# qq456cvb/CanonicalVoting

Hardware: AMD Instinct MI355X
Metric: scenes/sec (80k-pt synthetic scans) (higher is better)
Workload: dtype f32

## Files before the change

canonicalvoting_amd/_lib.py:

```python
import ctypes
import os
import threading

_HERE = os.path.dirname(os.path.abspath(__file__))
LIB_PATH = os.path.join(_HERE, "_C", "libcvhip.so")

c_float_p = ctypes.POINTER(ctypes.c_float)
c_int_p = ctypes.POINTER(ctypes.c_int)
c_i32_p = ctypes.POINTER(ctypes.c_int32)
c_i64_p = ctypes.POINTER(ctypes.c_int64)
vp = ctypes.c_void_p
ABI_VERSION = 6


class CvError(RuntimeError):
    pass


class DecodeParams(ctypes.Structure):
    _fields_ = [("thresh_high", ctypes.c_float), ("thresh_low", ctypes.c_float),
                ("valid_ratio", ctypes.c_float), ("elimination", ctypes.c_int),
                ("prob_thresh", ctypes.c_float), ("elim_hi_plus1", ctypes.c_int),
                ("max_iters", ctypes.c_int), ("err_thresh", ctypes.c_double)]


class ConvDesc(ctypes.Structure):
    _fields_ = [("in_", vp), ("n_in", ctypes.c_longlong), ("in_ld", ctypes.c_int), ("cin", ctypes.c_int),
                ("weight", vp), ("K", ctypes.c_int), ("cout", ctypes.c_int), ("nbr", vp),
                ("n_out", ctypes.c_longlong), ("scale", vp), ("shift", vp), ("residual", vp),
                ("res_ld", ctypes.c_int), ("relu", ctypes.c_int), ("out", vp), ("out_ld", ctypes.c_int),
                ("flavour", ctypes.c_int), ("ws", vp), ("ws_bytes", ctypes.c_size_t), ("row_perm", vp),
                ("j_begin", ctypes.c_int), ("j_end", ctypes.c_int), ("acc_in", vp), ("acc_ld", ctypes.c_int),
                ("perm_groups", ctypes.c_int), ("plan_ent", vp), ("plan_cnt", vp),
                ("weight_packed", vp), ("weight_x6", vp), ("in2", vp), ("in2_ld", ctypes.c_int), ("cin2", ctypes.c_int),
                ("weight2_x6", vp), ("perm_has_map", ctypes.c_int), ("weight_pieces", ctypes.c_int),
                ("acc_scale", ctypes.c_float), ("range_flag", vp), ("in_hl", ctypes.c_int), ("out_hl", ctypes.c_int),
                ("res_hl", ctypes.c_int), ("split_tickets", vp), ("acc_scale_dev", vp)]


class SceneMaps(ctypes.Structure):
    _fields_ = [("stem", ctypes.c_longlong), ("out", ctypes.c_longlong), ("down", ctypes.c_longlong * 4),
                ("k3", ctypes.c_longlong * 5), ("up", ctypes.c_longlong * 4), ("mask_perm", ctypes.c_longlong * 5),
                ("up_perm", ctypes.c_longlong * 4), ("scratch", ctypes.c_longlong), ("bitmap", ctypes.c_longlong)]


class ScenePlanLayout(ctypes.Structure):
    _fields_ = [("cap", ctypes.c_longlong), ("perm", ctypes.c_longlong), ("inv", ctypes.c_longlong),
                ("coords", ctypes.c_longlong * 5), ("vals", ctypes.c_longlong * 5), ("counts", ctypes.c_longlong),
                ("arena", ctypes.c_longlong), ("int_words", ctypes.c_longlong), ("key_words", ctypes.c_longlong),
                ("sort_ws_bytes", ctypes.c_size_t), ("levels_ws_bytes", ctypes.c_size_t)]


NET_MAP_SLOTS, NET_PERM_SLOTS = 15, 9


class NetBuf(ctypes.Structure):
    _fields_ = [("level", ctypes.c_int), ("channels", ctypes.c_int), ("rows_level", ctypes.c_int), ("hl", ctypes.c_int)]


class NetOp(ctypes.Structure):
    _fields_ = [("in_buf", ctypes.c_int), ("in_col", ctypes.c_int), ("cin", ctypes.c_int),
                ("out_buf", ctypes.c_int), ("out_col", ctypes.c_int), ("cout", ctypes.c_int),
                ("res_buf", ctypes.c_int), ("res_col", ctypes.c_int), ("map", ctypes.c_int), ("K", ctypes.c_int),
                ("perm", ctypes.c_int), ("perm_groups", ctypes.c_int), ("relu", ctypes.c_int),
                ("weight", vp), ("scale", vp), ("shift", vp), ("weight_x6", vp), ("in2_buf", ctypes.c_int),
                ("in2_col", ctypes.c_int), ("cin2", ctypes.c_int), ("weight2_x6", vp), ("weight_pieces", ctypes.c_int), ("acc_scale", ctypes.c_float)]


class NetModelParams(ctypes.Structure):
    _fields_ = [("weight_x6", vp), ("weight2_x6", vp), ("scale", vp), ("shift", vp), ("acc_scale", ctypes.c_float),
                ("reserved", ctypes.c_int * 3)]


class SceneDesc(ctypes.Structure):
    _fields_ = [("d_coords4", vp), ("n", ctypes.c_longlong), ("d_feats", vp), ("feats_ld", ctypes.c_int), ("d_points", vp),
                ("res", ctypes.c_float), ("num_rots", ctypes.c_int), ("ops", vp), ("n_ops", ctypes.c_int), ("bufs", vp),
                ("n_bufs", ctypes.c_int), ("stem_k", ctypes.c_int), ("mask_groups", ctypes.c_int),
                ("masked_min_rows", ctypes.c_longlong), ("max_channels", ctypes.c_int),
                ("use_range_flag", ctypes.c_int),
                ("d_out_feats", vp), ("out_ld", ctypes.c_int), ("out_channels", ctypes.c_int), ("nclasses", ctypes.c_int),
                ("log_scale", ctypes.c_int), ("d_xyz_in", vp), ("d_scale_in", vp), ("d_prob_in", vp), ("d_class_in", vp),
                ("vote_algo", ctypes.c_int), ("decode", DecodeParams), ("max_candidates", ctypes.c_int),
                ("nms_threshold", ctypes.c_double), ("d_ws", vp), ("ws_bytes", ctypes.c_size_t), ("d_grids", vp),
                ("grid_capacity_floats", ctypes.c_size_t), ("h_pinned", vp), ("pinned_bytes", ctypes.c_size_t),
                ("h_cand_idx", vp), ("h_verdict", vp), ("h_boxes", vp), ("h_scores", vp), ("h_classes", vp), ("h_pick", vp),
                ("adaptive_split", ctypes.c_int), ("events", vp * 5),
                ("conv_split_target", ctypes.c_int), ("vote_part_records", ctypes.c_int)]


MAX_CATEGORIES = 16


class SceneSeparateDesc(ctypes.Structure):
    _fields_ = [("d_coords4", vp), ("n", ctypes.c_longlong), ("d_feats", vp), ("feats_ld", ctypes.c_int), ("d_points", vp),
                ("res", ctypes.c_float), ("num_rots", ctypes.c_int), ("num_models", ctypes.c_int),
                ("ops", vp), ("n_ops", vp), ("bufs", vp), ("n_bufs", vp),
                ("stem_k", ctypes.c_int), ("mask_groups", ctypes.c_int), ("masked_min_rows", ctypes.c_longlong),
                ("max_channels", ctypes.c_int), ("use_range_flag", ctypes.c_int),
                ("d_out_feats", vp), ("out_ld", ctypes.c_int), ("out_channels", ctypes.c_int), ("log_scale", ctypes.c_int),
                ("d_xyz_in", vp), ("d_scale_in", vp), ("d_prob_in", vp), ("vote_algo", ctypes.c_int), ("decode", DecodeParams),
                ("max_candidates", ctypes.c_int), ("nms_threshold", ctypes.c_double), ("d_ws", vp), ("ws_bytes", ctypes.c_size_t),
                ("h_pinned", vp), ("pinned_bytes", ctypes.c_size_t), ("h_cand_idx", vp), ("h_verdict", vp), ("h_boxes", vp),
                ("h_scores", vp), ("h_det_cat", vp), ("h_det_box", vp), ("events", vp * 5),
                ("conv_split_target", ctypes.c_int), ("vote_part_records", ctypes.c_int),
                ("models_per_pass", ctypes.c_int), ("d_model_params", vp)]


class SceneSeparateResult(ctypes.Structure):
    _fields_ = [("n_cand", ctypes.c_int * MAX_CATEGORIES), ("n_boxes", ctypes.c_int * MAX_CATEGORIES),
                ("truncated", ctypes.c_int * MAX_CATEGORIES), ("n_det", ctypes.c_int), ("range_flag", ctypes.c_int),
                ("duplicates", ctypes.c_int), ("out_of_window", ctypes.c_int), ("dims", ctypes.c_int * 3),
                ("corner", ctypes.c_float * 3), ("level_rows", ctypes.c_longlong * 5), ("needed_ws_bytes", ctypes.c_size_t),
                ("d_grid_obj", vp), ("d_grid_rot", vp), ("d_grid_scale", vp), ("d_xyz", vp), ("d_scale", vp), ("d_prob", vp),
                ("host_us", ctypes.c_float * 4)]


class PackJob(ctypes.Structure):
    _fields_ = [("w", vp), ("wp", vp), ("K", ctypes.c_int), ("cin", ctypes.c_int), ("cout", ctypes.c_int), ("trans", ctypes.c_int),
                ("scale_log2", ctypes.c_int), ("reserved", ctypes.c_int)]


class SceneResult(ctypes.Structure):
    _fields_ = [("n_cand", ctypes.c_int), ("n_boxes", ctypes.c_int), ("n_det", ctypes.c_int), ("truncated", ctypes.c_int),
                ("range_flag", ctypes.c_int), ("duplicates", ctypes.c_int), ("out_of_window", ctypes.c_int),
                ("scenes_in_flight", ctypes.c_int), ("dims", ctypes.c_int * 3), ("corner", ctypes.c_float * 3), ("level_rows", ctypes.c_longlong * 5),
                ("needed_ws_bytes", ctypes.c_size_t), ("needed_grid_floats", ctypes.c_size_t),
                ("d_grid_obj", vp), ("d_grid_rot", vp), ("d_grid_scale", vp), ("d_xyz", vp), ("d_scale", vp),
                ("d_prob", vp), ("d_class", vp), ("host_us", ctypes.c_float * 4)]


GATHER_MAX_JOBS = 8


class GatherJob(ctypes.Structure):
    _fields_ = [("d_src", vp), ("src_ld", ctypes.c_longlong), ("d_dst", vp), ("dst_ld", ctypes.c_longlong),
                ("width", ctypes.c_int), ("recentre_from", ctypes.c_int)]


class PointsFront(ctypes.Structure):
    _fields_ = [("d_raw_points", vp), ("m", ctypes.c_longlong), ("points_ld", ctypes.c_longlong), ("points_f64", ctypes.c_int),
                ("quantization_size", ctypes.c_double), ("d_raw_feats", vp), ("raw_feats_ld", ctypes.c_longlong),
                ("in_channels", ctypes.c_int), ("recentre_from", ctypes.c_int), ("d_raw_xyz", vp), ("d_raw_scale", vp),
                ("d_raw_prob", vp), ("d_raw_class", vp), ("d_coords4", vp), ("d_index", vp), ("d_inverse", vp)]


class PointsDesc(ctypes.Structure):
    _fields_ = [("front", PointsFront), ("scene", SceneDesc)]


class PointsSeparateDesc(ctypes.Structure):
    _fields_ = [("front", PointsFront), ("scene", SceneSeparateDesc)]


class PointsResult(ctypes.Structure):
    _fields_ = [("scene", SceneResult), ("n", ctypes.c_longlong), ("rejected", ctypes.c_int), ("host_us_front", ctypes.c_float),
                ("front_ws_bytes", ctypes.c_size_t), ("d_feats", vp), ("d_points", vp), ("d_xyz_in", vp), ("d_scale_in", vp),
                ("d_prob_in", vp), ("d_class_in", vp)]


class PointsSeparateResult(ctypes.Structure):
    _fields_ = [("scene", SceneSeparateResult), ("n", ctypes.c_longlong), ("rejected", ctypes.c_int),
                ("host_us_front", ctypes.c_float), ("front_ws_bytes", ctypes.c_size_t), ("d_feats", vp), ("d_points", vp),
                ("d_xyz_in", vp), ("d_scale_in", vp), ("d_prob_in", vp)]


SIGNATURES = {
    "cv_abi_version": (ctypes.c_int, []),
    "cv_last_error": (ctypes.c_char_p, []),
    "cv_hv_minmax_workspace_bytes": (ctypes.c_size_t, []),
    "cv_hv_minmax_f32": (ctypes.c_int, [vp, ctypes.c_int64, c_float_p, c_float_p, vp, ctypes.c_size_t, vp]),
    "cv_hv_minmax_async_f32": (ctypes.c_int, [vp, ctypes.c_int64, vp, vp, ctypes.c_size_t, vp]),
    "cv_hv_grid_dims_f32": (ctypes.c_int, [c_float_p, c_float_p, ctypes.c_float, c_int_p]),
    "cv_hv_forward_workspace_bytes": (ctypes.c_size_t, [ctypes.c_int64, ctypes.c_int, c_int_p, ctypes.c_int]),
    "cv_hv_forward_f32": (ctypes.c_int, [vp, vp, vp, vp, ctypes.c_int64, ctypes.c_float, ctypes.c_int,
                                         c_float_p, c_int_p, vp, vp, vp, vp, ctypes.c_size_t,
                                         ctypes.c_int, vp]),
    "cv_hv_forward_cat_workspace_bytes": (ctypes.c_size_t, [ctypes.c_int64, ctypes.c_int, c_int_p, ctypes.c_int, ctypes.c_int]),
    "cv_hv_forward_cat_f32": (ctypes.c_int, [vp, vp, vp, vp, ctypes.c_int64, ctypes.c_float, ctypes.c_int, c_float_p, c_int_p,
                                             ctypes.c_int, vp, vp, vp, vp, ctypes.c_size_t, ctypes.c_int, vp]),
    "cv_hv_set_kernel_events": (ctypes.c_int, [vp, vp]),
    "cv_hv_backward_f32": (ctypes.c_int, [vp, vp, vp, vp, vp, ctypes.c_int64, ctypes.c_float,
                                          ctypes.c_int, c_float_p, c_int_p, vp, vp, vp, vp]),
    "cv_hv_count_votes_f32": (ctypes.c_int, [vp, vp, vp, ctypes.c_int64, ctypes.c_float, ctypes.c_int,
                                             c_float_p, c_int_p, c_i64_p, vp, ctypes.c_size_t, vp]),
    "cv_decode_workspace_bytes": (ctypes.c_size_t, [c_int_p, ctypes.c_int64, ctypes.c_int]),
    "cv_decode_f32": (ctypes.c_int, [vp, vp, vp, c_int_p, c_float_p, ctypes.c_float, vp, vp, vp, vp,
                                     ctypes.c_int64, ctypes.POINTER(DecodeParams), ctypes.c_int, vp,
                                     ctypes.c_size_t, c_int_p, c_i64_p, c_i32_p, c_int_p, c_float_p,
                                     c_float_p, c_i32_p, c_int_p, vp]),
    "cv_decode_cat_workspace_bytes": (ctypes.c_size_t, [c_int_p, ctypes.c_int64, ctypes.c_int, ctypes.c_int]),
    "cv_decode_cat_f32": (ctypes.c_int, [vp, vp, vp, c_int_p, c_float_p, ctypes.c_float, vp, vp, vp, vp, ctypes.c_int64,
                                         ctypes.c_int, ctypes.POINTER(DecodeParams), ctypes.c_int, vp, ctypes.c_size_t, c_int_p,
                                         c_i64_p, c_i32_p, c_int_p, c_float_p, c_float_p, c_i32_p, c_int_p, vp]),
    "cv_detect_scene_separate_f32": (ctypes.c_int, [ctypes.POINTER(SceneSeparateDesc), ctypes.POINTER(SceneSeparateResult), vp]),
    "cv_sp_table_capacity": (ctypes.c_longlong, [ctypes.c_longlong]),
    "cv_sp_levels_workspace_bytes": (ctypes.c_size_t, [ctypes.c_longlong]),
    "cv_sp_build_levels": (ctypes.c_int, [ctypes.POINTER(vp), ctypes.POINTER(vp), ctypes.POINTER(vp),
                                          ctypes.c_longlong, ctypes.c_longlong, ctypes.c_int, vp,
                                          c_i32_p, vp, ctypes.c_size_t, vp]),
    "cv_sp_quantize_workspace_bytes": (ctypes.c_size_t, [ctypes.c_longlong]),
    "cv_sp_quantize_f32": (ctypes.c_int, [vp, ctypes.c_longlong, ctypes.c_longlong, ctypes.c_float, ctypes.c_int, c_i64_p,
                                          ctypes.c_int, vp, vp, vp, vp, c_i32_p, vp, ctypes.c_size_t, vp]),
    "cv_sp_quantize_f64": (ctypes.c_int, [vp, ctypes.c_longlong, ctypes.c_longlong, ctypes.c_double, ctypes.c_int, c_i64_p,
                                          ctypes.c_int, vp, vp, vp, vp, c_i32_p, vp, ctypes.c_size_t, vp]),
    "cv_sp_voxel_rows_f32": (ctypes.c_int, [vp, vp, ctypes.c_longlong, ctypes.c_float, vp, ctypes.POINTER(GatherJob), ctypes.c_int, vp]),
    "cv_sizeof_gather_job": (ctypes.c_size_t, []),
    "cv_sp_morton_keys": (ctypes.c_int, [vp, ctypes.c_longlong, vp, vp]),
    "cv_sp_sort_workspace_bytes": (ctypes.c_size_t, [ctypes.c_longlong]),
    "cv_sp_sort_rows": (ctypes.c_int, [vp, ctypes.c_longlong, vp, vp, vp, vp, ctypes.c_size_t, vp]),
    "cv_sp_pack_weights_stem_h2_f32": (ctypes.c_int, [vp, ctypes.c_int, ctypes.c_int, vp, ctypes.c_int, vp, vp]),
    "cv_sp_to_hl_f32": (ctypes.c_int, [vp, ctypes.c_longlong, ctypes.c_int, ctypes.c_int, vp, ctypes.c_int, vp, vp]),
    "cv_sp_from_hl_f32": (ctypes.c_int, [vp, ctypes.c_longlong, ctypes.c_int, ctypes.c_int, vp, ctypes.c_int, vp]),
    "cv_sp_kernel_map": (ctypes.c_int, [vp, ctypes.c_longlong, vp, vp, ctypes.c_longlong, ctypes.c_int,
                                        ctypes.c_int, vp, vp]),
    "cv_sp_up_map": (ctypes.c_int, [vp, ctypes.c_longlong, ctypes.c_longlong, vp, vp]),
    "cv_sp_conv_workspace_bytes": (ctypes.c_size_t, [ctypes.c_longlong, ctypes.c_int, ctypes.c_int]),
    "cv_sp_conv_f32": (ctypes.c_int, [ctypes.POINTER(ConvDesc), vp]),
    "cv_sp_set_split_target": (ctypes.c_int, [ctypes.c_int]),
    "cv_hv_set_part_records": (ctypes.c_int, [ctypes.c_int]),
    "cv_hv_set_part_records_thread": (ctypes.c_int, [ctypes.c_int]),
    "cv_sp_pack_weights_h2_batch_f32": (ctypes.c_int, [ctypes.POINTER(PackJob), ctypes.c_int, vp, vp]),
    "cv_sp_copy_unless_flag": (ctypes.c_int, [ctypes.POINTER(vp), ctypes.POINTER(vp), ctypes.POINTER(ctypes.c_longlong), ctypes.c_int, vp, vp]),
    "cv_sp_pack_weights_t_f32": (ctypes.c_int, [vp, ctypes.c_int, ctypes.c_int, ctypes.c_int, ctypes.c_int, ctypes.c_int, vp, vp]),
    "cv_sp_set_split_target_thread": (ctypes.c_int, [ctypes.c_int]),
    "cv_sp_set_ablation": (ctypes.c_int, [ctypes.c_int]),
    "cv_sp_set_option": (ctypes.c_int, [ctypes.c_char_p, ctypes.c_longlong, ctypes.POINTER(ctypes.c_longlong)]),
    "cv_sp_get_option": (ctypes.c_int, [ctypes.c_char_p, ctypes.POINTER(ctypes.c_longlong)]),
    "cv_sp_pack_weights_x6_f32": (ctypes.c_int, [vp, ctypes.c_int, ctypes.c_int, ctypes.c_int, vp, vp, vp]),
    "cv_sp_pack_weights_h2_f32": (ctypes.c_int, [vp, ctypes.c_int, ctypes.c_int, ctypes.c_int, vp, ctypes.c_int, vp, vp]),
    "cv_sp_pack_weights_bf16_f32": (ctypes.c_int, [vp, ctypes.c_int, ctypes.c_int, ctypes.c_int, vp, vp, vp]),
    "cv_sp_scene_maps_words": (ctypes.c_size_t, [c_i64_p, ctypes.c_longlong, ctypes.c_int, ctypes.c_int,
                                                 ctypes.c_longlong, ctypes.POINTER(SceneMaps)]),
    "cv_sp_scene_maps": (ctypes.c_int, [ctypes.POINTER(vp), ctypes.POINTER(vp), ctypes.POINTER(vp), ctypes.c_longlong,
                                        c_i64_p, vp, ctypes.c_longlong, ctypes.c_int,
                                        ctypes.c_int, ctypes.c_longlong, vp, ctypes.c_size_t, vp]),
    "cv_sp_scene_plan_words": (ctypes.c_size_t, [ctypes.c_longlong, ctypes.c_int, ctypes.c_int, ctypes.c_longlong]),
    "cv_sp_scene_plan": (ctypes.c_int, [vp, ctypes.c_longlong, vp, vp, ctypes.POINTER(vp), ctypes.POINTER(vp),
                                        ctypes.POINTER(vp), ctypes.c_longlong, vp, c_i32_p, ctypes.c_int, ctypes.c_int,
                                        ctypes.c_longlong, vp, ctypes.c_size_t, ctypes.POINTER(SceneMaps), vp,
                                        ctypes.c_size_t, vp, ctypes.c_size_t, vp]),
    "cv_sp_scene_plan_layout": (ctypes.c_int, [ctypes.c_longlong, ctypes.c_int, ctypes.c_int, ctypes.c_longlong,
                                               ctypes.POINTER(ScenePlanLayout)]),
    "cv_sp_scene_plan_slots": (ctypes.c_int, [ctypes.POINTER(ScenePlanLayout), ctypes.POINTER(SceneMaps), c_i64_p,
                                              ctypes.c_longlong, vp, ctypes.POINTER(vp), ctypes.POINTER(vp)]),
    "cv_sp_scene_conv_workspace_bytes": (ctypes.c_size_t, [c_i64_p, c_int_p, ctypes.c_int, ctypes.c_int]),
    "cv_net_arena_bytes": (ctypes.c_size_t, [ctypes.POINTER(NetBuf), ctypes.c_int, c_i64_p, ctypes.c_int]),
    "cv_net_run_f32": (ctypes.c_int, [ctypes.POINTER(NetOp), ctypes.c_int, ctypes.POINTER(NetBuf), ctypes.c_int,
                                      c_i64_p, ctypes.c_int, vp, ctypes.c_size_t, ctypes.POINTER(vp), c_int_p,
                                      ctypes.POINTER(vp), ctypes.c_int, ctypes.POINTER(vp), ctypes.c_int,
                                      vp, ctypes.c_size_t, vp, vp]),
    "cv_net_models_params_bytes": (ctypes.c_size_t, [ctypes.c_int, ctypes.c_int]),
    "cv_net_models_params_fill": (ctypes.c_int, [ctypes.POINTER(vp), ctypes.c_int, ctypes.c_int, vp, ctypes.c_size_t]),
    "cv_net_models_arena_bytes": (ctypes.c_size_t, [ctypes.POINTER(NetBuf), ctypes.c_int, c_i64_p, ctypes.c_int, ctypes.c_int]),
    "cv_net_models_workspace_bytes": (ctypes.c_size_t, [ctypes.c_size_t, ctypes.c_int]),
    "cv_net_run_models_f32": (ctypes.c_int, [ctypes.POINTER(vp), ctypes.POINTER(vp), ctypes.c_int, ctypes.c_int, ctypes.c_int,
                                             c_i64_p, ctypes.c_int, vp, ctypes.c_size_t, ctypes.POINTER(vp), c_int_p,
                                             ctypes.POINTER(vp), ctypes.c_int, ctypes.POINTER(vp), ctypes.c_int,
                                             vp, ctypes.c_size_t, vp, vp, ctypes.c_int, vp]),
    "cv_head_separate_models_f32": (ctypes.c_int, [ctypes.POINTER(vp), ctypes.c_int, ctypes.c_longlong, ctypes.c_int, ctypes.c_int,
                                                   vp, vp, vp, vp]),
    "cv_sp_mask_keys": (ctypes.c_int, [vp, ctypes.c_longlong, ctypes.c_int, ctypes.c_int, ctypes.c_int, vp, vp]),
    "cv_sp_mask_perms": (ctypes.c_int, [vp, ctypes.c_longlong, ctypes.c_int, ctypes.c_int, vp, vp, ctypes.c_size_t,
                                        ctypes.c_int, vp]),
    "cv_sp_transpose_map": (ctypes.c_int, [vp, ctypes.c_longlong, ctypes.c_int, ctypes.c_longlong, vp, vp]),
    "cv_sp_wgrad_workspace_bytes": (ctypes.c_size_t, [ctypes.c_longlong, ctypes.c_int, ctypes.c_int, ctypes.c_int]),
    "cv_sp_conv_wgrad_f32": (ctypes.c_int, [vp, ctypes.c_int, ctypes.c_int, vp, ctypes.c_int, ctypes.c_int, vp,
                                            ctypes.c_int, ctypes.c_longlong, vp, vp, ctypes.c_size_t, vp]),
    "cv_sp_conv_wgrad_px_f32": (ctypes.c_int, [vp, ctypes.c_int, ctypes.c_int, vp, ctypes.c_int, ctypes.c_int, vp,
                                               ctypes.c_int, ctypes.c_longlong, vp, vp, ctypes.c_size_t, ctypes.c_int,
                                               vp]),
    "cv_sp_col_sum_f32": (ctypes.c_int, [vp, ctypes.c_longlong, ctypes.c_int, ctypes.c_int, vp, vp]),
    "cv_sp_col_sum_workspace_bytes": (ctypes.c_size_t, [ctypes.c_longlong, ctypes.c_int]),
    "cv_sp_col_sum_det_f32": (ctypes.c_int, [vp, ctypes.c_longlong, ctypes.c_int, ctypes.c_int, vp, vp, ctypes.c_size_t, vp]),
    "cv_sp_bn_workspace_bytes": (ctypes.c_size_t, [ctypes.c_int]),
    "cv_sp_bn_stats_f32": (ctypes.c_int, [vp, ctypes.c_longlong, ctypes.c_int, ctypes.c_int, vp, vp, ctypes.c_float,
                                          ctypes.c_float, vp, vp, vp, vp, vp, vp, vp, ctypes.c_size_t, vp]),
    "cv_sp_bn_backward_f32": (ctypes.c_int, [vp, vp, vp, ctypes.c_longlong, ctypes.c_int, ctypes.c_int, vp, vp,
                                             ctypes.c_float, vp, vp, vp, vp, vp, vp, ctypes.c_size_t, vp]),
    "cv_sp_bn_backward_hl_f32": (ctypes.c_int, [vp, vp, vp, ctypes.c_longlong, ctypes.c_int, ctypes.c_int, vp, vp,
                                                ctypes.c_float, vp, vp, vp, vp, vp, vp, ctypes.c_size_t, vp, vp, vp, vp, vp]),
    "cv_sp_affine_f32": (ctypes.c_int, [vp, ctypes.c_longlong, ctypes.c_int, ctypes.c_int, vp, vp, vp, ctypes.c_int,
                                        ctypes.c_int, vp, ctypes.c_int, vp]),
    "cv_sp_affine_hl_f32": (ctypes.c_int, [vp, ctypes.c_longlong, ctypes.c_int, ctypes.c_int, vp, vp, vp, ctypes.c_int,
                                           ctypes.c_int, vp, ctypes.c_int, vp, ctypes.c_int, vp, vp, vp]),
    "cv_sp_bn_fold_f32": (ctypes.c_int, [vp, vp, vp, vp, vp, ctypes.c_float, ctypes.c_int, vp, vp, vp]),
    "cv_head_joint_f32": (ctypes.c_int, [vp, ctypes.c_longlong, ctypes.c_int, ctypes.c_int, ctypes.c_int,
                                         vp, vp, vp, vp, vp]),
    "cv_head_separate_f32": (ctypes.c_int, [vp, ctypes.c_longlong, ctypes.c_int, ctypes.c_int, vp, vp, vp, vp]),
    "cv_detect_scene_f32": (ctypes.c_int, [ctypes.POINTER(SceneDesc), ctypes.POINTER(SceneResult), vp]),
    "cv_detect_points_f32": (ctypes.c_int, [ctypes.POINTER(PointsDesc), ctypes.POINTER(PointsResult), vp]),
    "cv_detect_points_separate_f32": (ctypes.c_int, [ctypes.POINTER(PointsSeparateDesc), ctypes.POINTER(PointsSeparateResult), vp]),
    "cv_sizeof_points_desc": (ctypes.c_size_t, []),
    "cv_sizeof_points_separate_desc": (ctypes.c_size_t, []),
    "cv_sizeof_points_result": (ctypes.c_size_t, []),
    "cv_sizeof_points_separate_result": (ctypes.c_size_t, []),
    "cv_iou_obb": (ctypes.c_double, [c_float_p, c_float_p]),
    "cv_nms_obb": (ctypes.c_int, [c_float_p, c_float_p, ctypes.c_int, ctypes.c_double, c_i32_p]),
}

_lib = None


def lib():
    global _lib
    if _lib is None:
        if not os.path.exists(LIB_PATH):
            raise CvError(
                "canonicalvoting_amd: HIP library %s not found. Build it with "
                "`python -m canonicalvoting_amd.csrc.build` (hipcc, gfx950). There is no CPU "
                "fallback for this op." % LIB_PATH)
        import torch
        if torch.cuda.is_available():
            torch.cuda.init()
        L = ctypes.CDLL(LIB_PATH)
        for name, (res, args) in SIGNATURES.items():
            fn = getattr(L, name)
            fn.restype = res
            fn.argtypes = args
        _lib = L
    return _lib


_scratch_lock = threading.Lock()
_scratch_bufs = {}


def scratch(dev, name, nbytes):
    import torch
    key = (dev.index if dev.index is not None else torch.cuda.current_device(),
           torch.cuda.current_stream(dev).cuda_stream, name)
    nbytes = max(int(nbytes), 256)
    with _scratch_lock:
# ... 26 lines not shown
```

canonicalvoting_amd/csrc/hv_vote.hip:

```cpp
#include "cv_common.h"

#include <atomic>
#include <algorithm>
#include <cmath>
#include <cstddef>
#include <mutex>
#include <type_traits>
#include <unordered_map>
#include <vector>

namespace {

struct F3 { float x, y, z; };
struct I3 { int x, y, z; };

std::mutex g_tab_mu;
std::unordered_map<uint64_t, float2*> g_tabs;

int get_rot_table(int num_rots, const float2** out) {
    int dev = 0;
    CV_HIP_CHECK(hipGetDevice(&dev));
    const uint64_t key = (uint64_t(uint32_t(dev)) << 32) | uint32_t(num_rots);
    std::lock_guard<std::mutex> lk(g_tab_mu);
    auto it = g_tabs.find(key);
// ... 343 lines not shown
    __shared__ int wsum[FILL ? 1 : LIST_MAX_TILES];
    const int ntiles = tiles_x * tiles_z;
    const int c = blockIdx.x;
    if (c >= chunk_start[Y]) return;
    if (FILL && list_ctl[1] != 0) return;
    const int bin = bin_of_chunk[c];
    const int idx = ystart[bin] + (c - chunk_start[bin]) * LIST_CHUNK_RECORDS + (int)threadIdx.x;
    const int end = ystart[bin + 1];
    for (int t = threadIdx.x; t < ntiles; t += 1024) {
        cnt[t] = FILL ? list_start[(int64_t)bin * ntiles + t] + chunk_off[(int64_t)c * ntiles + t] : 0;
        if (!FILL) wsum[t] = 0;
    }
    __syncthreads();
    if (idx < end) {
        const float ux = rec[9 * rec_stride + idx], uz = rec[10 * rec_stride + idx], r = rec[11 * rec_stride + idx];
        const float a0 = rec[12 * rec_stride + idx];
        const float ext = r + 2.f + 1e-5f * (r + fabsf(ux) + fabsf(uz));
        const int tx0 = max(0, (int)floorf((ux - ext - (float)TX) / (float)TX));
        const int tx1 = min(tiles_x - 1, (int)floorf((ux + ext + 1.f) / (float)TX));
        const int tz0 = max(0, (int)floorf((uz - ext - (float)TZ) / (float)TZ));
        const int tz1 = min(tiles_z - 1, (int)floorf((uz + ext + 1.f) / (float)TZ));
        for (int tx = tx0; tx <= tx1; ++tx)
            for (int tz = tz0; tz <= tz1; ++tz) {
                const float xlo = (float)(tx * TX - 1), xhi = (float)(tx * TX + TX), zlo = (float)(tz * TZ - 1),
                            zhi = (float)(tz * TZ + TZ);
                float dxn, dzn;
                if (!ring_touches(ux, uz, r, xlo, xhi, zlo, zhi, dxn, dzn)) continue;
                int a_start, a_len;
                ring_arc(ux, uz, a0, R, xlo, xhi, zlo, zhi, dxn, dzn, a_start, a_len);
                const int t = tx * tiles_z + tz;
                if (FILL) {
                    const int p = atomicAdd(&cnt[t], 1);
                    entries[p] = make_int2(idx, a_start | (a_len << 16));
                } else {
                    if (want_lists) atomicAdd(&cnt[t], 1);
                    atomicAdd(&wsum[t], a_len);
                }
            }
    }
    if (FILL) return;
    __syncthreads();
    for (int t = threadIdx.x; t < ntiles; t += 1024) {
        if (want_lists) chunk_off[(int64_t)c * ntiles + t] = cnt[t] ? atomicAdd(&list_cnt[(int64_t)bin * ntiles + t], cnt[t]) : 0;
        if (wsum[t]) atomicAdd(&tile_w[(int64_t)bin * ntiles + t], wsum[t]);
    }
}

__global__ __launch_bounds__(1024) void hv_list_scan(const int* __restrict__ list_cnt, int Y, int ntiles, long long list_cap,
                                                     int* __restrict__ list_ctl, int* __restrict__ list_start, int64_t ks_ws) {
    list_cnt = cat_ws(list_cnt, ks_ws); list_ctl = cat_ws(list_ctl, ks_ws); list_start = cat_ws(list_start, ks_ws);
    __shared__ int s[1024];
    __shared__ long long carry_s;
    if (threadIdx.x == 0) carry_s = 0;
    __syncthreads();
    const int total_lists = Y * ntiles;
    for (int base = 0; base < total_lists; base += 1024) {
        const int i = base + threadIdx.x;
        const int v = i < total_lists ? list_cnt[i] : 0;
        s[threadIdx.x] = v;
        __syncthreads();
        for (int off = 1; off < 1024; off <<= 1) {
            const int t = (int)threadIdx.x >= off ? s[threadIdx.x - off] : 0;
            __syncthreads();
            s[threadIdx.x] += t;
            __syncthreads();
        }
        const long long incl = (long long)s[threadIdx.x] + carry_s;
        if (i < total_lists) list_start[i] = incl - v < 0x7fffffffll ? (int)(incl - v) : 0x7fffffff;
        __syncthreads();
        if (threadIdx.x == 1023) carry_s = incl;
        __syncthreads();
    }
    if (threadIdx.x == 0) { list_ctl[0] = carry_s < 0x7fffffffll ? (int)carry_s : 0x7fffffff; list_ctl[1] = carry_s > list_cap ? 1 : 0; }
}

constexpr int PART_VOTES = 32768;
constexpr int QUEUE_MAX_PARTS = 32;

__global__ __launch_bounds__(1024) void hv_build_queue(const int* __restrict__ tile_w, int Y, int ntiles, int max_items,
                                                       int max_slots, int* __restrict__ list_ctl ,
                                                       int4* __restrict__ items, int64_t ks_ws) {
    tile_w = cat_ws(tile_w, ks_ws); list_ctl = cat_ws(list_ctl, ks_ws); items = cat_ws(items, ks_ws);
    __shared__ unsigned long long s[1024];
    __shared__ unsigned long long carry_s;
    const int total = Y * ntiles;
    for (int pass = 0; pass < 2; ++pass) {
        if (threadIdx.x == 0) carry_s = 0ull;
        __syncthreads();
        for (int base = 0; base < total; base += 1024) {
            const int i = base + threadIdx.x;
            int parts = 0, y = 0, t = 0;
            if (i < total) {
                y = i / ntiles; t = i - y * ntiles;
                const long long w = (long long)(y >= 1 ? tile_w[(int64_t)(y - 1) * ntiles + t] : 0) +
                                    (long long)(y <= Y - 2 ? tile_w[(int64_t)y * ntiles + t] : 0);
                parts = w == 0 ? 0 : (pass ? 1 : (int)min((long long)QUEUE_MAX_PARTS, (w + PART_VOTES - 1) / PART_VOTES));
            }
            const unsigned long long v = i < total ? (((unsigned long long)max(parts, 1) << 32) | (unsigned)(parts > 1 ? parts : 0)) : 0ull;
            s[threadIdx.x] = v;
            __syncthreads();
            for (int off = 1; off < 1024; off <<= 1) {
                const unsigned long long x = (int)threadIdx.x >= off ? s[threadIdx.x - off] : 0ull;
                __syncthreads();
                s[threadIdx.x] += x;
                __syncthreads();
            }
            const unsigned long long excl = s[threadIdx.x] + carry_s - v;
            const int item0 = (int)(excl >> 32), slot0 = (int)(excl & 0xffffffffull);
            if (i < total && item0 + max(parts, 1) <= max_items && slot0 + (parts > 1 ? parts : 0) <= max_slots) {
                if (parts == 0) items[item0] = make_int4(y, t, 0, 0);
                for (int p2 = 0; p2 < parts; ++p2) items[item0 + p2] = make_int4(y, t, p2 | (parts << 8), slot0);
            }
            __syncthreads();
            if (threadIdx.x == 1023) carry_s = s[1023] + carry_s;
            __syncthreads();
        }
        const int n_items = (int)(carry_s >> 32), n_slots = (int)(carry_s & 0xffffffffull);
        if (n_items <= max_items && n_slots <= max_slots) {
            if (threadIdx.x == 0) list_ctl[2] = n_items;
            return;
        }
        __syncthreads();
    }
    if (threadIdx.x == 0) list_ctl[2] = min(total, max_items);
}

__device__ __forceinline__ int lanes_below(uint64_t mask) {
    return __builtin_amdgcn_mbcnt_hi((uint32_t)(mask >> 32),
                                     __builtin_amdgcn_mbcnt_lo((uint32_t)mask, 0));
}

constexpr double FX_SCALE = 68719476736.0;
constexpr double FX_MAGIC = 6755399441055744.0;
template <bool SMALL>
__device__ __forceinline__ unsigned long long fx_from_float(float v) {
    if (SMALL) {
        const double d = __builtin_fma((double)v, FX_SCALE, FX_MAGIC);
        return (unsigned long long)__double_as_longlong(d) - (unsigned long long)__double_as_longlong(FX_MAGIC);
    }
    return (unsigned long long)__double2ll_rn((double)fminf(fmaxf(v, -6.0e7f), 6.0e7f) * FX_SCALE);
}
template <bool SMALL>
__device__ __forceinline__ void lds_add(unsigned long long* p, float v) {
    __hip_atomic_fetch_add(p, fx_from_float<SMALL>(v), __ATOMIC_RELAXED, __HIP_MEMORY_SCOPE_WORKGROUP);
}
__device__ __forceinline__ double fx_value(unsigned long long q) { return (double)(long long)q * (1.0 / FX_SCALE); }
template <bool SMALL>
__device__ __forceinline__ void lds_add_obj(unsigned long long* p, float v) {
    unsigned long long q = fx_from_float<SMALL>(v);
    if (q == 0ull && v != 0.f) q = v > 0.f ? 1ull : ~0ull;
    __hip_atomic_fetch_add(p, q, __ATOMIC_RELAXED, __HIP_MEMORY_SCOPE_WORKGROUP);
}

constexpr int ACC_PITCH = TZ + 8, ACC_CH = TX * ACC_PITCH + 4, ACC_WORDS = 6 * ACC_CH;
__device__ __forceinline__ int acc_idx(int ch, int cell) { return ch * ACC_CH + (cell >> 5) * ACC_PITCH + (cell & 31); }

struct TileShared {
    unsigned long long acc[ACC_WORDS];
    float pq[9][LQ];
    int arc_start[LQ];
    int arc_cum[LQ];
    uint32_t vq_rec[TW][VQ];
    float vq_rx[TW][VQ];
    float vq_rz[TW][VQ];
    float2 tab[MAX_R_TILES];
    int next_chunk[2];
    int wtot[TW];
    int list_len;
    int more;
};

template <bool SMALL>
__device__ __forceinline__ void drain_vote(TileShared& sh, int lx, int lz, float rx, float rz, float wy, float ob,
                                           float s0, float s1, float s2, float2 cs) {
    const float wx[2] = {1.f - rx, rx}, wz[2] = {1.f - rz, rz};
#pragma unroll
    for (int bx = 0; bx < 2; ++bx)
#pragma unroll
        for (int bz = 0; bz < 2; ++bz) {
            const int cxl = lx + bx, czl = lz + bz;
            if (cxl < 0 || cxl >= TX || czl < 0 || czl >= TZ) continue;
            const float w = wx[bx] * wy * wz[bz] * ob;
            unsigned long long* a = sh.acc + cxl * ACC_PITCH + czl;
            lds_add_obj<SMALL>(a, w);
            lds_add<SMALL>(a + ACC_CH, w * cs.x);
            lds_add<SMALL>(a + 2 * ACC_CH, w * cs.y);
            lds_add<SMALL>(a + 3 * ACC_CH, w * s0);
            lds_add<SMALL>(a + 4 * ACC_CH, w * s1);
            lds_add<SMALL>(a + 5 * ACC_CH, w * s2);
        }
}

__device__ __forceinline__ void drain64(TileShared& sh, int wave, int slot, bool active) {
    float rx = 0.f, rz = 0.f, wy = 0.f, ob = 0.f, s0 = 0.f, s1 = 0.f, s2 = 0.f;
    float2 cs = make_float2(0.f, 0.f);
    int lx = 0, lz = 0;
    if (active) {
        const uint32_t rec = sh.vq_rec[wave][slot];
        rx = sh.vq_rx[wave][slot]; rz = sh.vq_rz[wave][slot];
        const int e = rec & 511, rot = (rec >> 9) & 255;
        lx = (int)((rec >> 17) & 63) - 1; lz = (int)((rec >> 23) & 63) - 1;
        wy = sh.pq[4][e]; ob = sh.pq[5][e];
        s0 = sh.pq[6][e]; s1 = sh.pq[7][e]; s2 = sh.pq[8][e];
        cs = sh.tab[rot];
    }
    const bool small = fabsf(ob) * fmaxf(1.f, fmaxf(fabsf(s0), fmaxf(fabsf(s1), fabsf(s2)))) < 16384.f;
    if (__all(small)) {
        if (active) drain_vote<true>(sh, lx, lz, rx, rz, wy, ob, s0, s1, s2, cs);
    } else {
        if (active) drain_vote<false>(sh, lx, lz, rx, rz, wy, ob, s0, s1, s2, cs);
    }
}

__device__ __forceinline__ void wave_sync_lds() {
    __builtin_amdgcn_fence(__ATOMIC_RELEASE, "wavefront");
    __builtin_amdgcn_wave_barrier();
    __builtin_amdgcn_fence(__ATOMIC_ACQUIRE, "wavefront");
}

__device__ __forceinline__ float arc_atan2(float y, float x) {
    const float ax = fabsf(x), ay = fabsf(y);
    const float a = fminf(ax, ay) * __builtin_amdgcn_rcpf(fmaxf(fmaxf(ax, ay), 1e-30f));
    const float q = a * a;
    float r = ((-0.0464964749f * q + 0.15931422f) * q - 0.327622764f) * q * a + a;
    r = ay > ax ? 1.57079637f - r : r;
    r = x < 0.f ? 3.14159274f - r : r;
    return y < 0.f ? -r : r;
}

__device__ __forceinline__ void edge_arc(float ux, float uz, float r, float a0, int R, float xlo, float xhi, float zlo,
                                         float zhi, int& a_start, int& a_len) {
    if (!(r >= 2.f)) return;
    const float slack = 0.05f, half_pi = 1.57079637f, two_pi = 6.28318531f;
    const float d4[4] = {xhi - ux, zhi - uz, ux - xlo, uz - zlo};
    const float inv_r = 1.f / r;
    float h[4];
#pragma unroll
    for (int k = 0; k < 4; ++k) {
        const float t = (d4[k] + slack) * inv_r;
        const float hk = arc_atan2(sqrtf(fmaxf(1.f - t * t, 0.f)), t) - 0.01f;
        h[k] = (t < 1.f && hk > 0.f) ? hk : -1.f;
    }
    float best = 0.f, best_end = 0.f;
#pragma unroll
    for (int k = 0; k < 4; ++k) {
        float lo = -h[k], hi = h[k];
        bool ok = h[k] > 0.f;
        if (ok && hi - lo > best) { best = hi - lo; best_end = (float)k * half_pi + hi; }
#pragma unroll
        for (int j = 1; j < 4; ++j) {
            const float hp = h[(k + j - 1) & 3], hn = h[(k + j) & 3];
            ok = ok && hn > 0.f && hp + hn >= half_pi;
            if (ok) {
                lo = fminf(lo, (float)j * half_pi - hn);
                hi = fmaxf(hi, (float)j * half_pi + hn);
                if (hi - lo > best) { best = hi - lo; best_end = (float)k * half_pi + hi; }
            }
        }
    }
    const float inside = fmaxf(two_pi - best, 0.f);
    const float inv_step = (float)R * 0.159154943f;
    const int len = (int)(inside * inv_step) + 6;
    if (len < a_len) {
        float first = (best_end - a0) * inv_step - 2.f;
        first -= (float)R * floorf(first / (float)R);
        a_start = min(max((int)first, 0), R - 1);
        a_len = len;
    }
}

template <bool QUEUE>
__global__ __launch_bounds__(TW * 64) void hv_fwd_tiles(
    int R, float res, F3 corner, I3 dims, const float2* __restrict__ tab,
    const int* __restrict__ ystart, const int4* __restrict__ items, const float* __restrict__ rec,
    int64_t rec_stride, int tiles_x, int tiles_z, unsigned long long* __restrict__ partials,
    int* __restrict__ arrivals, float* __restrict__ g_obj, float* __restrict__ g_rot,
    float* __restrict__ g_scale, const int* __restrict__ list_ctl, const int* __restrict__ list_start, const int* __restrict__ list_cnt,
    const int2* __restrict__ entries, int list_mode ,
    const int4* __restrict__ q_info, CatStride ks) {
    ystart = cat_ws(ystart, ks.ws); items = cat_ws(items, ks.ws); rec = cat_ws(rec, ks.ws);
    partials = cat_ws(partials, ks.ws); arrivals = cat_ws(arrivals, ks.ws); list_ctl = cat_ws(list_ctl, ks.ws);
    list_start = cat_ws(list_start, ks.ws); list_cnt = cat_ws(list_cnt, ks.ws); entries = cat_ws(entries, ks.ws);
    q_info = cat_ws(q_info, ks.ws);
    g_obj = cat_el(g_obj, ks.cells); g_rot = cat_el(g_rot, 2 * ks.cells); g_scale = cat_el(g_scale, 3 * ks.cells);
    __shared__ TileShared sh;
    __shared__ int last_flag;
    const int X = dims.x, Y = dims.y, Z = dims.z;
    const int ntiles = tiles_x * tiles_z;
    int y, tile, part, nparts, slot0, slot_stride;
    if (QUEUE) {
        if ((int)blockIdx.x >= list_ctl[2]) return;
        const int4 item = items[blockIdx.x];
        y = item.x; tile = item.y; part = item.z & 0xff; nparts = item.z >> 8; slot0 = item.w; slot_stride = 1;
    } else {
        tile = blockIdx.x % ntiles;
        const int4 qi = q_info[blockIdx.x / ntiles];
        if (qi.z < 0) return;
        y = qi.x; part = qi.y; nparts = qi.z;
        slot0 = qi.w * ntiles + tile; slot_stride = ntiles;
    }
    const int x0 = (tile / tiles_z) * TX, z0 = (tile % tiles_z) * TZ;
    const int lane = threadIdx.x & 63, wave = threadIdx.x >> 6;
    if (nparts == 0) {
        const int nx0 = min(TX, X - x0), nz0 = min(TZ, Z - z0);
        for (int i = threadIdx.x; i < TCELLS; i += TW * 64) {
            const int lx = i / TZ, lz = i % TZ;
            if (lx < nx0 && lz < nz0) {
                const int64_t cell = ((int64_t)(x0 + lx) * Y + y) * Z + z0 + lz;
                g_obj[cell] = 0.f;
                reinterpret_cast<float2*>(g_rot)[cell] = make_float2(0.f, 0.f);
                g_scale[cell * 3 + 0] = 0.f; g_scale[cell * 3 + 1] = 0.f; g_scale[cell * 3 + 2] = 0.f;
            }
        }
        return;
    }
    const bool use_list = QUEUE && list_mode == 2 && list_ctl[1] == 0;
    int lbeg[2] = {0, 0}, llen[2] = {0, 0};
    if (use_list) {
#pragma unroll
        for (int k = 0; k < 2; ++k) {
            const int s = y - 1 + k;
            if (s >= 0 && s <= Y - 2) {
                lbeg[k] = list_start[(int64_t)s * ntiles + tile];
                llen[k] = list_cnt[(int64_t)s * ntiles + tile];
            }
        }
    }

    int bin_beg[2], bin_end[2];
#pragma unroll
    for (int k = 0; k < 2; ++k) {
        const int s = y - 1 + k;
        const bool valid = s >= 0 && s <= Y - 2;
        bin_beg[k] = !valid ? 0 : (use_list ? lbeg[k] : ystart[s]);
        bin_end[k] = !valid ? 0 : (use_list ? lbeg[k] + llen[k] : ystart[s + 1]);
    }
    const float2 tab_mine = (int)threadIdx.x < R ? tab[threadIdx.x] : make_float2(0.f, 0.f);
    for (int i = threadIdx.x; i < ACC_WORDS; i += TW * 64) sh.acc[i] = 0ull;
    if ((int)threadIdx.x < R) sh.tab[threadIdx.x] = tab_mine;
    if (threadIdx.x < 2) sh.next_chunk[threadIdx.x] = 0;
    if (threadIdx.x == 2) { sh.list_len = 0; sh.more = 0; }
    __syncthreads();

    const float slack = 0.05f;
    const float xlo = (float)(x0 - 1), xhi = (float)(x0 + TX), zlo = (float)(z0 - 1),
                zhi = (float)(z0 + TZ);
    int vq_len = 0;

    const int per = use_list ? LIST_CHUNK : 64;
    int sb = 0;
    int c_mask = 0, c_idx[CULL_BATCH], c_arc = 0, c_k = 0;
#pragma unroll
    for (int j = 0; j < CULL_BATCH; ++j) c_idx[j] = 0;
    auto append = [&](int mask, const int (&idx)[CULL_BATCH], int arc, int k) -> int {
        int tot = 0, before[CULL_BATCH];
#pragma unroll
        for (int j = 0; j < CULL_BATCH; ++j) {
            const uint64_t m = __ballot((mask >> j) & 1);
            before[j] = tot + lanes_below(m);
            tot += __popcll(m);
        }
        if (tot == 0) return 0;
        int p0 = 0;
        if (lane == 0) p0 = atomicAdd(&sh.list_len, tot);
        p0 = __builtin_amdgcn_readfirstlane(p0);
#pragma unroll
        for (int j = 0; j < CULL_BATCH; ++j) {
            const int pos = p0 + before[j];
            if (((mask >> j) & 1) && pos < LQ) {
                sh.arc_start[pos] = idx[j] | (int)((unsigned)k << 31);
                if (use_list) sh.arc_cum[pos] = arc;
                mask &= ~(1 << j);
            }
        }
        return mask;
    };

    for (;;) {
        bool more = false;
        if (__ballot(c_mask != 0) != 0) {
            c_mask = append(c_mask, c_idx, c_arc, c_k);
            more = __ballot(c_mask != 0) != 0;
        }
        while (!more && sb < 2) {
            if (bin_beg[sb] >= bin_end[sb]) { ++sb; continue; }
            const int len = __builtin_amdgcn_readfirstlane(
                __hip_atomic_load(&sh.list_len, __ATOMIC_RELAXED, __HIP_MEMORY_SCOPE_WORKGROUP));
            if (len > LQ - 64) { more = true; break; }
            const int take = use_list ? 64 / LIST_CHUNK : CULL_BATCH;
            int c = 0;
            if (lane == 0) c = atomicAdd(&sh.next_chunk[sb], take);
            c = __builtin_amdgcn_readfirstlane(c);
            const int end = bin_end[sb];
            if (bin_beg[sb] + (c * nparts + part) * per >= end) { ++sb; continue; }
            int idx[CULL_BATCH], mask = 0, arc = 0;
#pragma unroll
            for (int j = 0; j < CULL_BATCH; ++j) idx[j] = 0;
            if (use_list) {
                const int e = bin_beg[sb] + ((c + lane / LIST_CHUNK) * nparts + part) * LIST_CHUNK + lane % LIST_CHUNK;
                if (e < end) {
                    const int2 en = entries[e];
                    idx[0] = en.x;
                    arc = en.y;
                    mask = 1;
                }
            } else {
                float ux[CULL_BATCH], uz[CULL_BATCH], r[CULL_BATCH];
#pragma unroll
                for (int j = 0; j < CULL_BATCH; ++j) {
                    idx[j] = bin_beg[sb] + ((c + j) * nparts + part) * 64 + lane;
                    const bool in = idx[j] < end;
                    ux[j] = in ? rec[9 * rec_stride + idx[j]] : 0.f;
                    uz[j] = in ? rec[10 * rec_stride + idx[j]] : 0.f;
                    r[j] = in ? rec[11 * rec_stride + idx[j]] : 0.f;
                }
#pragma unroll
                for (int j = 0; j < CULL_BATCH; ++j) {
                    const float dxn = fmaxf(0.f, fmaxf(xlo - ux[j], ux[j] - xhi));
                    const float dzn = fmaxf(0.f, fmaxf(zlo - uz[j], uz[j] - zhi));
                    const float dxf = fmaxf(fabsf(ux[j] - xlo), fabsf(ux[j] - xhi));
                    const float dzf = fmaxf(fabsf(uz[j] - zlo), fabsf(uz[j] - zhi));
                    const float dmin = sqrtf(dxn * dxn + dzn * dzn), dmax = sqrtf(dxf * dxf + dzf * dzf);
                    const float tol = slack + 1e-5f * (r[j] + fabsf(ux[j]) + fabsf(uz[j]));
                    const bool keep = idx[j] < end && (r[j] >= dmin - tol) && (r[j] <= dmax + tol);
                    mask |= (int)keep << j;
                }
            }
            c_mask = append(mask, idx, arc, sb);
            if (__ballot(c_mask != 0) != 0) {
#pragma unroll
                for (int j = 0; j < CULL_BATCH; ++j) c_idx[j] = idx[j];
                c_arc = arc; c_k = sb;
                more = true;
            }
        }
        if (more && lane == 0) sh.more = 1;
        __syncthreads();
        const int n = min(sh.list_len, LQ);
        const bool again = sh.more != 0;
        if (n == 0) break;

        const int p = threadIdx.x;
        int a_start = 0, a_len = 0;
        if (p < n) {
            const int w = sh.arc_start[p];
            const int idx = w & 0x7fffffff;
            if (use_list) {
                const int arc = sh.arc_cum[p];
                a_start = arc & 0xffff;
                a_len = arc >> 16;
            } else {
                const float ux = rec[9 * rec_stride + idx], uz = rec[10 * rec_stride + idx];
                const float dxn = fmaxf(0.f, fmaxf(xlo - ux, ux - xhi));
                const float dzn = fmaxf(0.f, fmaxf(zlo - uz, uz - zhi));
                a_len = R;
                if (dxn + dzn > 0.5f) {
                    const float b0 = arc_atan2(0.5f * (zlo + zhi) - uz, 0.5f * (xlo + xhi) - ux);
                    float lo = 0.f, hi = 0.f;
#pragma unroll
                    for (int k = 0; k < 4; ++k) {
                        float d = arc_atan2(((k & 2) ? zhi : zlo) - uz, ((k & 1) ? xhi : xlo) - ux) - b0;
                        d -= 6.28318531f * rintf(d * 0.159154943f);
                        lo = fminf(lo, d);
                        hi = fmaxf(hi, d);
                    }
                    const float a0 = rec[12 * rec_stride + idx];
                    const float inv_step = (float)R * 0.159154943f;
                    float first = (b0 + lo - a0) * inv_step - 2.f;
                    const int len = (int)((hi - lo) * inv_step) + 6;
                    first -= (float)R * floorf(first / (float)R);
                    a_start = min(max((int)first, 0), R - 1);
                    a_len = min(len, R);
                }
                edge_arc(ux, uz, rec[11 * rec_stride + idx], rec[12 * rec_stride + idx], R, xlo, xhi, zlo, zhi, a_start, a_len);
            }
            const float ry = rec[4 * rec_stride + idx];
            sh.pq[0][p] = rec[0 * rec_stride + idx];
            sh.pq[1][p] = rec[1 * rec_stride + idx];
            sh.pq[2][p] = rec[2 * rec_stride + idx];
            sh.pq[3][p] = rec[3 * rec_stride + idx];
            sh.pq[4][p] = (w < 0) ? (1.f - ry) : ry;
            sh.pq[5][p] = rec[5 * rec_stride + idx];
            sh.pq[6][p] = rec[6 * rec_stride + idx];
            sh.pq[7][p] = rec[7 * rec_stride + idx];
            sh.pq[8][p] = rec[8 * rec_stride + idx];
            sh.arc_start[p] = a_start;
        }
        int cum = a_len;
#pragma unroll
        for (int off = 1; off < 64; off <<= 1) {
            const int t = __shfl_up(cum, off);
            if (lane >= off) cum += t;
        }
        if (lane == 63) sh.wtot[wave] = cum;
        __syncthreads();
        if (threadIdx.x == 0) { sh.list_len = 0; sh.more = 0; }
        int items = 0;
#pragma unroll
        for (int w = 0; w < TW; ++w) {
            const int t = sh.wtot[w];
            if (w < wave) cum += t;
            items += t;
        }
        if (p < n) sh.arc_cum[p] = cum;
        __syncthreads();

        const int S = (items + LQ - 1) / LQ;
        const int slice = wave * 64 + lane;
        int it0 = slice * S;
        const int it1 = min(it0 + S, items);
        int e = 0;
        {
            int lo = 0, hi = n - 1;
            while (lo < hi) {
                const int mid = (lo + hi) >> 1;
                if (sh.arc_cum[mid] > it0) hi = mid; else lo = mid + 1;
            }
            e = lo;
        }
        int e_end = it0 < items ? sh.arc_cum[e] : 0;
        int rot = 0;
        float epx = 0.f, epz = 0.f, ecx = 0.f, ecz = 0.f;
        if (it0 < items) {
            const int e_beg = e > 0 ? sh.arc_cum[e - 1] : 0;
            rot = sh.arc_start[e] + (it0 - e_beg);
            if (rot >= R) rot -= R;
            epx = sh.pq[0][e]; epz = sh.pq[1][e];
            ecx = sh.pq[2][e]; ecz = sh.pq[3][e];
        }
        for (int step = 0; step < S; ++step, ++it0) {
            bool isvote = false;
            uint32_t vrec = 0;
            float rx = 0, rz = 0;
            if (it0 < it1) {
                if (it0 == e_end) {
                    ++e;
                    e_end = sh.arc_cum[e];
                    rot = sh.arc_start[e];
                    epx = sh.pq[0][e]; epz = sh.pq[1][e];
                    ecx = sh.pq[2][e]; ecz = sh.pq[3][e];
                }
                const float2 cs = sh.tab[rot];
                const float ox = (-cs.x) * ecx + cs.y * ecz;
                const float oz = (-cs.y) * ecx - cs.x * ecz;
                const float gx = grid_pos(epx, ox, corner.x, res);
                const float gz = grid_pos(epz, oz, corner.z, res);
                if (gx >= 0 && gz >= 0 && gx < (float)(X - 1) && gz < (float)(Z - 1)) {
                    const int lx = (int)gx - x0, lz = (int)gz - z0;
                    if (lx >= -1 && lx < TX && lz >= -1 && lz < TZ) {
                        isvote = true;
                        rx = gx - floorf(gx);
                        rz = gz - floorf(gz);
                        vrec = (uint32_t)e | ((uint32_t)rot << 9) | ((uint32_t)(lx + 1) << 17) |
                               ((uint32_t)(lz + 1) << 23);
                    }
                }
                if (++rot == R) rot = 0;
            }
            const uint64_t mv = __ballot(isvote);
            if (isvote) {
                const int q = vq_len + lanes_below(mv);
                sh.vq_rec[wave][q] = vrec;
                sh.vq_rx[wave][q] = rx;
                sh.vq_rz[wave][q] = rz;
            }
            vq_len += __popcll(mv);
            wave_sync_lds();
            if (vq_len >= 64) {
                vq_len -= 64;
                drain64(sh, wave, vq_len + lane, true);
            }
        }
        if (vq_len > 0) {
            drain64(sh, wave, lane, lane < vq_len);
            vq_len = 0;
        }
        wave_sync_lds();
        if (!again) break;
        __syncthreads();
    }
    __syncthreads();

    if (nparts > 1) {
        unsigned long long* mine = partials + ((int64_t)slot0 + (int64_t)part * slot_stride) * (6 * TCELLS);
        for (int i = threadIdx.x; i < 6 * TCELLS; i += TW * 64) mine[i] = sh.acc[acc_idx(i / TCELLS, i % TCELLS)];
        asm volatile("s_waitcnt vmcnt(0)" ::: "memory");
        __syncthreads();
        if (threadIdx.x == 0) {
            __builtin_amdgcn_fence(__ATOMIC_RELEASE, "agent");
            asm volatile("s_waitcnt vmcnt(0)" ::: "memory");
            const int old = __hip_atomic_fetch_add(&arrivals[y * ntiles + tile], 1, __ATOMIC_RELAXED,
                                                   __HIP_MEMORY_SCOPE_AGENT);
            last_flag = old == nparts - 1;
            if (last_flag) __builtin_amdgcn_fence(__ATOMIC_ACQUIRE, "agent");
        }
        __syncthreads();
        if (!last_flag) return;
        const unsigned long long* base = partials + (int64_t)slot0 * (6 * TCELLS);
        for (int i = threadIdx.x; i < 6 * TCELLS; i += TW * 64) {
            unsigned long long sum = 0ull;
            for (int p2 = 0; p2 < nparts; ++p2) sum += base[(int64_t)p2 * slot_stride * (6 * TCELLS) + i];
            sh.acc[acc_idx(i / TCELLS, i % TCELLS)] = sum;
        }
        __syncthreads();
    }

    const int nx = min(TX, X - x0), nz = min(TZ, Z - z0);
    for (int i = threadIdx.x; i < TCELLS; i += TW * 64) {
        const int lx = i / TZ, lz = i % TZ;
        if (lx < nx && lz < nz)
            g_obj[((int64_t)(x0 + lx) * Y + y) * Z + z0 + lz] = (float)fx_value(sh.acc[acc_idx(0, i)]);
    }
    for (int i = threadIdx.x; i < TCELLS * 2; i += TW * 64) {
        const int cell = i >> 1, j = i & 1;
        const int lx = cell / TZ, lz = cell % TZ;
        if (lx < nx && lz < nz) {
            const double d = (double)(float)fx_value(sh.acc[acc_idx(0, cell)]) + 1e-7;
            g_rot[(((int64_t)(x0 + lx) * Y + y) * Z + z0 + lz) * 2 + j] =
                (float)((double)(float)fx_value(sh.acc[acc_idx(1 + j, cell)]) / d);
        }
    }
    for (int i = threadIdx.x; i < TCELLS * 3; i += TW * 64) {
        const int cell = i / 3, j = i - cell * 3;
        const int lx = cell / TZ, lz = cell % TZ;
        if (lx < nx && lz < nz) {
            const double d = (double)(float)fx_value(sh.acc[acc_idx(0, cell)]) + 1e-7;
            g_scale[(((int64_t)(x0 + lx) * Y + y) * Z + z0 + lz) * 3 + j] =
                (float)((double)(float)fx_value(sh.acc[acc_idx(3 + j, cell)]) / d);
        }
    }
}

__global__ __launch_bounds__(256) void hv_bwd(
    const float* __restrict__ grad, const float* __restrict__ pts, const float* __restrict__ xyz,
    const float* __restrict__ scl, const float* __restrict__ obj, int64_t n, int R, float res,
    F3 corner, I3 dims, const float2* __restrict__ tab, float* __restrict__ d_xyz,
    float* __restrict__ d_scl, float* __restrict__ d_obj) {
    const int lane = threadIdx.x & 63;
    const int64_t c = blockIdx.x * 4ll + (threadIdx.x >> 6);
    if (c >= n) return;
    const int Y = dims.y, Z = dims.z;
    const float s0 = scl[c * 3 + 0], s1 = scl[c * 3 + 1], s2 = scl[c * 3 + 2];
    const float x0 = xyz[c * 3 + 0], x1 = xyz[c * 3 + 1], x2 = xyz[c * 3 + 2];
    const float cx = x0 * s0, cy = x1 * s1, cz = x2 * s2;
    const float px = pts[c * 3 + 0], py = pts[c * 3 + 1], pz = pts[c * 3 + 2];
    const float ob = obj[c];
    float a_obj = 0, a_x0 = 0, a_x1 = 0, a_x2 = 0, a_s0 = 0, a_s1 = 0, a_s2 = 0;
    for (int i = lane; i < R; i += 64) {
        const float2 cs = tab[i];
        const float ox = (-cs.x) * cx + cs.y * cz;
        const float oy = -cy;
        const float oz = (-cs.y) * cx - cs.x * cz;
        const float gx = grid_pos(px, ox, corner.x, res);
        const float gy = grid_pos(py, oy, corner.y, res);
        const float gz = grid_pos(pz, oz, corner.z, res);
        if (gx < 0 || gy < 0 || gz < 0 || gx >= (float)(dims.x - 1) || gy >= (float)(dims.y - 1) ||
            gz >= (float)(dims.z - 1))
            continue;
        const int fx = (int)gx, fy = (int)gy, fz = (int)gz;
        const float rx = gx - floorf(gx), ry = gy - floorf(gy), rz = gz - floorf(gz);
        const float w0x = 1.f - rx, w0y = 1.f - ry, w0z = 1.f - rz, w1x = rx, w1y = ry, w1z = rz;
        const int64_t b = ((int64_t)fx * Y + fy) * Z + fz;
        const int64_t sx = (int64_t)Y * Z, sy = Z;
        const float lll = grad[b], llh = grad[b + 1], lhl = grad[b + sy], lhh = grad[b + sy + 1];
        const float hll = grad[b + sx], hlh = grad[b + sx + 1], hhl = grad[b + sx + sy],
                    hhh = grad[b + sx + sy + 1];
        float dob = lll * w0x * w0y * w0z;
        dob += llh * w0x * w0y * w1z;
        dob += lhl * w0x * w1y * w0z;
        dob += lhh * w0x * w1y * w1z;
        dob += hll * w1x * w0y * w0z;
        dob += hlh * w1x * w0y * w1z;
        dob += hhl * w1x * w1y * w0z;
        dob += hhh * w1x * w1y * w1z;
        a_obj += dob;
        float dx = -lll * w0y * w0z;
        dx = dx - llh * w0y * w1z; dx = dx - lhl * w1y * w0z; dx = dx - lhh * w1y * w1z;
        dx = dx + hll * w0y * w0z; dx = dx + hlh * w0y * w1z; dx = dx + hhl * w1y * w0z;
        dx = dx + hhh * w1y * w1z;
        float dy = -lll * w0x * w0z;
        dy = dy - llh * w0x * w1z; dy = dy + lhl * w0x * w0z; dy = dy + lhh * w0x * w1z;
        dy = dy - hll * w1x * w0z; dy = dy - hlh * w1x * w1z; dy = dy + hhl * w1x * w0z;
        dy = dy + hhh * w1x * w1z;
        float dz = -lll * w0x * w0y;
        dz = dz + llh * w0x * w0y; dz = dz - lhl * w0x * w1y; dz = dz + lhh * w0x * w1y;
        dz = dz - hll * w1x * w0y; dz = dz + hlh * w1x * w0y; dz = dz - hhl * w1x * w1y;
        dz = dz + hhh * w1x * w1y;
        dx *= ob; dy *= ob; dz *= ob;
        const float dcx = (-cs.x) * dx - cs.y * dz;
        const float dcy = -dy;
        const float dcz = cs.y * dx - cs.x * dz;
        a_x0 += dcx * s0; a_x1 += dcy * s1; a_x2 += dcz * s2;
        a_s0 += dcx * x0; a_s1 += dcy * x1; a_s2 += dcz * x2;
    }
#pragma unroll
    for (int off = 32; off > 0; off >>= 1) {
        a_obj += __shfl_xor(a_obj, off);
        a_x0 += __shfl_xor(a_x0, off); a_x1 += __shfl_xor(a_x1, off); a_x2 += __shfl_xor(a_x2, off);
        a_s0 += __shfl_xor(a_s0, off); a_s1 += __shfl_xor(a_s1, off); a_s2 += __shfl_xor(a_s2, off);
    }
    if (lane == 0) {
        d_obj[c] = a_obj;
        d_xyz[c * 3 + 0] = a_x0; d_xyz[c * 3 + 1] = a_x1; d_xyz[c * 3 + 2] = a_x2;
        d_scl[c * 3 + 0] = a_s0; d_scl[c * 3 + 1] = a_s1; d_scl[c * 3 + 2] = a_s2;
    }
}

__global__ __launch_bounds__(256) void hv_count_votes(
    const float* __restrict__ pts, const float* __restrict__ xyz, const float* __restrict__ scl,
    int64_t n, int R, float res, F3 corner, I3 dims, const float2* __restrict__ tab,
    unsigned long long* __restrict__ count) {
    unsigned local = 0;
    for (int64_t t = blockIdx.x * 256ll + threadIdx.x; t < n * R; t += (int64_t)gridDim.x * 256) {
        const int64_t c = t / R;
        const int i = (int)(t - c * R);
        const float cx = xyz[c * 3 + 0] * scl[c * 3 + 0], cy = xyz[c * 3 + 1] * scl[c * 3 + 1],
                    cz = xyz[c * 3 + 2] * scl[c * 3 + 2];
        const float2 cs = tab[i];
        const float ox = (-cs.x) * cx + cs.y * cz, oy = -cy, oz = (-cs.y) * cx - cs.x * cz;
        const float gx = grid_pos(pts[c * 3 + 0], ox, corner.x, res);
        const float gy = grid_pos(pts[c * 3 + 1], oy, corner.y, res);
        const float gz = grid_pos(pts[c * 3 + 2], oz, corner.z, res);
        local += !(gx < 0 || gy < 0 || gz < 0 || gx >= (float)(dims.x - 1) ||
                   gy >= (float)(dims.y - 1) || gz >= (float)(dims.z - 1));
    }
    __shared__ unsigned s[256];
    s[threadIdx.x] = local;
    __syncthreads();
    for (int st = 128; st > 0; st >>= 1) {
        if (threadIdx.x < st) s[threadIdx.x] += s[threadIdx.x + st];
        __syncthreads();
    }
    if (threadIdx.x == 0 && s[0]) atomicAdd(count, (unsigned long long)s[0]);
}

__global__ __launch_bounds__(256) void hv_zero_cat(int* __restrict__ base, int64_t words, int64_t ks_ws) {
    base = cat_ws(base, ks_ws);
    for (int64_t i = blockIdx.x * 256ll + threadIdx.x; i < words; i += (int64_t)gridDim.x * 256) base[i] = 0;
}

int check_common(const void* a, const void* b, const void* c, int64_t n, float res, int num_rots,
                 const float* corner, const int* dims) {
    CV_REQUIRE(a && b && c && corner && dims, CV_EINVAL, "null pointer argument");
    CV_REQUIRE(n > 0, CV_EINVAL, "n must be positive (got %lld)", (long long)n);
    CV_REQUIRE(res > 0.f, CV_EINVAL, "res must be positive");
    CV_REQUIRE(num_rots > 0 && num_rots <= 4096, CV_EINVAL, "num_rots out of range (%d)", num_rots);
    CV_REQUIRE(dims[0] > 0 && dims[1] > 0 && dims[2] > 0, CV_EINVAL, "bad grid dims");
    CV_REQUIRE((int64_t)dims[0] * dims[1] * dims[2] < (1ll << 31), CV_EINVAL, "grid too large");
    CV_REQUIRE(n * (int64_t)num_rots < (1ll << 40), CV_EINVAL, "n*num_rots too large");
    return CV_OK;
}

int64_t tiles_q_bound(int64_t n, int Y) { return (int64_t)Y + (2 * n + PART_RECORDS - 1) / PART_RECORDS; }
constexpr int QUEUE_MIN_TILES = 128;
int64_t queue_max_slots(int64_t n, int num_rots) { return 4 * n * (int64_t)num_rots / PART_VOTES + 256; }
int64_t queue_max_items(int64_t n, int num_rots, int64_t Y, int64_t ntiles) { return Y * ntiles + queue_max_slots(n, num_rots); }
int64_t list_capacity(int64_t n, int64_t ntiles) { return std::min<int64_t>(n * ntiles, 40 * n + 65536); }

struct TilesLayout {
    bool queue;
    int tiles_x, tiles_z, ntiles;
    int64_t max_q;
    int64_t max_items, max_slots;
    int64_t list_cap, max_chunks;
    int* fy; float* rec;
    int* list_ctl; int* list_cnt; int* tile_w; int* ycount; int* arrivals;
    int* ystart; int* cursor; int* part_start; int4* q_info;
    unsigned long long* partials;
    int4* items; int* list_start; int* chunk_start; int* bin_of_chunk; int* chunk_off; int2* entries;
    int* zero_from;
    size_t zero_bytes;
    size_t bytes;
};
TilesLayout tiles_layout(int64_t n, int num_rots, const int* dims, void* base) {
    TilesLayout L{};
    const size_t Y = (size_t)dims[1];
    L.tiles_x = (dims[0] + TX - 1) / TX;
    L.tiles_z = (dims[2] + TZ - 1) / TZ;
    const int64_t ntiles = (int64_t)L.tiles_x * L.tiles_z;
    L.ntiles = (int)ntiles;
    L.max_q = tiles_q_bound(n, (int)Y);
    L.max_slots = queue_max_slots(n, num_rots);
    L.max_items = queue_max_items(n, num_rots, (int64_t)Y, ntiles);
    L.list_cap = list_capacity(n, ntiles);
    L.max_chunks = (int64_t)Y + (n + LIST_CHUNK_RECORDS - 1) / LIST_CHUNK_RECORDS;
    L.queue = ntiles >= QUEUE_MIN_TILES && ntiles <= LIST_MAX_TILES && L.list_cap < (1ll << 31) && L.max_items < (1ll << 31);
    const size_t q = L.queue ? 1 : 0, planes = Y * (size_t)ntiles;
    size_t off = 0;
    auto take = [&](auto*& p, size_t count) {
        off = cv_align_up(off, 256);
        const size_t at = off;
        p = reinterpret_cast<std::remove_reference_t<decltype(p)>>(reinterpret_cast<uintptr_t>(base) + at);
        off += count * sizeof(*p);
        return at;
    };
    take(L.fy, (size_t)n);
    take(L.rec, (size_t)n * REC_F);
    const size_t ctl_at = take(L.list_ctl, 64);
    take(L.list_cnt, q * planes);
    take(L.tile_w, q * planes);
    const size_t ycount_at = take(L.ycount, Y);
    take(L.arrivals, planes);
    L.zero_from = L.queue ? L.list_ctl : L.ycount;
    L.zero_bytes = off - (L.queue ? ctl_at : ycount_at);
    take(L.ystart, Y + 1);
    take(L.cursor, Y);
    take(L.part_start, Y + 1);
    take(L.q_info, (size_t)L.max_q);
    take(L.partials, (size_t)(L.queue ? L.max_slots : L.max_q * ntiles) * 6 * TCELLS);
    take(L.items, q * (size_t)L.max_items);
    take(L.list_start, q * planes);
    take(L.chunk_start, Y + 1);
    take(L.bin_of_chunk, (size_t)L.max_chunks);
    take(L.chunk_off, q * (size_t)L.max_chunks * (size_t)ntiles);
    take(L.entries, q * (size_t)L.list_cap);
    L.bytes = cv_align_up(off, 256);
    return L;
}

bool algo_ok(int algo) { return algo >= 0 && algo <= 2; }
int pick_algo(int algo, int64_t n, int num_rots) {
    if (algo == 1 || algo == 2) return algo;
    if (num_rots <= MAX_R_TILES && n < (1ll << 31)) return 2;
    return 1;
}

}

extern "C" {

size_t cv_hv_minmax_workspace_bytes(void) { return 256 + sizeof(float) * 6 * (MM_BLOCKS + 1) + 256; }

int cv_hv_minmax_f32(const float* d_points, int64_t n, float* h_min3, float* h_max3, void* d_ws,
                     size_t ws_bytes, void* stream) {
    CV_REQUIRE(h_min3 && h_max3, CV_EINVAL, "null pointer argument");
    float h[6];
    const int rc = cv_hv_minmax_async_ex(d_points, n, h, d_ws, ws_bytes, nullptr, nullptr, stream);
    if (rc) return rc;
    CV_HIP_CHECK(hipStreamSynchronize(static_cast<hipStream_t>(stream)));
    for (int k = 0; k < 3; ++k) { h_min3[k] = h[k]; h_max3[k] = h[3 + k]; }
    return CV_OK;
}

int cv_hv_minmax_async_f32(const float* d_points, int64_t n, float* h_minmax6, void* d_ws, size_t ws_bytes,
                           void* stream) {
    return cv_hv_minmax_async_ex(d_points, n, h_minmax6, d_ws, ws_bytes, nullptr, nullptr, stream);
}

}

int cv_hv_minmax_async_ex(const float* d_points, int64_t n, float* h_minmax6, void* d_ws, size_t ws_bytes, int32_t* d_zero_word,
                          int32_t* d_fill7f, void* stream) {
    CV_REQUIRE(d_points && h_minmax6 && d_ws, CV_EINVAL, "null pointer argument");
    CV_REQUIRE(n > 0, CV_EINVAL, "n must be positive (got %lld)", (long long)n);
    CV_REQUIRE(ws_bytes >= cv_hv_minmax_workspace_bytes(), CV_ENOMEM, "workspace too small");
    hipStream_t st = static_cast<hipStream_t>(stream);
    CvCarver cv(d_ws);
    float* part = cv.take<float>(6 * MM_BLOCKS);
    float* out = cv.take<float>(6);
    const int blocks = (int)std::min<int64_t>(MM_BLOCKS, (n + 255) / 256);
    minmax_partial<<<blocks, 256, 0, st>>>(d_points, n, part);
    CV_LAUNCH_CHECK();
    minmax_final<<<1, 256, 0, st>>>(part, blocks, out, d_zero_word, d_fill7f);
    CV_LAUNCH_CHECK();
    CV_HIP_CHECK(hipMemcpyAsync(h_minmax6, out, 6 * sizeof(float), hipMemcpyDeviceToHost, st));
    return CV_OK;
}

extern "C" {

int cv_hv_grid_dims_f32(const float h_min3[3], const float h_max3[3], float res, int dims_out[3]) {
    CV_REQUIRE(h_min3 && h_max3 && dims_out, CV_EINVAL, "null pointer argument");
    CV_REQUIRE(res > 0.f, CV_EINVAL, "res must be positive");
    for (int k = 0; k < 3; ++k) {
        volatile float d = h_max3[k] - h_min3[k];
        volatile float q = d / res;
        dims_out[k] = (int)q + 1;
    }
    return CV_OK;
}

size_t cv_hv_forward_workspace_bytes(int64_t n, int num_rots, const int dims[3], int algo) {
    if (!dims || n <= 0 || !algo_ok(algo)) return 0;
    if (pick_algo(algo, n, num_rots) == 1) return 256;
    return tiles_layout(n, num_rots, dims, nullptr).bytes;
}

static thread_local hipEvent_t t_ev_start = nullptr, t_ev_stop = nullptr;

static std::atomic<long long> g_part_records{getenv("CV_HV_PART_RECORDS") ? std::max<long long>(PART_RECORDS, atoll(getenv("CV_HV_PART_RECORDS")))
                                                                          : (long long)PART_RECORDS};

static thread_local long long t_part_records = 0;

int cv_hv_set_part_records(int records) {
    const long long v = records <= 0 ? (long long)PART_RECORDS : std::max<long long>(PART_RECORDS, records);
    return (int)g_part_records.exchange(v, std::memory_order_relaxed);
}

int cv_hv_set_part_records_thread(int records) {
    const int before = (int)t_part_records;
    t_part_records = records <= 0 ? 0 : std::max<long long>(PART_RECORDS, records);
    return before;
}

int cv_hv_set_kernel_events(void* ev_start, void* ev_stop) {
    t_ev_start = static_cast<hipEvent_t>(ev_start);
    t_ev_stop = static_cast<hipEvent_t>(ev_stop);
    return CV_OK;
}

size_t cv_hv_forward_cat_workspace_bytes(int64_t n, int num_rots, const int dims[3], int algo, int num_cats) {
    if (num_cats < 1 || num_cats > CV_MAX_CATEGORIES) return 0;
    return (size_t)num_cats * cv_hv_forward_workspace_bytes(n, num_rots, dims, algo);
}

static int hv_forward_cats(const float* d_points, const float* d_xyz, const float* d_scale, const float* d_obj, int64_t n,
                           float res, int num_rots, const float h_corner3[3], const int dims[3], float* d_grid_obj,
                           float* d_grid_rot, float* d_grid_scale, void* d_ws, size_t ws_bytes, int algo, int K,
                           hipStream_t st) {
    int rc = CV_OK;
    const float2* tab = nullptr;
    rc = get_rot_table(num_rots, &tab);
    if (rc) return rc;
    const F3 corner{h_corner3[0], h_corner3[1], h_corner3[2]};
    const I3 d3{dims[0], dims[1], dims[2]};
    const int64_t cells = (int64_t)dims[0] * dims[1] * dims[2];
    const int a = pick_algo(algo, n, num_rots);
    if (a == 2) CV_REQUIRE(num_rots <= MAX_R_TILES, CV_EINVAL, "tiles algorithm needs num_rots <= %d", MAX_R_TILES);
    if (a == 1) {
        for (int k = 0; k < K; ++k) {
            float* g_obj = d_grid_obj + (int64_t)k * cells;
            float* g_rot = d_grid_rot + (int64_t)k * cells * 2;
            float* g_scale = d_grid_scale + (int64_t)k * cells * 3;
            CV_HIP_CHECK(hipMemsetAsync(g_obj, 0, sizeof(float) * cells, st));
            CV_HIP_CHECK(hipMemsetAsync(g_rot, 0, sizeof(float) * cells * 2, st));
            CV_HIP_CHECK(hipMemsetAsync(g_scale, 0, sizeof(float) * cells * 3, st));
            const int64_t total = n * num_rots;
            hv_fwd_direct<<<(unsigned)((total + 255) / 256), 256, 0, st>>>(
                d_points, d_xyz + (int64_t)k * n * 3, d_scale + (int64_t)k * n * 3, d_obj + (int64_t)k * n, n, num_rots, res,
                corner, d3, tab, g_obj, g_rot, g_scale);
            CV_LAUNCH_CHECK();
            hv_normalise<<<(unsigned)((cells + 255) / 256), 256, 0, st>>>(g_obj, g_rot, g_scale, cells);
            CV_LAUNCH_CHECK();
        }
        return CV_OK;
    }
    const int Y = dims[1];
    const TilesLayout L = tiles_layout(n, num_rots, dims, d_ws);
    CV_REQUIRE(d_ws && ws_bytes >= (size_t)K * L.bytes, CV_ENOMEM, "workspace too small for the tiles algorithm");
    const CatStride ks{K > 1 ? (int64_t)L.bytes : 0, n, cells};
    const int tiles_x = L.tiles_x, tiles_z = L.tiles_z, ntiles = L.ntiles;
    const bool queue = L.queue;
    const int list_mode = queue ? 2 : 1;
    if (K == 1) CV_HIP_CHECK(hipMemsetAsync(L.zero_from, 0, L.zero_bytes, st));
    else {
        hv_zero_cat<<<dim3((unsigned)std::min<size_t>((L.zero_bytes / 4 + 255) / 256, 1024), K), 256, 0, st>>>(L.zero_from,
                                                                                                          L.zero_bytes / 4, ks.ws);
        CV_LAUNCH_CHECK();
    }
    const unsigned prep_wgs = (unsigned)((n + PREP_THREADS - 1) / PREP_THREADS);
    hv_prep_count<<<dim3(prep_wgs, K), PREP_THREADS, 0, st>>>(d_points, d_xyz, d_scale, n, res, corner.y, Y, L.fy, L.ycount, ks);
    CV_LAUNCH_CHECK();
    hv_prep_scan<<<dim3(1, K), 256, 0, st>>>(L.ycount, Y, L.ystart, L.cursor, L.part_start, L.q_info, (int)L.max_q, L.chunk_start,
                                             L.bin_of_chunk,
                                             (int)(t_part_records > 0 ? t_part_records : g_part_records.load(std::memory_order_relaxed)),
                                             ks.ws);
    CV_LAUNCH_CHECK();
    hv_prep_scatter<<<dim3(prep_wgs, K), PREP_THREADS, 0, st>>>(d_points, d_xyz, d_scale, d_obj, L.fy, n, Y, res, corner, L.cursor,
                                                                 L.rec, n, ks);
    CV_LAUNCH_CHECK();
    if (queue) {
        hv_list_pass<false><<<dim3((unsigned)L.max_chunks, K), 1024, 0, st>>>(L.ystart, L.chunk_start, L.bin_of_chunk, Y, L.rec, n,
                                                                               num_rots, tiles_x, tiles_z, L.list_ctl, L.list_cnt,
                                                                               L.list_start, L.chunk_off, L.entries, L.tile_w, 1, ks.ws);
        CV_LAUNCH_CHECK();
        hv_build_queue<<<dim3(1, K), 1024, 0, st>>>(L.tile_w, Y, ntiles, (int)L.max_items, (int)L.max_slots, L.list_ctl, L.items,
                                                    ks.ws);
        CV_LAUNCH_CHECK();
        hv_list_scan<<<dim3(1, K), 1024, 0, st>>>(L.list_cnt, Y, ntiles, L.list_cap, L.list_ctl, L.list_start, ks.ws);
        CV_LAUNCH_CHECK();
        hv_list_pass<true><<<dim3((unsigned)L.max_chunks, K), 1024, 0, st>>>(L.ystart, L.chunk_start, L.bin_of_chunk, Y, L.rec, n,
                                                                              num_rots, tiles_x, tiles_z, L.list_ctl, L.list_cnt,
                                                                              L.list_start, L.chunk_off, L.entries, L.tile_w, 1, ks.ws);
        CV_LAUNCH_CHECK();
    }
    const int64_t wgs = queue ? L.max_items : L.max_q * ntiles;
    CV_REQUIRE(wgs < (1ll << 31), CV_EINVAL, "grid too large");
#define CV_TILES_ARGS num_rots, res, corner, d3, tab, L.ystart, L.items, L.rec, n, tiles_x, tiles_z, L.partials, L.arrivals, d_grid_obj, \
                      d_grid_rot, d_grid_scale, L.list_ctl, L.list_start, L.list_cnt, L.entries, list_mode, L.q_info, ks
    if (t_ev_start) CV_HIP_CHECK(hipEventRecord(t_ev_start, st));
    if (queue) hv_fwd_tiles<true><<<dim3((unsigned)wgs, K), TW * 64, 0, st>>>(CV_TILES_ARGS);
    else hv_fwd_tiles<false><<<dim3((unsigned)wgs, K), TW * 64, 0, st>>>(CV_TILES_ARGS);
    if (t_ev_stop) CV_HIP_CHECK(hipEventRecord(t_ev_stop, st));
#undef CV_TILES_ARGS
    CV_LAUNCH_CHECK();
    return CV_OK;
}

int cv_hv_forward_f32(const float* d_points, const float* d_xyz, const float* d_scale,
                      const float* d_obj, int64_t n, float res, int num_rots,
                      const float h_corner3[3], const int dims[3], float* d_grid_obj,
                      float* d_grid_rot, float* d_grid_scale, void* d_ws, size_t ws_bytes, int algo,
                      void* stream) {
    CV_REQUIRE(algo_ok(algo), CV_EINVAL, "algo out of range (%d: 0 auto, 1 direct, 2 tiles)", algo);
    int rc = check_common(d_points, d_xyz, d_scale, n, res, num_rots, h_corner3, dims);
    if (rc) return rc;
    CV_REQUIRE(d_obj && d_grid_obj && d_grid_rot && d_grid_scale, CV_EINVAL, "null pointer argument");
    return hv_forward_cats(d_points, d_xyz, d_scale, d_obj, n, res, num_rots, h_corner3, dims, d_grid_obj, d_grid_rot, d_grid_scale,
                           d_ws, ws_bytes, algo, 1, static_cast<hipStream_t>(stream));
}

int cv_hv_forward_cat_f32(const float* d_points, const float* d_xyz, const float* d_scale, const float* d_obj, int64_t n,
                          float res, int num_rots, const float h_corner3[3], const int dims[3], int num_cats, float* d_grid_obj,
                          float* d_grid_rot, float* d_grid_scale, void* d_ws, size_t ws_bytes, int algo, void* stream) {
    CV_REQUIRE(num_cats >= 1 && num_cats <= CV_MAX_CATEGORIES, CV_EINVAL, "num_cats out of range (%d, 1..%d)", num_cats,
               CV_MAX_CATEGORIES);
    CV_REQUIRE(algo_ok(algo), CV_EINVAL, "algo out of range (%d: 0 auto, 1 direct, 2 tiles)", algo);
    int rc = check_common(d_points, d_xyz, d_scale, n, res, num_rots, h_corner3, dims);
    if (rc) return rc;
    CV_REQUIRE(d_obj && d_grid_obj && d_grid_rot && d_grid_scale, CV_EINVAL, "null pointer argument");
    return hv_forward_cats(d_points, d_xyz, d_scale, d_obj, n, res, num_rots, h_corner3, dims, d_grid_obj, d_grid_rot, d_grid_scale,
                           d_ws, ws_bytes, algo, num_cats, static_cast<hipStream_t>(stream));
}

int cv_hv_backward_f32(const float* d_grad_obj, const float* d_points, const float* d_xyz,
                       const float* d_scale, const float* d_obj, int64_t n, float res, int num_rots,
                       const float h_corner3[3], const int dims[3], float* d_dxyz, float* d_dscale,
                       float* d_dobj, void* stream) {
    int rc = check_common(d_points, d_xyz, d_scale, n, res, num_rots, h_corner3, dims);
    if (rc) return rc;
    CV_REQUIRE(d_grad_obj && d_obj && d_dxyz && d_dscale && d_dobj, CV_EINVAL, "null pointer argument");
    hipStream_t st = static_cast<hipStream_t>(stream);
    const float2* tab = nullptr;
    rc = get_rot_table(num_rots, &tab);
    if (rc) return rc;
    const F3 corner{h_corner3[0], h_corner3[1], h_corner3[2]};
    const I3 d3{dims[0], dims[1], dims[2]};
    hv_bwd<<<(unsigned)((n + 3) / 4), 256, 0, st>>>(d_grad_obj, d_points, d_xyz, d_scale, d_obj, n,
                                                   num_rots, res, corner, d3, tab, d_dxyz, d_dscale,
                                                   d_dobj);
    CV_LAUNCH_CHECK();
    return CV_OK;
}

int cv_hv_count_votes_f32(const float* d_points, const float* d_xyz, const float* d_scale, int64_t n,
                          float res, int num_rots, const float h_corner3[3], const int dims[3],
                          int64_t* h_count, void* d_ws, size_t ws_bytes, void* stream) {
    int rc = check_common(d_points, d_xyz, d_scale, n, res, num_rots, h_corner3, dims);
    if (rc) return rc;
    CV_REQUIRE(h_count && d_ws && ws_bytes >= 256, CV_ENOMEM, "workspace too small");
    hipStream_t st = static_cast<hipStream_t>(stream);
    const float2* tab = nullptr;
    rc = get_rot_table(num_rots, &tab);
    if (rc) return rc;
    unsigned long long* cnt = static_cast<unsigned long long*>(d_ws);
    CV_HIP_CHECK(hipMemsetAsync(cnt, 0, sizeof(*cnt), st));
    const F3 corner{h_corner3[0], h_corner3[1], h_corner3[2]};
    const I3 d3{dims[0], dims[1], dims[2]};
    const int64_t total = n * num_rots;
    hv_count_votes<<<(unsigned)std::min<int64_t>((total + 255) / 256, 2048), 256, 0, st>>>(
        d_points, d_xyz, d_scale, n, num_rots, res, corner, d3, tab, cnt);
    CV_LAUNCH_CHECK();
    unsigned long long h = 0;
    CV_HIP_CHECK(hipMemcpyAsync(&h, cnt, sizeof h, hipMemcpyDeviceToHost, st));
    CV_HIP_CHECK(hipStreamSynchronize(st));
    *h_count = (int64_t)h;
    return CV_OK;
}

}
```

canonicalvoting_amd/csrc/scene_exec.cpp:

```cpp
#include <algorithm>
#include <atomic>
#include <chrono>
#include <cstdlib>
#include <cstring>
#include <vector>

#include "cv_common.h"

namespace {

struct Carver {
    char* base; size_t off = 0, cap;
    Carver(void* p, size_t c) : base(static_cast<char*>(p)), cap(c) {}
    template <typename T> T* take(size_t count) {
        off = cv_align_up(off, 256);
        T* r = (base && off + count * sizeof(T) <= cap) ? reinterpret_cast<T*>(base + off) : nullptr;
        off += count * sizeof(T);
        return r;
    }
};

std::atomic<int> g_scenes_inside{0};
struct SceneCount {
    int before;
// ... 11 lines not shown
        g_scenes_inside.fetch_sub(1, std::memory_order_relaxed);
    }
};

struct StageClock {
    void* const* events; hipStream_t st; float* host_us;
    std::chrono::steady_clock::time_point t_prev = std::chrono::steady_clock::now();
    hipError_t mark(int i) const { return events[i] ? hipEventRecord(static_cast<hipEvent_t>(events[i]), st) : hipSuccess; }
    void lap(int i) {
        const auto t = std::chrono::steady_clock::now();
        host_us[i] += std::chrono::duration<float, std::micro>(t - t_prev).count();
        t_prev = t;
    }
};

struct SceneFront {
    const int32_t* d_coords4; long long n; const float* d_points; float res;
    int stem_k, mask_groups; long long masked_min_rows; int max_channels;
    float* h_minmax;
    cv_scene_plan_layout lay;
    void* mm_ws; int32_t* ibuf; unsigned long long* kbuf; char* sort_ws; char* lev_ws;
    cv_scene_maps off;
    long long rows[5];
    float mn[3]; int dims[3]; size_t cells;
    const int32_t* maps[CV_NET_MAP_SLOTS]; const int32_t* perms[CV_NET_PERM_SLOTS];
    size_t conv_ws_b;

    template <class D> explicit SceneFront(const D* d)
        : d_coords4(d->d_coords4), n(d->n), d_points(d->d_points), res(d->res), stem_k(d->stem_k), mask_groups(d->mask_groups),
          masked_min_rows(d->masked_min_rows), max_channels(d->max_channels), h_minmax(static_cast<float*>(d->h_pinned)) {}

    bool carve(Carver& cv) {
        mm_ws = cv.take<char>(cv_hv_minmax_workspace_bytes());
        cv_sp_scene_plan_layout(n, stem_k, mask_groups, masked_min_rows, &lay);
        ibuf = cv.take<int32_t>((size_t)lay.int_words);
        kbuf = cv.take<unsigned long long>((size_t)lay.key_words);
        sort_ws = cv.take<char>(lay.sort_ws_bytes);
        lev_ws = cv.take<char>(lay.levels_ws_bytes);
        return mm_ws && ibuf && kbuf && sort_ws && lev_ws;
    }

    template <class R> int run(int32_t* d_zero_word, R* r, StageClock& clock, void* stream) {
        int rc = cv_hv_minmax_async_ex(d_points, n, h_minmax, mm_ws, cv_hv_minmax_workspace_bytes(), d_zero_word,
                                       reinterpret_cast<int32_t*>(sort_ws), stream);
        if (rc != CV_OK) return rc;
        int32_t *c_coords[5], *c_vals[5];
        unsigned long long* c_keys[5];
        for (int i = 0; i < 5; ++i) {
            c_coords[i] = ibuf + lay.coords[i];
            c_keys[i] = kbuf + (size_t)lay.cap * i;
            c_vals[i] = ibuf + lay.vals[i];
        }
        int32_t counts_h[8] = {0};
        rc = cv_sp_scene_plan_ex(d_coords4, n, ibuf + lay.perm, ibuf + lay.inv, c_coords, c_keys, c_vals, lay.cap, ibuf + lay.counts,
                                 counts_h, stem_k, mask_groups, masked_min_rows, ibuf + lay.arena, (size_t)(lay.int_words - lay.arena),
                                 &off, sort_ws, lay.sort_ws_bytes, lev_ws, lay.levels_ws_bytes,
                                  true, stream,  true);
        if (rc != CV_OK) return rc;
        r->duplicates = counts_h[5];
        r->out_of_window = counts_h[6];
        CV_REQUIRE(counts_h[5] == 0 && counts_h[6] == 0, CV_EINVAL,
                   "duplicate coordinates (%d) or coordinates outside the 16-bit key window (%d)", counts_h[5], counts_h[6]);
        clock.lap(0);
        for (int i = 0; i < 5; ++i) { rows[i] = counts_h[i]; r->level_rows[i] = counts_h[i]; }
        float mx[3];
        for (int k = 0; k < 3; ++k) { mn[k] = h_minmax[k]; mx[k] = h_minmax[3 + k]; r->corner[k] = mn[k]; }
        rc = cv_hv_grid_dims_f32(mn, mx, res, dims);
        if (rc != CV_OK) return rc;
        for (int k = 0; k < 3; ++k) r->dims[k] = dims[k];
        cells = (size_t)dims[0] * dims[1] * dims[2];
        int masked[5];
        for (int i = 0; i < 5; ++i) masked[i] = off.mask_perm[i] >= 0;
        conv_ws_b = cv_sp_scene_conv_workspace_bytes(rows, masked, mask_groups, max_channels);
        return cv_sp_scene_plan_slots(&lay, &off, rows, masked_min_rows, ibuf, maps, perms);
    }
};

template <class R> int fixed_part_too_small(R* r, size_t fixed_end) {
    r->needed_ws_bytes = fixed_end * 2 + ((size_t)256 << 20);
    cv_set_error("scene workspace too small (needs at least %zu bytes)", r->needed_ws_bytes);
    return CV_ENOMEM;
}

}

extern "C" {

int cv_detect_scene_f32(const cv_scene_desc* d, cv_scene_result* r, void* stream) {
    CV_REQUIRE(d && r, CV_EINVAL, "null scene descriptor / result");
    CV_REQUIRE(d->d_coords4 && d->d_feats && d->d_points && d->n > 0 && d->ops && d->bufs && d->n_ops > 0 && d->n_bufs > 0,
               CV_EINVAL, "bad scene descriptor");
    CV_REQUIRE(d->d_out_feats && d->out_ld >= d->out_channels && d->out_channels > 0, CV_EINVAL, "bad network output buffer");
    CV_REQUIRE(d->h_pinned && d->pinned_bytes >= 256 && d->d_ws, CV_EINVAL, "pinned scratch (>= 256 bytes) and a device workspace are required");
    CV_REQUIRE(d->h_boxes && d->h_scores && d->h_classes && d->h_cand_idx && d->h_verdict && d->h_pick && d->max_candidates > 0,
               CV_EINVAL, "null result arrays");
    hipStream_t st = static_cast<hipStream_t>(stream);
    const long long n = d->n;
    std::memset(r, 0, sizeof(*r));
    CV_REQUIRE(d->conv_split_target >= 0 && d->vote_part_records >= 0, CV_EINVAL, "negative launch sizing");
    CV_REQUIRE(d->vote_algo >= 0 && d->vote_algo <= 2, CV_EINVAL, "vote_algo out of range (%d: 0 auto, 1 direct, 2 tiles)", d->vote_algo);
    SceneCount in_flight(d->adaptive_split != 0, d->conv_split_target, d->vote_part_records);
    r->scenes_in_flight = in_flight.before + 1;
    Carver cv(d->d_ws, d->ws_bytes);
    StageClock clock{d->events, st, r->host_us};
    CV_HIP_CHECK(clock.mark(0));

    SceneFront f(d);
    int32_t* h_flag = reinterpret_cast<int32_t*>(static_cast<char*>(d->h_pinned) + 64);
    const bool plan_fits = f.carve(cv);
    float* xyz = cv.take<float>((size_t)n * 3);
    float* scale = cv.take<float>((size_t)n * 3);
    float* prob = cv.take<float>((size_t)n);
    int32_t* cls = cv.take<int32_t>((size_t)n);
    int32_t* d_flag = cv.take<int32_t>(64);
    if (!plan_fits || !xyz || !scale || !prob || !cls || !d_flag) return fixed_part_too_small(r, cv.off);
    int rc = f.run(d_flag, r, clock, stream);
    if (rc != CV_OK) return rc;
    const size_t cells = f.cells;

    const size_t arena_b = cv_net_arena_bytes(d->bufs, d->n_bufs, f.rows, 5);
    const size_t vote_ws_b = cv_hv_forward_workspace_bytes(n, d->num_rots, f.dims, d->vote_algo);
    const size_t dec_ws_b = cv_decode_workspace_bytes(f.dims, n, d->max_candidates);
    char* arena = cv.take<char>(arena_b);
    char* conv_ws = cv.take<char>(f.conv_ws_b);
    char* vote_ws = cv.take<char>(std::max<size_t>(vote_ws_b, 256));
    char* dec_ws = cv.take<char>(dec_ws_b);
    float* grids = d->d_grids ? d->d_grids : cv.take<float>(6 * cells);
    r->needed_ws_bytes = cv.off + 4096;
    r->needed_grid_floats = 6 * cells;
    CV_REQUIRE(arena && conv_ws && vote_ws && dec_ws && grids, CV_ENOMEM, "scene workspace too small (needs %zu bytes)", r->needed_ws_bytes);
    CV_REQUIRE(!d->d_grids || d->grid_capacity_floats >= 6 * cells, CV_ENOMEM, "grid buffer too small (needs %zu floats)", 6 * cells);
    float* g_obj = grids;
    float* g_rot = grids + cells;
    float* g_scale = grids + 3 * cells;
    r->d_grid_obj = g_obj; r->d_grid_rot = g_rot; r->d_grid_scale = g_scale;

    const void* ext_ptr[2] = {d->d_feats, d->d_out_feats};
    const int ext_ld[2] = {d->feats_ld, d->out_ld};
    rc = cv_net_run_f32(d->ops, d->n_ops, d->bufs, d->n_bufs, f.rows, 5, arena, arena_b, ext_ptr, ext_ld, f.maps, CV_NET_MAP_SLOTS,
                        f.perms, CV_NET_PERM_SLOTS, conv_ws, f.conv_ws_b, d->use_range_flag ? d_flag : nullptr, stream);
    if (rc != CV_OK) return rc;
    clock.lap(1);
    CV_HIP_CHECK(clock.mark(1));
    rc = cv_head_joint_f32(d->d_out_feats, n, d->out_ld, d->nclasses, d->log_scale, xyz, scale, prob, cls, stream);
    if (rc != CV_OK) return rc;
    if (d->use_range_flag) CV_HIP_CHECK(hipMemcpyAsync(h_flag, d_flag, sizeof(int32_t), hipMemcpyDeviceToHost, st));
    r->d_xyz = xyz; r->d_scale = scale; r->d_prob = prob; r->d_class = cls;
    CV_HIP_CHECK(clock.mark(2));

    const float* v_xyz = d->d_xyz_in ? d->d_xyz_in : xyz;
    const float* v_scale = d->d_scale_in ? d->d_scale_in : scale;
    const float* v_prob = d->d_prob_in ? d->d_prob_in : prob;
    const int32_t* v_cls = d->d_class_in ? d->d_class_in : cls;
    rc = cv_hv_forward_f32(d->d_points, v_xyz, v_scale, v_prob, n, d->res, d->num_rots, f.mn, f.dims, g_obj, g_rot, g_scale, vote_ws,
                           std::max<size_t>(vote_ws_b, 256), d->vote_algo, stream);
    if (rc != CV_OK) return rc;
    CV_HIP_CHECK(clock.mark(3));
    clock.lap(2);
    cv_decode_params prm = d->decode;
    prm.max_iters = d->max_candidates;
    int n_cand = 0, n_boxes = 0, truncated = 0;
    const DecodeCall dc{g_obj, g_rot, g_scale, f.dims, f.mn, d->res, d->d_points, v_xyz, v_prob, v_cls, n, &prm, 0, dec_ws, dec_ws_b, &n_cand,
                        d->h_cand_idx, d->h_verdict, &n_boxes, d->h_boxes, d->h_scores, d->h_classes, &truncated, stream, d->events[4]};
    rc = cv_decode_run(dc, 1, true);
    if (rc != CV_OK) return rc;
    r->n_cand = n_cand;
    r->n_boxes = n_boxes;
    r->truncated = truncated;
    r->range_flag = d->use_range_flag ? *h_flag : 0;

    int n_det = 0;
    std::vector<float> bc, sc;
    std::vector<int32_t> idx, pick;
    for (int c = 0; c < d->nclasses; ++c) {
        bc.clear(); sc.clear(); idx.clear();
        for (int i = 0; i < n_boxes; ++i)
            if (d->h_classes[i] == c) {
                bc.insert(bc.end(), d->h_boxes + (size_t)i * 24, d->h_boxes + (size_t)i * 24 + 24);
                sc.push_back(d->h_scores[i]);
                idx.push_back(i);
            }
        if (idx.empty()) continue;
        pick.assign(idx.size(), 0);
        const int k = cv_nms_obb(bc.data(), sc.data(), (int)idx.size(), d->nms_threshold, pick.data());
        if (k < 0) return k;
        for (int j = 0; j < k; ++j) d->h_pick[n_det++] = idx[(size_t)pick[j]];
    }
    r->n_det = n_det;
    clock.lap(3);
    return CV_OK;
}

int cv_detect_scene_separate_f32(const cv_scene_separate_desc* d, cv_scene_separate_result* r, void* stream) {
    CV_REQUIRE(d && r, CV_EINVAL, "null scene descriptor / result");
    std::memset(r, 0, sizeof(*r));
    const int K = d->num_models;
    CV_REQUIRE(K >= 1 && K <= CV_MAX_CATEGORIES, CV_EINVAL, "num_models out of range (%d, 1..%d)", K, CV_MAX_CATEGORIES);
    CV_REQUIRE(d->d_coords4 && d->d_feats && d->d_points && d->n > 0 && d->ops && d->n_ops && d->bufs && d->n_bufs && d->d_out_feats,
               CV_EINVAL, "bad scene descriptor");
    for (int k = 0; k < K; ++k)
        CV_REQUIRE(d->ops[k] && d->bufs[k] && d->n_ops[k] > 0 && d->n_bufs[k] > 0 && d->d_out_feats[k], CV_EINVAL,
                   "bad program or output buffer of model %d", k);
    CV_REQUIRE(d->out_ld >= d->out_channels && d->out_channels >= 8, CV_EINVAL, "bad network output buffer");
    CV_REQUIRE(d->h_pinned && d->pinned_bytes >= 64 + 64 * (size_t)K && d->d_ws, CV_EINVAL,
               "pinned scratch (>= 64 + 64 K bytes) and a device workspace are required");
    CV_REQUIRE(d->h_boxes && d->h_scores && d->h_cand_idx && d->h_verdict && d->h_det_cat && d->h_det_box && d->max_candidates > 0,
               CV_EINVAL, "null result arrays");
    CV_REQUIRE(!!d->d_xyz_in == !!d->d_scale_in && !!d->d_xyz_in == !!d->d_prob_in, CV_EINVAL, "predictions: all three or none");
    CV_REQUIRE(d->conv_split_target >= 0 && d->vote_part_records >= 0, CV_EINVAL, "negative launch sizing");
    CV_REQUIRE(d->vote_algo >= 0 && d->vote_algo <= 2, CV_EINVAL, "vote_algo out of range (%d: 0 auto, 1 direct, 2 tiles)", d->vote_algo);
    CV_REQUIRE(d->models_per_pass >= 0, CV_EINVAL, "negative models_per_pass (%d)", d->models_per_pass);
    const int G = std::min(d->models_per_pass, K);
    if (G > 0) {
        CV_REQUIRE(d->d_model_params, CV_EINVAL, "models_per_pass needs d_model_params (cv_net_models_params_fill)");
        for (int k = 1; k < K; ++k)
            CV_REQUIRE(d->n_ops[k] == d->n_ops[0] && d->n_bufs[k] == d->n_bufs[0], CV_EINVAL,
                       "models_per_pass: the program of model %d has another length than model 0's", k);
    }
    hipStream_t st = static_cast<hipStream_t>(stream);
    const long long n = d->n;
    SceneCount in_flight(false, d->conv_split_target, d->vote_part_records);
    Carver cv(d->d_ws, d->ws_bytes);
    StageClock clock{d->events, st, r->host_us};
    CV_HIP_CHECK(clock.mark(0));

    SceneFront f(d);
    int32_t* h_flags = reinterpret_cast<int32_t*>(static_cast<char*>(d->h_pinned) + 64);
    const bool plan_fits = f.carve(cv);
    float* xyz = cv.take<float>((size_t)K * n * 3);
    float* scale = cv.take<float>((size_t)K * n * 3);
    float* prob = cv.take<float>((size_t)K * n);
    int32_t* d_flags = cv.take<int32_t>(16 * (size_t)K);
    if (!plan_fits || !xyz || !scale || !prob || !d_flags) return fixed_part_too_small(r, cv.off);
    if (d->use_range_flag) CV_HIP_CHECK(hipMemsetAsync(d_flags, 0, sizeof(int32_t) * 16 * K, st));
    int rc = f.run(nullptr, r, clock, stream);
    if (rc != CV_OK) return rc;
    const size_t cells = f.cells;

    size_t arena_b = 0;
    for (int k = 0; k < K; ++k) arena_b = std::max(arena_b, cv_net_arena_bytes(d->bufs[k], d->n_bufs[k], f.rows, 5));
    const size_t vote_ws_b = cv_hv_forward_cat_workspace_bytes(n, d->num_rots, f.dims, d->vote_algo, K);
    const size_t dec_ws_b = cv_decode_cat_workspace_bytes(f.dims, n, d->max_candidates, K);
    const size_t arena_all = G > 0 ? (size_t)G * arena_b : arena_b;
    const size_t conv_ws_all = G > 0 ? cv_net_models_workspace_bytes(f.conv_ws_b, G) : f.conv_ws_b;
    char* arena = cv.take<char>(arena_all);
    char* conv_ws = cv.take<char>(conv_ws_all);
    char* vote_ws = cv.take<char>(std::max<size_t>(vote_ws_b, 256));
    char* dec_ws = cv.take<char>(dec_ws_b);
    float* grids = cv.take<float>(6 * cells * (size_t)K);
    r->needed_ws_bytes = cv.off + 4096;
    CV_REQUIRE(arena && conv_ws && vote_ws && dec_ws && grids, CV_ENOMEM, "scene workspace too small (needs %zu bytes)", r->needed_ws_bytes);
    float* g_obj = grids;
    float* g_rot = grids + cells * K;
    float* g_scale = grids + 3 * cells * K;
    r->d_grid_obj = g_obj; r->d_grid_rot = g_rot; r->d_grid_scale = g_scale;

    for (int m0 = 0; G > 0 && m0 < K; m0 += G) {
        const int g = std::min(G, K - m0);
        const void* ext_ptr[CV_MAX_CATEGORIES][2];
        const void* const* ext_tab[CV_MAX_CATEGORIES];
        for (int m = 0; m < g; ++m) {
            ext_ptr[m][0] = d->d_feats, ext_ptr[m][1] = d->d_out_feats[m0 + m];
            ext_tab[m] = ext_ptr[m];
        }
        const int ext_ld[2] = {d->feats_ld, d->out_ld};
        rc = cv_net_run_models_f32(d->ops + m0, d->bufs + m0, d->n_ops[0], d->n_bufs[0], g, f.rows, 5, arena, arena_all, ext_tab, ext_ld,
                                   f.maps, CV_NET_MAP_SLOTS, f.perms, CV_NET_PERM_SLOTS, conv_ws, conv_ws_all,
                                   d->use_range_flag ? d_flags + 16 * m0 : nullptr,
                                   static_cast<const cv_net_model_params*>(d->d_model_params) + m0, K, stream);
        if (rc != CV_OK) return rc;
    }
    for (int k = 0; G == 0 && k < K; ++k) {
        const void* ext_ptr[2] = {d->d_feats, d->d_out_feats[k]};
        const int ext_ld[2] = {d->feats_ld, d->out_ld};
        rc = cv_net_run_f32(d->ops[k], d->n_ops[k], d->bufs[k], d->n_bufs[k], f.rows, 5, arena, arena_b, ext_ptr, ext_ld, f.maps,
                            CV_NET_MAP_SLOTS, f.perms, CV_NET_PERM_SLOTS, conv_ws, f.conv_ws_b,
                            d->use_range_flag ? d_flags + 16 * k : nullptr, stream);
        if (rc != CV_OK) return rc;
    }
    clock.lap(1);
    CV_HIP_CHECK(clock.mark(1));
    if (G > 0) {
        rc = cv_head_separate_models_f32(d->d_out_feats, K, n, d->out_ld, d->log_scale, xyz, scale, prob, stream);
        if (rc != CV_OK) return rc;
    }
    for (int k = 0; G == 0 && k < K; ++k) {
        rc = cv_head_separate_f32(d->d_out_feats[k], n, d->out_ld, d->log_scale, xyz + (size_t)k * n * 3, scale + (size_t)k * n * 3,
                                  prob + (size_t)k * n, stream);
        if (rc != CV_OK) return rc;
    }
    if (d->use_range_flag) CV_HIP_CHECK(hipMemcpyAsync(h_flags, d_flags, sizeof(int32_t) * 16 * K, hipMemcpyDeviceToHost, st));
    r->d_xyz = xyz; r->d_scale = scale; r->d_prob = prob;
    CV_HIP_CHECK(clock.mark(2));

    const float* v_xyz = d->d_xyz_in ? d->d_xyz_in : xyz;
    const float* v_scale = d->d_xyz_in ? d->d_scale_in : scale;
    const float* v_prob = d->d_xyz_in ? d->d_prob_in : prob;
    rc = cv_hv_forward_cat_f32(d->d_points, v_xyz, v_scale, v_prob, n, d->res, d->num_rots, f.mn, f.dims, K, g_obj, g_rot, g_scale, vote_ws,
                               std::max<size_t>(vote_ws_b, 256), d->vote_algo, stream);
    if (rc != CV_OK) return rc;
    CV_HIP_CHECK(clock.mark(3));
    clock.lap(2);
    cv_decode_params prm = d->decode;
    prm.max_iters = d->max_candidates;
    const int M = d->max_candidates;
    std::vector<int32_t> classes((size_t)K * M);
    const DecodeCall dc{g_obj, g_rot, g_scale, f.dims, f.mn, d->res, d->d_points, v_xyz, v_prob, nullptr, n, &prm, 0, dec_ws, dec_ws_b,
                        r->n_cand, d->h_cand_idx, d->h_verdict, r->n_boxes, d->h_boxes, d->h_scores, classes.data(), r->truncated, stream,
// ... 172 lines not shown
```

canonicalvoting_amd/pipeline.py:

```python
import collections
import contextlib
import ctypes
import os

import torch

from . import _lib, decode, hv_cuda
from . import me as ME

vp = ctypes.c_void_p


class ScenePolicy(collections.namedtuple("ScenePolicy", "conv_split_target vote_part_records masked_min_rows")):
    __slots__ = ()

    def as_config(self):
        return {"conv_split_target": self.conv_split_target, "vote_part_records": self.vote_part_records,
                "masked_min_rows": self.masked_min_rows}


def policy_for_scenes_in_flight(n):
    lib_rows = ME.CoordinateManager.LIB_MASKED_MIN_ROWS
    if int(n) >= 4:
        return ScenePolicy(256, 12288, min(8192, lib_rows))
# ... 218 lines not shown
                                               c_ext, ext_ld, c_maps, len(map_ptrs), c_perms, len(perm_ptrs), vp(ws.data_ptr()),
                                               ws.numel(), flag, vp(table.data_ptr() + entry * k0), K,
                                               vp(torch.cuda.current_stream(dev).cuda_stream)), "cv_net_run_models_f32")
    return ys


def detect_scene_separate_c(models, hv, coords4, feats, res, predictions=None, policy=None, keep=None, events=None,
                            log_scale=True, overlap_threshold=0.3, max_candidates=512, scan_points=None,
                            models_per_pass=None, **decode_kw):
    import numpy as np
    decode_kw.setdefault("separate_variant", True)
    decode_kw.setdefault("err_thresh", float(np.float32(0.3)))
    L = _lib.lib()
    dev = feats.device
    n = coords4.shape[0]
    categories = list(models.keys())
    mods = [models[c] for c in categories]
    K = len(mods)
    if not 1 <= K <= _lib.MAX_CATEGORIES:
        raise ValueError("detect_scene_separate_c: 1..%d models (got %d)" % (_lib.MAX_CATEGORIES, K))
    if scan_points is None:
        scan_points = (coords4[:, 1:].to(dev) * res).float().contiguous()
    pieces = 1 if ME.COMPUTE_DTYPE == "bf16" else mods[0].PIECES
    G = int(models_per_pass or 0)
    if G < 0:
        raise ValueError("detect_scene_separate_c: models_per_pass must be >= 0 (got %d)" % G)
    if G > 0:
        progs, table = model_params_table(mods, dev, pieces)
    else:
        progs, table = [m._program(dev, pieces) for m in mods], None
    coords4 = coords4.to(device=dev, dtype=torch.int32).contiguous()
    feats = feats.contiguous()
    ys = [torch.empty((n, m.final.out_channels), dtype=torch.float32, device=dev) for m in mods]
    M = int(max_candidates)
    host = _sep_host(dev, K, M)
    d = _lib.SceneSeparateDesc()
    _fill_scene_desc(d, mods[0], hv, coords4, feats, scan_points, res, policy, pieces, max(max(m.PLANES) for m in mods), log_scale)
    if predictions is not None:
        px, ps, pp = [a.contiguous() for a in predictions]
        d.d_xyz_in, d.d_scale_in, d.d_prob_in = vp(px.data_ptr()), vp(ps.data_ptr()), vp(pp.data_ptr())
    alive = _fill_separate_desc(d, host, progs, table, G, ys, decode_kw, overlap_threshold, events)
    r = _lib.SceneSeparateResult()
    ws = _call_growing(L.cv_detect_scene_separate_f32, "cv_detect_scene_separate_f32", d, r, dev, "scene_call_separate",
                       host["ws_hint"])
    del alive
    host["ws_hint"] = max(host["ws_hint"], int(r.needed_ws_bytes))
    if keep is not None:
        keep.update(range_flag=int(r.range_flag), needed_ws_bytes=int(r.needed_ws_bytes))
    if r.range_flag or any(r.truncated[k] for k in range(K)):
        kw = dict(decode_kw, max_candidates=M)
        if predictions is None:
            return detect_scene_separate(models, hv, coords4, feats, res, log_scale=log_scale,
                                         overlap_threshold=overlap_threshold, **kw)
        return _separate_by_calls(hv, scan_points, predictions[0], predictions[1], predictions[2], res, categories,
                                  overlap_threshold, **kw)
    return _separate_results(host, r, keep, categories, ys, n, dev, ws)


def _sep_host(dev, K, M):
    import numpy as np
    key = (dev.index, torch.cuda.current_stream(dev).cuda_stream)
    with _scene_lock:
        host = _sep_hosts.get(key)
        if host is None or host["M"] < M or host["K"] < K:
            host = _sep_hosts[key] = dict(
                M=M, K=K, ws_hint=0, pinned=torch.empty(64 + 64 * _lib.MAX_CATEGORIES, dtype=torch.uint8).pin_memory(),
                cand=np.zeros((K, M), np.int64), verdict=np.zeros((K, M), np.int32), boxes=np.zeros((K, M, 8, 3), np.float32),
                scores=np.zeros((K, M), np.float32), det_cat=np.zeros(K * M, np.int32), det_box=np.zeros(K * M, np.int32))
    return host


def _fill_separate_desc(d, host, progs, table, G, ys, decode_kw, overlap_threshold, events):
    K = len(progs)
    d.num_models = K
    if G > 0:
        d.models_per_pass, d.d_model_params = G, vp(table.data_ptr())
    ops = (vp * K)(*[ctypes.cast(p[0], vp) for p in progs])
    n_ops = (ctypes.c_int * K)(*[len(p[0]) for p in progs])
    bufs = (vp * K)(*[ctypes.cast(p[1], vp) for p in progs])
    n_bufs = (ctypes.c_int * K)(*[len(p[1]) for p in progs])
    outs = (vp * K)(*[y.data_ptr() for y in ys])
    d.ops, d.n_ops, d.bufs, d.n_bufs = ctypes.cast(ops, vp), ctypes.cast(n_ops, vp), ctypes.cast(bufs, vp), ctypes.cast(n_bufs, vp)
    d.d_out_feats, d.out_ld, d.out_channels = ctypes.cast(outs, vp), ys[0].stride(0), ys[0].shape[1]
    _fill_decode_params(d.decode, decode_kw, True)
    d.max_candidates, d.nms_threshold = host["M"], float(overlap_threshold)
    _set_events(d, events)
    d.h_pinned, d.pinned_bytes = vp(host["pinned"].data_ptr()), host["pinned"].numel()
    d.h_cand_idx, d.h_verdict = vp(host["cand"].ctypes.data), vp(host["verdict"].ctypes.data)
    d.h_boxes, d.h_scores = vp(host["boxes"].ctypes.data), vp(host["scores"].ctypes.data)
    d.h_det_cat, d.h_det_box = vp(host["det_cat"].ctypes.data), vp(host["det_box"].ctypes.data)
    return ops, n_ops, bufs, n_bufs, outs


def _separate_results(host, r, keep, categories, ys, n, dev, ws):
    K = len(categories)
    dets = [(categories[int(c)], host["boxes"][int(c), int(b)].copy(), float(host["scores"][int(c), int(b)]))
            for c, b in zip(host["det_cat"][:r.n_det], host["det_box"][:r.n_det])]
    if keep is not None:
        X, Y, Z = r.dims
        view = lambda ptr, shape: _device_view(ptr, shape, torch.float32, dev, ws)
        raw = [dict(boxes=host["boxes"][k, :r.n_boxes[k]].copy(), scores=host["scores"][k, :r.n_boxes[k]].copy(),
                    cand_idx=host["cand"][k, :r.n_cand[k]].copy(), verdict=host["verdict"][k, :r.n_cand[k]].copy())
               for k in range(K)]
        keep.update(y=ys, dims=(X, Y, Z), corner=tuple(r.corner), level_rows=list(r.level_rows), raw=raw,
                    grids=(view(r.d_grid_obj, (K, X, Y, Z)), view(r.d_grid_rot, (K, X, Y, Z, 2)),
                           view(r.d_grid_scale, (K, X, Y, Z, 3))),
                    net_pred=(view(r.d_xyz, (K, n, 3)), view(r.d_scale, (K, n, 3)), view(r.d_prob, (K, n))),
                    host_us=tuple(r.host_us))
    return dets


class _SceneHost:

    def __init__(self, max_candidates):
        import numpy as np
        self.M = max_candidates
        self.pinned = torch.empty(256, dtype=torch.uint8).pin_memory()
        self.cand = np.zeros(max_candidates, np.int64)
        self.verdict = np.zeros(max_candidates, np.int32)
        self.boxes = np.zeros((max_candidates, 8, 3), np.float32)
        self.scores = np.zeros(max_candidates, np.float32)
        self.classes = np.zeros(max_candidates, np.int32)
        self.pick = np.zeros(max_candidates, np.int32)
        self.ws_hint = 0
        self.last_host_us = (0.0, 0.0, 0.0, 0.0)


_scene_hosts = {}
_scene_lock = __import__("threading").Lock()


def detect_scene_c(model, hv, coords4, feats, res, nclasses=9, log_scale=True, scan_points=None, predictions=None,
                   max_candidates=512, keep=None, events=None, adaptive_split=False, policy=None, **decode_kw):
    import numpy as np
    L = _lib.lib()
    dev = feats.device
    n = coords4.shape[0]
    if scan_points is None:
        scan_points = (coords4[:, 1:].to(dev) * res).float().contiguous()
    pieces = 1 if ME.COMPUTE_DTYPE == "bf16" else model.PIECES
    c_ops, c_bufs, _ = model._program(dev, pieces)
    coords4 = coords4.to(device=dev, dtype=torch.int32).contiguous()
    feats = feats.contiguous()
    y = torch.empty((n, model.final.out_channels), dtype=torch.float32, device=dev)
    host = _scene_host(dev, max_candidates)
    d = _lib.SceneDesc()
    _fill_scene_desc(d, model, hv, coords4, feats, scan_points, res, policy, pieces, max(model.PLANES), log_scale)
    if predictions is not None:
        px, ps, pp, pc = predictions
        pc = pc.to(torch.int32).contiguous()
        d.d_xyz_in, d.d_scale_in, d.d_prob_in, d.d_class_in = (vp(px.data_ptr()), vp(ps.data_ptr()), vp(pp.data_ptr()),
                                                                 vp(pc.data_ptr()))
    _fill_joint_desc(d, host, c_ops, c_bufs, y, nclasses, decode_kw, adaptive_split, events)
    r = _lib.SceneResult()
    ws = _call_growing(L.cv_detect_scene_f32, "cv_detect_scene_f32", d, r, dev, "scene_call", host.ws_hint)
    host.ws_hint = max(host.ws_hint, int(r.needed_ws_bytes))
    host.last_host_us = tuple(r.host_us)
    if r.range_flag or r.truncated:
        if r.range_flag:
            model.range_fallbacks = getattr(model, "range_fallbacks", 0) + 1
        with torch.no_grad(), scene_policy(policy):
            x = ME.SparseTensor(feats, coords4, device=dev)
            yy = model.program_forward(x, pieces=3) if r.range_flag else x._like(y, 1)
            pred = head_joint(yy.F, nclasses, log_scale) if predictions is None else predictions
            dets, raw = decode.detect(hv, coords4[:, 1:], pred[0], pred[1], pred[2], pred[3], res, nclasses,
                                      scan_points=scan_points, **decode_kw)
        return dets, raw, yy.F
    dets, raw = _joint_results(host, r, keep, y, n, dev, ws)
    return dets, raw, y


def _scene_host(dev, max_candidates):
    key = (dev.index, torch.cuda.current_stream(dev).cuda_stream)
    with _scene_lock:
        host = _scene_hosts.get(key)
        if host is None or host.M < max_candidates:
            host = _scene_hosts[key] = _SceneHost(max_candidates)
    return host


def _fill_joint_desc(d, host, c_ops, c_bufs, y, nclasses, decode_kw, adaptive_split, events):
    d.ops, d.n_ops, d.bufs, d.n_bufs = ctypes.cast(c_ops, vp), len(c_ops), ctypes.cast(c_bufs, vp), len(c_bufs)
    d.d_out_feats, d.out_ld, d.out_channels = vp(y.data_ptr()), y.stride(0), y.shape[1]
    d.nclasses = nclasses
    _fill_decode_params(d.decode, decode_kw, False)
    d.max_candidates, d.nms_threshold = host.M, 0.3
    d.adaptive_split = 1 if adaptive_split else 0
    _set_events(d, events)
    d.h_pinned, d.pinned_bytes = vp(host.pinned.data_ptr()), host.pinned.numel()
    d.h_cand_idx, d.h_verdict = vp(host.cand.ctypes.data), vp(host.verdict.ctypes.data)
    d.h_boxes, d.h_scores, d.h_classes, d.h_pick = (vp(host.boxes.ctypes.data), vp(host.scores.ctypes.data),
                                                    vp(host.classes.ctypes.data), vp(host.pick.ctypes.data))


def _joint_results(host, r, keep, y, n, dev, ws):
    k, m = r.n_boxes, r.n_cand
    raw = dict(boxes=host.boxes[:k].copy(), scores=host.scores[:k].copy(), classes=host.classes[:k].copy(),
               cand_idx=host.cand[:m].copy(), verdict=host.verdict[:m].copy(), truncated=False)
    dets = [(int(raw["classes"][i]), raw["boxes"][i], float(raw["scores"][i])) for i in host.pick[:r.n_det]]
    if keep is not None:
        view = lambda ptr, shape, dt=torch.float32: _device_view(ptr, shape, dt, dev, ws)
        X, Y, Z = r.dims
        keep.update(y=y, dims=(X, Y, Z), corner=tuple(r.corner), level_rows=list(r.level_rows),
                    grids=(view(r.d_grid_obj, (X, Y, Z)), view(r.d_grid_rot, (X, Y, Z, 2)), view(r.d_grid_scale, (X, Y, Z, 3))),
                    net_pred=(view(r.d_xyz, (n, 3)), view(r.d_scale, (n, 3)), view(r.d_prob, (n,)),
                              view(r.d_class, (n,), torch.int32)), raw=raw)
    return dets, raw


def detect_points(model, hv, points, feats, res, predictions=None, return_inverse=False, **kw):
    coords4, index, inverse = ME.utils.quantize_device(points, res, None, return_inverse)
    gi = index.long()
    dev = coords4.device
    f = feats.to(dev)[gi]
    if predictions is not None:
        predictions = tuple(p.to(dev)[gi].contiguous() for p in predictions)
    out = detect_scene_c(model, hv, coords4, f, res, predictions=predictions, **kw)
    return out + ((index, inverse) if return_inverse else (index,))


def _points_front(front, points, feats, in_channels, recentre_from, predictions, return_inverse, with_class):
    dev = points.device
    assert points.is_cuda and points.dim() == 2 and points.shape[1] == 3, "points: a [M, 3] device tensor"
    if points.dtype not in (torch.float32, torch.float64):
        points = points.to(torch.float64)
    if points.stride(1) != 1 or points.stride(0) < 3:
        points = points.contiguous()
    m = points.shape[0]
    if m == 0:
        raise RuntimeError("sparse_quantize: empty point cloud")
    feats = feats.to(device=dev, dtype=torch.float32)
    if feats.stride(1) != 1 or feats.stride(0) < feats.shape[1]:
        feats = feats.contiguous()
    if feats.shape != (m, in_channels):
        raise ValueError("raw cloud: feats must be [%d, %d] (got %s)" % (m, in_channels, tuple(feats.shape)))
    coords4 = torch.empty((m, 4), dtype=torch.int32, device=dev)
    index = torch.empty(m, dtype=torch.int32, device=dev)
    inverse = torch.empty(m, dtype=torch.int32, device=dev) if return_inverse else None
    front.d_raw_points, front.m, front.points_ld = vp(points.data_ptr()), m, points.stride(0)
    front.points_f64 = 1 if points.dtype == torch.float64 else 0
    front.d_raw_feats, front.raw_feats_ld, front.in_channels = vp(feats.data_ptr()), feats.stride(0), in_channels
    front.recentre_from = -1 if recentre_from is None else int(recentre_from)
    front.d_coords4, front.d_index = vp(coords4.data_ptr()), vp(index.data_ptr())
    front.d_inverse = vp(inverse.data_ptr()) if return_inverse else None
    alive = [points, feats]
    if predictions is not None:
        pred = [p.to(dev).contiguous() for p in predictions]
        if with_class:
            pred[3] = pred[3].to(torch.int32).contiguous()
            front.d_raw_class = vp(pred[3].data_ptr())
        front.d_raw_xyz, front.d_raw_scale, front.d_raw_prob = vp(pred[0].data_ptr()), vp(pred[1].data_ptr()), vp(pred[2].data_ptr())
        alive += pred
    return coords4, index, inverse, alive


def _call_points(fn, name, d, r, dev, scratch_name, ws_hint):
    call = lambda _d, _r, stream: fn(ctypes.byref(d), ctypes.byref(r), stream)
    try:
        return _call_growing(call, name, d.scene, r.scene, dev, scratch_name, ws_hint)
    except _lib.CvError:
        if r.rejected:
            raise RuntimeError("sparse_quantize: %d points rejected (a non-finite component, or a voxel outside the supported "
                               "window: spatial coordinates in [-32704, 32703])" % r.rejected) from None
        raise


def detect_points_c(model, hv, points, feats, res, predictions=None, return_inverse=False, recentre_from=None, nclasses=9,
                    log_scale=True, max_candidates=512, keep=None, events=None, adaptive_split=False, policy=None, **decode_kw):
    L = _lib.lib()
    dev = points.device
    pieces = 1 if ME.COMPUTE_DTYPE == "bf16" else model.PIECES
    c_ops, c_bufs, _ = model._program(dev, pieces)
    d, r = _lib.PointsDesc(), _lib.PointsResult()
    coords4, index, inverse, alive = _points_front(d.front, points, feats, feats.shape[1], recentre_from, predictions,
                                                   return_inverse, True)
    d.front.quantization_size = float(res)
    y = torch.empty((coords4.shape[0], model.final.out_channels), dtype=torch.float32, device=dev)
    host = _scene_host(dev, max_candidates)
    _fill_scene_desc(d.scene, model, hv, None, None, None, res, policy, pieces, max(model.PLANES), log_scale)
    _fill_joint_desc(d.scene, host, c_ops, c_bufs, y, nclasses, decode_kw, adaptive_split, events)
    ws = _call_points(L.cv_detect_points_f32, "cv_detect_points_f32", d, r, dev, "scene_call", host.ws_hint)
    del alive
    n = int(r.n)
    host.ws_hint = max(host.ws_hint, int(r.scene.needed_ws_bytes))
    host.last_host_us = tuple(r.scene.host_us)
    coords4, index, y = coords4[:n], index[:n], y[:n]
    tail = (index, inverse) if return_inverse else (index,)
    view = lambda ptr, shape, dt=torch.float32: _device_view(ptr, shape, dt, dev, ws)
    if r.scene.range_flag or r.scene.truncated:
        pred = None
        if predictions is not None:
            pred = (view(r.d_xyz_in, (n, 3)), view(r.d_scale_in, (n, 3)), view(r.d_prob_in, (n,)), view(r.d_class_in, (n,), torch.int32))
        return detect_scene_c(model, hv, coords4, view(r.d_feats, (n, d.front.in_channels)), res, nclasses=nclasses,
                              log_scale=log_scale, predictions=pred, max_candidates=max_candidates, keep=keep, events=events,
                              adaptive_split=adaptive_split, policy=policy, **decode_kw) + tail
    if keep is not None:
        keep.update(scan_points=view(r.d_points, (n, 3)), feats=view(r.d_feats, (n, d.front.in_channels)),
                    host_us=tuple(r.scene.host_us), host_us_front=float(r.host_us_front), front_ws_bytes=int(r.front_ws_bytes))
    dets, raw = _joint_results(host, r.scene, keep, y, n, dev, ws)
    return (dets, raw, y) + tail


def detect_points_separate_c(models, hv, points, feats, res, predictions=None, models_per_pass=None, return_inverse=False,
                             recentre_from=None, policy=None, keep=None, events=None, log_scale=True, overlap_threshold=0.3,
                             max_candidates=512, **decode_kw):
    import numpy as np
    decode_kw.setdefault("separate_variant", True)
    decode_kw.setdefault("err_thresh", float(np.float32(0.3)))
    L = _lib.lib()
    dev = points.device
    categories = list(models.keys())
    mods = [models[c] for c in categories]
    K = len(mods)
    if not 1 <= K <= _lib.MAX_CATEGORIES:
        raise ValueError("detect_points_separate_c: 1..%d models (got %d)" % (_lib.MAX_CATEGORIES, K))
    pieces = 1 if ME.COMPUTE_DTYPE == "bf16" else mods[0].PIECES
    G = int(models_per_pass or 0)
    if G < 0:
        raise ValueError("detect_points_separate_c: models_per_pass must be >= 0 (got %d)" % G)
    if G > 0:
        progs, table = model_params_table(mods, dev, pieces)
    else:
        progs, table = [m._program(dev, pieces) for m in mods], None
    d, r = _lib.PointsSeparateDesc(), _lib.PointsSeparateResult()
    coords4, index, inverse, alive = _points_front(d.front, points, feats, feats.shape[1], recentre_from, predictions,
                                                   return_inverse, False)
    d.front.quantization_size = float(res)
    m = coords4.shape[0]
    ys = [torch.empty((m, mod.final.out_channels), dtype=torch.float32, device=dev) for mod in mods]
    M = int(max_candidates)
    host = _sep_host(dev, K, M)
    _fill_scene_desc(d.scene, mods[0], hv, None, None, None, res, policy, pieces, max(max(mod.PLANES) for mod in mods), log_scale)
    alive.append(_fill_separate_desc(d.scene, host, progs, table, G, ys, decode_kw, overlap_threshold, events))
    ws = _call_points(L.cv_detect_points_separate_f32, "cv_detect_points_separate_f32", d, r, dev, "scene_call_separate",
                      host["ws_hint"])
    del alive
    n = int(r.n)
    host["ws_hint"] = max(host["ws_hint"], int(r.scene.needed_ws_bytes))
    coords4, index, ys = coords4[:n], index[:n], [y[:n] for y in ys]
    tail = (index, inverse) if return_inverse else (index,)
    if keep is not None:
        keep.update(range_flag=int(r.scene.range_flag), needed_ws_bytes=int(r.scene.needed_ws_bytes), coords4=coords4)
    if r.scene.range_flag or any(r.scene.truncated[k] for k in range(K)):
        view = lambda ptr, shape: _device_view(ptr, shape, torch.float32, dev, ws)
        pred = None
        if predictions is not None:
            pred = (view(r.d_xyz_in, (K, n, 3)), view(r.d_scale_in, (K, n, 3)), view(r.d_prob_in, (K, n)))
        return (detect_scene_separate_c(models, hv, coords4, view(r.d_feats, (n, d.front.in_channels)), res, predictions=pred,
                                        policy=policy, keep=keep, events=events, log_scale=log_scale,
                                        overlap_threshold=overlap_threshold, max_candidates=M, models_per_pass=models_per_pass,
                                        **decode_kw),) + tail
    return (_separate_results(host, r.scene, keep, categories, ys, n, dev, ws),) + tail


def last_scene_host_us(dev=None):
    dev = torch.device("cuda", torch.cuda.current_device()) if dev is None else dev
    host = _scene_hosts.get((dev.index, torch.cuda.current_stream(dev).cuda_stream))
    return host.last_host_us if host is not None else None


def _device_view(ptr, shape, dtype, dev, owner):
    import numpy as np
    count = int(np.prod(shape))
    off = int(ptr) - owner.data_ptr()
    nbytes = count * torch.empty((), dtype=dtype).element_size()
    assert 0 <= off and off + nbytes <= owner.numel()
    return owner[off:off + nbytes].view(dtype).view(*shape).clone()
```

include/cv_hip.h:

```cpp
#ifndef CV_HIP_H
#define CV_HIP_H

#include <stddef.h>
#include <stdint.h>

#ifdef __cplusplus
extern "C" {
#endif

#define CV_OK 0
#define CV_EINVAL (-22)
#define CV_ENOMEM (-12)
#define CV_EHIP (-5)
#define CV_ERANGE (-34)

#define CV_ABI_VERSION 6
int cv_abi_version(void);
const char* cv_last_error(void);


size_t cv_hv_minmax_workspace_bytes(void);
int cv_hv_minmax_f32(const float* d_points, int64_t n, float* h_min3, float* h_max3,
                     void* d_ws, size_t ws_bytes, void* stream);
int cv_hv_minmax_async_f32(const float* d_points, int64_t n, float* h_minmax6, void* d_ws, size_t ws_bytes,
                           void* stream);

int cv_hv_grid_dims_f32(const float h_min3[3], const float h_max3[3], float res, int dims_out[3]);

size_t cv_hv_forward_workspace_bytes(int64_t n, int num_rots, const int dims[3], int algo);

int cv_hv_forward_f32(const float* d_points, const float* d_xyz, const float* d_scale,
                      const float* d_obj, int64_t n, float res, int num_rots,
                      const float h_corner3[3], const int dims[3], float* d_grid_obj,
                      float* d_grid_rot, float* d_grid_scale, void* d_ws, size_t ws_bytes,
                      int algo, void* stream);

#define CV_MAX_CATEGORIES 16
size_t cv_hv_forward_cat_workspace_bytes(int64_t n, int num_rots, const int dims[3], int algo, int num_cats);
int cv_hv_forward_cat_f32(const float* d_points, const float* d_xyz, const float* d_scale, const float* d_obj, int64_t n,
                          float res, int num_rots, const float h_corner3[3], const int dims[3], int num_cats, float* d_grid_obj,
                          float* d_grid_rot, float* d_grid_scale, void* d_ws, size_t ws_bytes, int algo, void* stream);

int cv_hv_set_part_records(int records);
int cv_hv_set_part_records_thread(int records);
int cv_hv_set_kernel_events(void* ev_start, void* ev_stop);

int cv_hv_backward_f32(const float* d_grad_obj, const float* d_points, const float* d_xyz,
                       const float* d_scale, const float* d_obj, int64_t n, float res,
                       int num_rots, const float h_corner3[3], const int dims[3], float* d_dxyz,
                       float* d_dscale, float* d_dobj, void* stream);

int cv_hv_count_votes_f32(const float* d_points, const float* d_xyz, const float* d_scale, int64_t n,
                          float res, int num_rots, const float h_corner3[3], const int dims[3],
                          int64_t* h_count, void* d_ws, size_t ws_bytes, void* stream);

typedef struct cv_decode_params {
    float thresh_high;
    float thresh_low;
    float valid_ratio;
    int elimination;
    float prob_thresh;
    int elim_hi_plus1;
    int max_iters;
    double err_thresh;
} cv_decode_params;

size_t cv_decode_workspace_bytes(const int dims[3], int64_t n, int max_iters);

int cv_decode_f32(float* d_grid_obj, const float* d_grid_rot, const float* d_grid_scale,
                  const int dims[3], const float h_corner3[3], float res, const float* d_points,
                  const float* d_xyz, const float* d_prob, const int32_t* d_class, int64_t n,
                  const cv_decode_params* params, int mutate_grid, void* d_ws, size_t ws_bytes,
                  int* h_n_cand, int64_t* h_cand_idx, int32_t* h_verdict, int* h_n_boxes,
                  float* h_boxes, float* h_scores, int32_t* h_classes, int* h_truncated, void* stream);

size_t cv_decode_cat_workspace_bytes(const int dims[3], int64_t n, int max_iters, int num_cats);
int cv_decode_cat_f32(float* d_grid_obj, const float* d_grid_rot, const float* d_grid_scale, const int dims[3],
                      const float h_corner3[3], float res, const float* d_points, const float* d_xyz, const float* d_prob,
                      const int32_t* d_class, int64_t n, int num_cats, const cv_decode_params* params, int mutate_grid, void* d_ws,
                      size_t ws_bytes, int* h_n_cand, int64_t* h_cand_idx, int32_t* h_verdict, int* h_n_boxes, float* h_boxes,
                      float* h_scores, int32_t* h_classes, int* h_truncated, void* stream);

double cv_iou_obb(const float* h_box1, const float* h_box2);
int cv_nms_obb(const float* h_boxes, const float* h_scores, int n, double thr, int32_t* h_pick);


long long cv_sp_table_capacity(long long n);
size_t cv_sp_levels_workspace_bytes(long long n);

int cv_sp_build_levels(int32_t* const* d_coords, unsigned long long* const* d_keys,
                       int32_t* const* d_vals, long long n, long long cap, int num_levels,
                       int32_t* d_counts, int32_t* h_counts, void* d_ws, size_t ws_bytes, void* stream);

#define CV_QUANTIZE_MAX_CLOUDS 256
size_t cv_sp_quantize_workspace_bytes(long long m);
int cv_sp_quantize_f32(const float* d_points, long long m, long long ld, float quantization_size, int floor_only,
                       const long long* h_offsets, int n_clouds, int32_t* d_coords4, int32_t* d_index, int32_t* d_inverse,
                       int32_t* d_counts, int32_t* h_counts, void* d_ws, size_t ws_bytes, void* stream);
int cv_sp_quantize_f64(const double* d_points, long long m, long long ld, double quantization_size, int floor_only,
                       const long long* h_offsets, int n_clouds, int32_t* d_coords4, int32_t* d_index, int32_t* d_inverse,
                       int32_t* d_counts, int32_t* h_counts, void* d_ws, size_t ws_bytes, void* stream);

#define CV_GATHER_MAX_JOBS 8
typedef struct cv_gather_job {
    const void* d_src; long long src_ld;
    void* d_dst; long long dst_ld;
    int width;
    int recentre_from;
} cv_gather_job;
int cv_sp_voxel_rows_f32(const int32_t* d_coords4, const int32_t* d_index, long long n, float res, float* d_points_out,
                         const cv_gather_job* jobs, int n_jobs, void* stream);

size_t cv_sp_sort_workspace_bytes(long long n);
int cv_sp_sort_rows(const int32_t* d_coords, long long n, int32_t* d_sorted, int32_t* d_perm, int32_t* d_inv,
                    void* d_ws, size_t ws_bytes, void* stream);

int cv_sp_morton_keys(const int32_t* d_coords, long long n, long long* d_keys, void* stream);

int cv_sp_kernel_map(const int32_t* d_out_coords, long long n_out, const unsigned long long* d_keys,
                     const int32_t* d_vals, long long cap, int k, int ts, int32_t* d_nbr, void* stream);

int cv_sp_up_map(const int32_t* d_nbr_down, long long n_coarse, long long n_fine, int32_t* d_up,
                 void* stream);

typedef struct cv_conv_desc {
    const float* in;
    long long n_in;
    int in_ld, cin;
    const float* weight;
    int K, cout;
    const int32_t* nbr;
    long long n_out;
    const float* scale;
    const float* shift;
    const float* residual;
    int res_ld;
    int relu;
    float* out;
    int out_ld;
    int flavour;
    void* ws;
    size_t ws_bytes;
    const int32_t* row_perm;
    int j_begin, j_end;
    const float* acc_in;
    int acc_ld;
    int perm_groups;
    const int32_t* plan_ent;
    const int32_t* plan_cnt;
    const float* weight_packed;
    const void* weight_x6;
    const float* in2;
    int in2_ld, cin2;
    const void* weight2_x6;
    int perm_has_map;
    int weight_pieces;
    float acc_scale;
    int32_t* range_flag;
    int in_hl, out_hl, res_hl;
    int32_t* split_tickets;
    const float* acc_scale_dev;
} cv_conv_desc;
#define CV_SPLIT_TICKETS 4096

int cv_sp_to_hl_f32(const float* d_x, long long n, int c, int x_ld, float* d_y, int y_ld, int32_t* range_flag, void* stream);
int cv_sp_from_hl_f32(const float* d_x, long long n, int c, int x_ld, float* d_y, int y_ld, void* stream);

int cv_sp_pack_weights_x6_f32(const float* d_w, int K, int cin, int cout, const float* d_col_scale, void* d_wp6,
                              void* stream);
int cv_sp_pack_weights_h2_f32(const float* d_w, int K, int cin, int cout, const float* d_col_scale, int scale_log2,
                              void* d_wp, void* stream);
typedef struct cv_pack_job {
    const float* w;
    void* wp;
    int K, cin, cout;
    int trans;
    int scale_log2;
    int reserved;
} cv_pack_job;
int cv_sp_pack_weights_h2_batch_f32(const cv_pack_job* h_jobs, int n_jobs, void* d_jobs, void* stream);
int cv_sp_pack_weights_bf16_f32(const float* d_w, int K, int cin, int cout, const float* d_col_scale, void* d_wp,
                                void* stream);
int cv_sp_pack_weights_t_f32(const float* d_w, int K, int rows, int cols, int pieces, int scale_log2, void* d_wp, void* stream);
int cv_sp_pack_weights_stem_h2_f32(const float* d_w, int K, int cin, const float* d_col_scale, int scale_log2, void* d_wp,
                                   void* stream);

size_t cv_sp_conv_workspace_bytes(long long n_out, int cout, int K);
int cv_sp_conv_f32(const cv_conv_desc* desc, void* stream);

int cv_sp_set_split_target(int workgroups);
int cv_sp_set_split_target_thread(int workgroups);
int cv_sp_set_ablation(int bits);
int cv_sp_set_option(const char* name, long long value, long long* previous);
int cv_sp_get_option(const char* name, long long* value);
// ... 8 lines not shown
                     long long cap, const long long* level_rows, const int32_t* d_perm, long long n_orig, int stem_k,
                     int mask_groups, long long masked_min_rows, int32_t* d_arena, size_t arena_words, void* stream);

size_t cv_sp_scene_plan_words(long long n, int stem_k, int mask_groups, long long masked_min_rows);
int cv_sp_scene_plan(const int32_t* d_input, long long n, int32_t* d_perm, int32_t* d_inv, int32_t* const* d_coords,
                     unsigned long long* const* d_keys, int32_t* const* d_vals, long long cap, int32_t* d_counts,
                     int32_t* h_counts, int stem_k, int mask_groups, long long masked_min_rows, int32_t* d_arena,
                     size_t arena_words, cv_scene_maps* offsets, void* d_sort_ws, size_t sort_ws_bytes, void* d_levels_ws,
                     size_t levels_ws_bytes, void* stream);

typedef struct cv_scene_plan_layout {
    long long cap;
    long long perm, inv, coords[5], vals[5], counts, arena;
    long long int_words, key_words;
    size_t sort_ws_bytes, levels_ws_bytes;
} cv_scene_plan_layout;
int cv_sp_scene_plan_layout(long long n, int stem_k, int mask_groups, long long masked_min_rows, cv_scene_plan_layout* out);
#define CV_NET_MAP_SLOTS 15
#define CV_NET_PERM_SLOTS 9
int cv_sp_scene_plan_slots(const cv_scene_plan_layout* layout, const cv_scene_maps* offsets, const long long* level_rows,
                           long long min_rows, const int32_t* d_ibuf, const int32_t** maps, const int32_t** perms);
size_t cv_sp_scene_conv_workspace_bytes(const long long* level_rows, const int* masked, int mask_groups, int max_channels);

typedef struct cv_net_buf {
    int level, channels, rows_level;
    int hl;
} cv_net_buf;
typedef struct cv_net_op {
    int in_buf, in_col, cin;
    int out_buf, out_col, cout;
    int res_buf, res_col;
    int map, K;
    int perm, perm_groups;
    int relu;
    const float* weight;
    const float* scale;
    const float* shift;
    const void* weight_x6;
    int in2_buf, in2_col, cin2;
    const void* weight2_x6;
    int weight_pieces;
    float acc_scale;
} cv_net_op;
size_t cv_net_arena_bytes(const cv_net_buf* bufs, int n_bufs, const long long* level_rows, int n_levels);
int cv_net_run_f32(const cv_net_op* ops, int n_ops, const cv_net_buf* bufs, int n_bufs, const long long* level_rows,
                   int n_levels, void* d_arena, size_t arena_bytes, const void* const* ext_ptr, const int* ext_ld,
                   const int32_t* const* maps, int n_maps, const int32_t* const* perms, int n_perms,
                   void* d_ws, size_t ws_bytes, int32_t* range_flag, void* stream);

typedef struct cv_net_model_params {
    const void* weight_x6;
    const void* weight2_x6;
    const float* scale;
    const float* shift;
    float acc_scale;
    int reserved[3];
} cv_net_model_params;
size_t cv_net_models_params_bytes(int n_ops, int K);
int cv_net_models_params_fill(const cv_net_op* const* ops, int n_ops, int K, void* h_params, size_t params_bytes);
size_t cv_net_models_arena_bytes(const cv_net_buf* bufs, int n_bufs, const long long* level_rows, int n_levels, int K);
size_t cv_net_models_workspace_bytes(size_t one_model_bytes, int K);
int cv_net_run_models_f32(const cv_net_op* const* ops, const cv_net_buf* const* bufs, int n_ops, int n_bufs, int K,
                          const long long* level_rows, int n_levels, void* d_arena, size_t arena_bytes,
                          const void* const* const* ext_ptr, const int* ext_ld, const int32_t* const* maps, int n_maps,
                          const int32_t* const* perms, int n_perms, void* d_ws, size_t ws_bytes, int32_t* range_flag,
                          const void* d_params, int params_ld, void* stream);

int cv_sp_mask_keys(const int32_t* d_nbr, long long n, int K, int j_begin, int j_end, long long* d_keys,
                    void* stream);

int cv_sp_mask_perms(const int32_t* d_nbr, long long n, int K, int groups, int32_t* d_perm, void* d_ws,
                     size_t ws_bytes, int with_map, void* stream);

int cv_sp_transpose_map(const int32_t* d_nbr, long long n_out, int K, long long n_in, int32_t* d_nbr_t, void* stream);
size_t cv_sp_wgrad_workspace_bytes(long long n_out, int cin, int cout, int K);
int cv_sp_conv_wgrad_f32(const float* d_x, int x_ld, int cin, const float* d_dy, int dy_ld, int cout,
                         const int32_t* d_nbr, int K, long long n_out, float* d_dw, void* d_ws, size_t ws_bytes,
                         void* stream);
int cv_sp_conv_wgrad_px_f32(const float* d_x, int x_ld, int cin, const float* d_dy, int dy_ld, int cout,
                            const int32_t* d_nbr, int K, long long n_out, float* d_dw, void* d_ws, size_t ws_bytes,
                            int pieces, void* stream);
int cv_sp_col_sum_f32(const float* d_x, long long n, int c, int ld, float* d_out, void* stream);
size_t cv_sp_col_sum_workspace_bytes(long long n, int c);
int cv_sp_col_sum_det_f32(const float* d_x, long long n, int c, int ld, float* d_out, void* d_ws, size_t ws_bytes,
                          void* stream);

size_t cv_sp_bn_workspace_bytes(int c);
int cv_sp_bn_stats_f32(const float* d_x, long long n, int c, int ld, const float* d_gamma, const float* d_beta,
                       float eps, float momentum, float* d_running_mean, float* d_running_var, float* d_mean,
                       float* d_var, float* d_scale, float* d_shift, void* d_ws, size_t ws_bytes, void* stream);
int cv_sp_bn_backward_f32(const float* d_x, const float* d_dy, const float* d_y, long long n, int c, int ld,
                          const float* d_mean, const float* d_var, float eps, const float* d_gamma, float* d_dgamma,
                          float* d_dbeta, float* d_dx, float* d_dres, void* d_ws, size_t ws_bytes, void* stream);

#define CV_BN_SLOT_WORDS 8200
int cv_sp_bn_backward_hl_f32(const float* d_x, const float* d_dy, const float* d_y, long long n, int c, int ld,
                             const float* d_mean, const float* d_var, float eps, const float* d_gamma, float* d_dgamma,
                             float* d_dbeta, float* d_dx, float* d_dres, void* d_ws, size_t ws_bytes, float* d_dx_hl,
                             uint32_t* d_slot, int32_t* range_flag, const uint32_t* d_relu_bits, void* stream);

int cv_sp_copy_unless_flag(const void* const* h_src, void* const* h_dst, const long long* h_bytes, int n, const int32_t* flag,
                           void* stream);

int cv_sp_affine_f32(const float* d_x, long long n, int c, int x_ld, const float* d_scale,
                     const float* d_shift, const float* d_residual, int res_ld, int relu, float* d_y, int y_ld,
                     void* stream);
int cv_sp_affine_hl_f32(const float* d_x, long long n, int c, int x_ld, const float* d_scale, const float* d_shift,
                        const float* d_residual, int res_ld, int relu, float* d_y, int y_ld, float* d_y_hl, int y_hl_ld,
                        uint32_t* d_relu_bits, int32_t* range_flag, void* stream);

int cv_sp_bn_fold_f32(const float* d_gamma, const float* d_beta, const float* d_mean, const float* d_var,
                      const float* d_bias, float eps, int c, float* d_scale, float* d_shift, void* stream);

int cv_head_joint_f32(const float* d_feats, long long n, int ld, int nclasses, int log_scale, float* d_xyz,
                      float* d_scale, float* d_prob, int32_t* d_class, void* stream);

int cv_head_separate_f32(const float* d_feats, long long n, int ld, int log_scale, float* d_xyz, float* d_scale,
                         float* d_prob, void* stream);
int cv_head_separate_models_f32(const float* const* d_feats, int K, long long n, int ld, int log_scale, float* d_xyz,
                                float* d_scale, float* d_prob, void* stream);

typedef struct cv_scene_desc {
    const int32_t* d_coords4;
    long long n;
    const float* d_feats;
    int feats_ld;
    const float* d_points;
    float res;
    int num_rots;
    const cv_net_op* ops; int n_ops;
    const cv_net_buf* bufs; int n_bufs;
    int stem_k, mask_groups;
    long long masked_min_rows;
    int max_channels;
    int use_range_flag;
    float* d_out_feats;
    int out_ld, out_channels;
    int nclasses, log_scale;
    const float* d_xyz_in; const float* d_scale_in; const float* d_prob_in; const int32_t* d_class_in;
    int vote_algo;
    cv_decode_params decode;
    int max_candidates;
    double nms_threshold;
    void* d_ws; size_t ws_bytes;
    float* d_grids; size_t grid_capacity_floats;
    void* h_pinned; size_t pinned_bytes;
    int64_t* h_cand_idx; int32_t* h_verdict;
    float* h_boxes; float* h_scores; int32_t* h_classes;
    int32_t* h_pick;
    int adaptive_split;
    void* events[5];
    int conv_split_target;
    int vote_part_records;
} cv_scene_desc;
typedef struct cv_scene_result {
    int n_cand, n_boxes, n_det, truncated, range_flag, duplicates, out_of_window;
    int scenes_in_flight;
    int dims[3];
    float corner[3];
    long long level_rows[5];
    size_t needed_ws_bytes, needed_grid_floats;
    float* d_grid_obj; float* d_grid_rot; float* d_grid_scale;
    float* d_xyz; float* d_scale; float* d_prob; int32_t* d_class;
    float host_us[4];
} cv_scene_result;
int cv_detect_scene_f32(const cv_scene_desc* desc, cv_scene_result* result, void* stream);

typedef struct cv_scene_separate_desc {
    const int32_t* d_coords4; long long n;
    const float* d_feats; int feats_ld;
    const float* d_points; float res; int num_rots;
    int num_models;
    const cv_net_op* const* ops; const int* n_ops;
    const cv_net_buf* const* bufs; const int* n_bufs;
    int stem_k, mask_groups;
    long long masked_min_rows;
    int max_channels;
    int use_range_flag;
    float* const* d_out_feats;
    int out_ld, out_channels;
    int log_scale;
    const float* d_xyz_in; const float* d_scale_in; const float* d_prob_in;
    int vote_algo;
    cv_decode_params decode;
    int max_candidates;
    double nms_threshold;
    void* d_ws; size_t ws_bytes;
    void* h_pinned; size_t pinned_bytes;
    int64_t* h_cand_idx; int32_t* h_verdict;
    float* h_boxes; float* h_scores;
    int32_t* h_det_cat; int32_t* h_det_box;
    void* events[5];
    int conv_split_target, vote_part_records;
    int models_per_pass;
    const void* d_model_params;
} cv_scene_separate_desc;
typedef struct cv_scene_separate_result {
    int n_cand[CV_MAX_CATEGORIES], n_boxes[CV_MAX_CATEGORIES], truncated[CV_MAX_CATEGORIES];
    int n_det, range_flag, duplicates, out_of_window;
    int dims[3];
    float corner[3];
    long long level_rows[5];
    size_t needed_ws_bytes;
    float* d_grid_obj; float* d_grid_rot; float* d_grid_scale;
    float* d_xyz; float* d_scale; float* d_prob;
    float host_us[4];
} cv_scene_separate_result;
int cv_detect_scene_separate_f32(const cv_scene_separate_desc* desc, cv_scene_separate_result* result, void* stream);

typedef struct cv_points_front {
    const void* d_raw_points; long long m, points_ld; int points_f64;
    double quantization_size;
    const float* d_raw_feats; long long raw_feats_ld; int in_channels;
    int recentre_from;
    const float* d_raw_xyz; const float* d_raw_scale; const float* d_raw_prob; const int32_t* d_raw_class;
    int32_t* d_coords4; int32_t* d_index; int32_t* d_inverse;
} cv_points_front;
typedef struct cv_points_desc { cv_points_front front; cv_scene_desc scene; } cv_points_desc;
typedef struct cv_points_separate_desc { cv_points_front front; cv_scene_separate_desc scene; } cv_points_separate_desc;
typedef struct cv_points_result {
    cv_scene_result scene;
    long long n;
    int rejected;
    float host_us_front;
    size_t front_ws_bytes;
    float* d_feats; float* d_points; float* d_xyz_in; float* d_scale_in; float* d_prob_in; int32_t* d_class_in;
} cv_points_result;
typedef struct cv_points_separate_result {
    cv_scene_separate_result scene;
    long long n; int rejected; float host_us_front; size_t front_ws_bytes;
    float* d_feats; float* d_points; float* d_xyz_in; float* d_scale_in; float* d_prob_in;
} cv_points_separate_result;
int cv_detect_points_f32(const cv_points_desc* desc, cv_points_result* result, void* stream);
int cv_detect_points_separate_f32(const cv_points_separate_desc* desc, cv_points_separate_result* result, void* stream);
size_t cv_sizeof_gather_job(void);
size_t cv_sizeof_points_desc(void);
size_t cv_sizeof_points_separate_desc(void);
size_t cv_sizeof_points_result(void);
size_t cv_sizeof_points_separate_result(void);

#ifdef __cplusplus
}
#endif
#endif
```

Baseline: 638.6.

## Split Hough voting into objectness pass then rot/scale pass on hot boxes only

Voting now runs in two passes. The first pass accumulates only objectness and records, for each (plane, tile), a bounding box of cells at or above the decode high threshold. The second pass accumulates rotation and scale quotients only inside those hot boxes, which cuts LDS atomics, record loads and grid writes for the cold regions. It costs an extra vote pass over the records, and rot/scale outside the hot boxes are no longer computed, so downstream code may only read them at peaks.

```diff
diff --git a/canonicalvoting_amd/_lib.py b/canonicalvoting_amd/_lib.py
--- a/canonicalvoting_amd/_lib.py
+++ b/canonicalvoting_amd/_lib.py
@@ -85,7 +85,7 @@
                 ("grid_capacity_floats", ctypes.c_size_t), ("h_pinned", vp), ("pinned_bytes", ctypes.c_size_t),
                 ("h_cand_idx", vp), ("h_verdict", vp), ("h_boxes", vp), ("h_scores", vp), ("h_classes", vp), ("h_pick", vp),
                 ("adaptive_split", ctypes.c_int), ("events", vp * 5),
-                ("conv_split_target", ctypes.c_int), ("vote_part_records", ctypes.c_int)]
+                ("conv_split_target", ctypes.c_int), ("vote_part_records", ctypes.c_int), ("peak_quotients", ctypes.c_int)]
 
 
 MAX_CATEGORIES = 16
@@ -178,6 +178,12 @@
     "cv_hv_forward_cat_workspace_bytes": (ctypes.c_size_t, [ctypes.c_int64, ctypes.c_int, c_int_p, ctypes.c_int, ctypes.c_int]),
     "cv_hv_forward_cat_f32": (ctypes.c_int, [vp, vp, vp, vp, ctypes.c_int64, ctypes.c_float, ctypes.c_int, c_float_p, c_int_p,
                                              ctypes.c_int, vp, vp, vp, vp, ctypes.c_size_t, ctypes.c_int, vp]),
+    "cv_hv_forward_peaks_f32": (ctypes.c_int, [vp, vp, vp, vp, ctypes.c_int64, ctypes.c_float, ctypes.c_int,
+                                               c_float_p, c_int_p, vp, vp, vp, vp, ctypes.c_size_t,
+                                               ctypes.c_int, ctypes.c_float, vp]),
+    "cv_hv_forward_peaks_cat_f32": (ctypes.c_int, [vp, vp, vp, vp, ctypes.c_int64, ctypes.c_float, ctypes.c_int, c_float_p, c_int_p,
+                                                   ctypes.c_int, vp, vp, vp, vp, ctypes.c_size_t, ctypes.c_int, ctypes.c_float,
+                                                   vp]),
     "cv_hv_set_kernel_events": (ctypes.c_int, [vp, vp]),
     "cv_hv_backward_f32": (ctypes.c_int, [vp, vp, vp, vp, vp, ctypes.c_int64, ctypes.c_float,
                                           ctypes.c_int, c_float_p, c_int_p, vp, vp, vp, vp]),
diff --git a/canonicalvoting_amd/csrc/hv_vote.hip b/canonicalvoting_amd/csrc/hv_vote.hip
--- a/canonicalvoting_amd/csrc/hv_vote.hip
+++ b/canonicalvoting_amd/csrc/hv_vote.hip
@@ -519,12 +519,18 @@
     __hip_atomic_fetch_add(p, q, __ATOMIC_RELAXED, __HIP_MEMORY_SCOPE_WORKGROUP);
 }
 
-constexpr int ACC_PITCH = TZ + 8, ACC_CH = TX * ACC_PITCH + 4, ACC_WORDS = 6 * ACC_CH;
+constexpr int ACC_PITCH = TZ + 8, ACC_CH = TX * ACC_PITCH + 4;
 __device__ __forceinline__ int acc_idx(int ch, int cell) { return ch * ACC_CH + (cell >> 5) * ACC_PITCH + (cell & 31); }
 
-struct TileShared {
+constexpr int VOTE_FULL = 0, VOTE_OBJ = 1, VOTE_PEAKS = 2;
+constexpr int vote_channels(int mode) { return mode == VOTE_FULL ? 6 : (mode == VOTE_OBJ ? 1 : 5); }
+struct HotBox { int x0, x1, z0, z1; };
+
+template <int MODE>
+struct TileSharedT {
+    static constexpr int ACC_WORDS = vote_channels(MODE) * ACC_CH;
     unsigned long long acc[ACC_WORDS];
-    float pq[9][LQ];
+    float pq[MODE == VOTE_OBJ ? 6 : 9][LQ];
     int arc_start[LQ];
     int arc_cum[LQ];
     uint32_t vq_rec[TW][VQ];
@@ -537,28 +543,35 @@
     int more;
 };
 
-template <bool SMALL>
-__device__ __forceinline__ void drain_vote(TileShared& sh, int lx, int lz, float rx, float rz, float wy, float ob,
-                                           float s0, float s1, float s2, float2 cs) {
+template <bool SMALL, int MODE>
+__device__ __forceinline__ void drain_vote(TileSharedT<MODE>& sh, int lx, int lz, float rx, float rz, float wy, float ob,
+                                           float s0, float s1, float s2, float2 cs, HotBox box) {
     const float wx[2] = {1.f - rx, rx}, wz[2] = {1.f - rz, rz};
 #pragma unroll
     for (int bx = 0; bx < 2; ++bx)
 #pragma unroll
         for (int bz = 0; bz < 2; ++bz) {
             const int cxl = lx + bx, czl = lz + bz;
-            if (cxl < 0 || cxl >= TX || czl < 0 || czl >= TZ) continue;
+            if (MODE == VOTE_PEAKS) {
+                if (cxl < box.x0 || cxl > box.x1 || czl < box.z0 || czl > box.z1) continue;
+            } else {
+                if (cxl < 0 || cxl >= TX || czl < 0 || czl >= TZ) continue;
+            }
             const float w = wx[bx] * wy * wz[bz] * ob;
             unsigned long long* a = sh.acc + cxl * ACC_PITCH + czl;
-            lds_add_obj<SMALL>(a, w);
-            lds_add<SMALL>(a + ACC_CH, w * cs.x);
-            lds_add<SMALL>(a + 2 * ACC_CH, w * cs.y);
-            lds_add<SMALL>(a + 3 * ACC_CH, w * s0);
-            lds_add<SMALL>(a + 4 * ACC_CH, w * s1);
-            lds_add<SMALL>(a + 5 * ACC_CH, w * s2);
-        }
-}
-
-__device__ __forceinline__ void drain64(TileShared& sh, int wave, int slot, bool active) {
+            if (MODE != VOTE_PEAKS) lds_add_obj<SMALL>(a, w);
+            if (MODE == VOTE_OBJ) continue;
+            if (MODE == VOTE_FULL) a += ACC_CH;
+            lds_add<SMALL>(a, w * cs.x);
+            lds_add<SMALL>(a + ACC_CH, w * cs.y);
+            lds_add<SMALL>(a + 2 * ACC_CH, w * s0);
+            lds_add<SMALL>(a + 3 * ACC_CH, w * s1);
+            lds_add<SMALL>(a + 4 * ACC_CH, w * s2);
+        }
+}
+
+template <int MODE>
+__device__ __forceinline__ void drain64(TileSharedT<MODE>& sh, int wave, int slot, bool active, HotBox box) {
     float rx = 0.f, rz = 0.f, wy = 0.f, ob = 0.f, s0 = 0.f, s1 = 0.f, s2 = 0.f;
     float2 cs = make_float2(0.f, 0.f);
     int lx = 0, lz = 0;
@@ -568,14 +581,16 @@
         const int e = rec & 511, rot = (rec >> 9) & 255;
         lx = (int)((rec >> 17) & 63) - 1; lz = (int)((rec >> 23) & 63) - 1;
         wy = sh.pq[4][e]; ob = sh.pq[5][e];
-        s0 = sh.pq[6][e]; s1 = sh.pq[7][e]; s2 = sh.pq[8][e];
-        cs = sh.tab[rot];
+        if constexpr (MODE != VOTE_OBJ) {
+            s0 = sh.pq[6][e]; s1 = sh.pq[7][e]; s2 = sh.pq[8][e];
+            cs = sh.tab[rot];
+        }
     }
     const bool small = fabsf(ob) * fmaxf(1.f, fmaxf(fabsf(s0), fmaxf(fabsf(s1), fabsf(s2)))) < 16384.f;
     if (__all(small)) {
-        if (active) drain_vote<true>(sh, lx, lz, rx, rz, wy, ob, s0, s1, s2, cs);
+        if (active) drain_vote<true, MODE>(sh, lx, lz, rx, rz, wy, ob, s0, s1, s2, cs, box);
     } else {
-        if (active) drain_vote<false>(sh, lx, lz, rx, rz, wy, ob, s0, s1, s2, cs);
+        if (active) drain_vote<false, MODE>(sh, lx, lz, rx, rz, wy, ob, s0, s1, s2, cs, box);
     }
 }
 
@@ -636,48 +651,46 @@
     }
 }
 
-template <bool QUEUE>
-__global__ __launch_bounds__(TW * 64) void hv_fwd_tiles(
-    int R, float res, F3 corner, I3 dims, const float2* __restrict__ tab,
-    const int* __restrict__ ystart, const int4* __restrict__ items, const float* __restrict__ rec,
+template <bool QUEUE, int MODE>
+__device__ __forceinline__ void hv_tile_item(
+    int y, int tile, int part, int nparts, int slot0, int slot_stride,
+    int R, float res, F3 corner, I3 dims,
+    const int* __restrict__ ystart, const float* __restrict__ rec,
     int64_t rec_stride, int tiles_x, int tiles_z, unsigned long long* __restrict__ partials,
     int* __restrict__ arrivals, float* __restrict__ g_obj, float* __restrict__ g_rot,
     float* __restrict__ g_scale, const int* __restrict__ list_ctl, const int* __restrict__ list_start, const int* __restrict__ list_cnt,
     const int2* __restrict__ entries, int list_mode ,
-    const int4* __restrict__ q_info, CatStride ks) {
-    ystart = cat_ws(ystart, ks.ws); items = cat_ws(items, ks.ws); rec = cat_ws(rec, ks.ws);
-    partials = cat_ws(partials, ks.ws); arrivals = cat_ws(arrivals, ks.ws); list_ctl = cat_ws(list_ctl, ks.ws);
-    list_start = cat_ws(list_start, ks.ws); list_cnt = cat_ws(list_cnt, ks.ws); entries = cat_ws(entries, ks.ws);
-    q_info = cat_ws(q_info, ks.ws);
-    g_obj = cat_el(g_obj, ks.cells); g_rot = cat_el(g_rot, 2 * ks.cells); g_scale = cat_el(g_scale, 3 * ks.cells);
-    __shared__ TileShared sh;
+    int4* __restrict__ hot, float thresh, int4* __restrict__ hot_items, const float2* __restrict__ tab) {
+    constexpr int NCH = vote_channels(MODE);
+    __shared__ TileSharedT<MODE> sh;
     __shared__ int last_flag;
+    __shared__ int hot_lds[MODE == VOTE_OBJ ? 4 : 1];
     const int X = dims.x, Y = dims.y, Z = dims.z;
     const int ntiles = tiles_x * tiles_z;
-    int y, tile, part, nparts, slot0, slot_stride;
-    if (QUEUE) {
-        if ((int)blockIdx.x >= list_ctl[2]) return;
-        const int4 item = items[blockIdx.x];
-        y = item.x; tile = item.y; part = item.z & 0xff; nparts = item.z >> 8; slot0 = item.w; slot_stride = 1;
-    } else {
-        tile = blockIdx.x % ntiles;
-        const int4 qi = q_info[blockIdx.x / ntiles];
-        if (qi.z < 0) return;
-        y = qi.x; part = qi.y; nparts = qi.z;
-        slot0 = qi.w * ntiles + tile; slot_stride = ntiles;
-    }
     const int x0 = (tile / tiles_z) * TX, z0 = (tile % tiles_z) * TZ;
     const int lane = threadIdx.x & 63, wave = threadIdx.x >> 6;
+    HotBox box{0, TX - 1, 0, TZ - 1};
+    if (MODE == VOTE_PEAKS) {
+        const int4 h = hot[y * ntiles + tile];
+        box = HotBox{h.x, h.y, h.z, h.w};
+        if (box.x0 > box.x1) return;
+    }
     if (nparts == 0) {
         const int nx0 = min(TX, X - x0), nz0 = min(TZ, Z - z0);
         for (int i = threadIdx.x; i < TCELLS; i += TW * 64) {
             const int lx = i / TZ, lz = i % TZ;
             if (lx < nx0 && lz < nz0) {
                 const int64_t cell = ((int64_t)(x0 + lx) * Y + y) * Z + z0 + lz;
-                g_obj[cell] = 0.f;
-                reinterpret_cast<float2*>(g_rot)[cell] = make_float2(0.f, 0.f);
-                g_scale[cell * 3 + 0] = 0.f; g_scale[cell * 3 + 1] = 0.f; g_scale[cell * 3 + 2] = 0.f;
-            }
+                if (MODE != VOTE_PEAKS) g_obj[cell] = 0.f;
+                if (MODE != VOTE_OBJ) {
+                    reinterpret_cast<float2*>(g_rot)[cell] = make_float2(0.f, 0.f);
+                    g_scale[cell * 3 + 0] = 0.f; g_scale[cell * 3 + 1] = 0.f; g_scale[cell * 3 + 2] = 0.f;
+                }
+            }
+        }
+        if (MODE == VOTE_OBJ && threadIdx.x == 0) {
+            hot[y * ntiles + tile] = 0.f >= thresh ? make_int4(0, nx0 - 1, 0, nz0 - 1) : make_int4(TX, -1, TZ, -1);
+            if (0.f >= thresh) hot_items[atomicAdd(&arrivals[Y * ntiles], 1)] = make_int4(y, tile, 0, slot0);
         }
         return;
     }
@@ -703,15 +716,19 @@
         bin_end[k] = !valid ? 0 : (use_list ? lbeg[k] + llen[k] : ystart[s + 1]);
     }
     const float2 tab_mine = (int)threadIdx.x < R ? tab[threadIdx.x] : make_float2(0.f, 0.f);
-    for (int i = threadIdx.x; i < ACC_WORDS; i += TW * 64) sh.acc[i] = 0ull;
+    for (int i = threadIdx.x; i < TileSharedT<MODE>::ACC_WORDS; i += TW * 64) sh.acc[i] = 0ull;
     if ((int)threadIdx.x < R) sh.tab[threadIdx.x] = tab_mine;
     if (threadIdx.x < 2) sh.next_chunk[threadIdx.x] = 0;
     if (threadIdx.x == 2) { sh.list_len = 0; sh.more = 0; }
+    if (MODE == VOTE_OBJ && threadIdx.x >= 4 && threadIdx.x < 8)
+        hot_lds[threadIdx.x - 4] = (threadIdx.x & 1) ? -1 : (threadIdx.x == 4 ? TX : TZ);
     __syncthreads();
 
     const float slack = 0.05f;
-    const float xlo = (float)(x0 - 1), xhi = (float)(x0 + TX), zlo = (float)(z0 - 1),
-                zhi = (float)(z0 + TZ);
+    const float xlo = MODE == VOTE_PEAKS ? (float)(x0 + box.x0 - 1) : (float)(x0 - 1),
+                xhi = MODE == VOTE_PEAKS ? (float)(x0 + box.x1 + 1) : (float)(x0 + TX),
+                zlo = MODE == VOTE_PEAKS ? (float)(z0 + box.z0 - 1) : (float)(z0 - 1),
+                zhi = MODE == VOTE_PEAKS ? (float)(z0 + box.z1 + 1) : (float)(z0 + TZ);
     int vq_len = 0;
 
     const int per = use_list ? LIST_CHUNK : 64;
@@ -848,9 +865,11 @@
             sh.pq[3][p] = rec[3 * rec_stride + idx];
             sh.pq[4][p] = (w < 0) ? (1.f - ry) : ry;
             sh.pq[5][p] = rec[5 * rec_stride + idx];
-            sh.pq[6][p] = rec[6 * rec_stride + idx];
-            sh.pq[7][p] = rec[7 * rec_stride + idx];
-            sh.pq[8][p] = rec[8 * rec_stride + idx];
+            if constexpr (MODE != VOTE_OBJ) {
+                sh.pq[6][p] = rec[6 * rec_stride + idx];
+                sh.pq[7][p] = rec[7 * rec_stride + idx];
+                sh.pq[8][p] = rec[8 * rec_stride + idx];
+            }
             sh.arc_start[p] = a_start;
         }
         int cum = a_len;
@@ -914,7 +933,8 @@
                 const float gz = grid_pos(epz, oz, corner.z, res);
                 if (gx >= 0 && gz >= 0 && gx < (float)(X - 1) && gz < (float)(Z - 1)) {
                     const int lx = (int)gx - x0, lz = (int)gz - z0;
-                    if (lx >= -1 && lx < TX && lz >= -1 && lz < TZ) {
+                    if (MODE == VOTE_PEAKS ? (lx >= box.x0 - 1 && lx <= box.x1 && lz >= box.z0 - 1 && lz <= box.z1)
+                                           : (lx >= -1 && lx < TX && lz >= -1 && lz < TZ)) {
                         isvote = true;
                         rx = gx - floorf(gx);
                         rz = gz - floorf(gz);
@@ -935,11 +955,11 @@
             wave_sync_lds();
             if (vq_len >= 64) {
                 vq_len -= 64;
-                drain64(sh, wave, vq_len + lane, true);
+                drain64<MODE>(sh, wave, vq_len + lane, true, box);
             }
         }
         if (vq_len > 0) {
-            drain64(sh, wave, lane, lane < vq_len);
+            drain64<MODE>(sh, wave, lane, lane < vq_len, box);
             vq_len = 0;
         }
         wave_sync_lds();
@@ -950,7 +970,7 @@
 
     if (nparts > 1) {
         unsigned long long* mine = partials + ((int64_t)slot0 + (int64_t)part * slot_stride) * (6 * TCELLS);
-        for (int i = threadIdx.x; i < 6 * TCELLS; i += TW * 64) mine[i] = sh.acc[acc_idx(i / TCELLS, i % TCELLS)];
+        for (int i = threadIdx.x; i < NCH * TCELLS; i += TW * 64) mine[i] = sh.acc[acc_idx(i / TCELLS, i % TCELLS)];
         asm volatile("s_waitcnt vmcnt(0)" ::: "memory");
         __syncthreads();
         if (threadIdx.x == 0) {
@@ -960,11 +980,13 @@
                                                    __HIP_MEMORY_SCOPE_AGENT);
             last_flag = old == nparts - 1;
             if (last_flag) __builtin_amdgcn_fence(__ATOMIC_ACQUIRE, "agent");
+            if (MODE == VOTE_OBJ && last_flag)
+                __hip_atomic_store(&arrivals[y * ntiles + tile], 0, __ATOMIC_RELAXED, __HIP_MEMORY_SCOPE_AGENT);
         }
         __syncthreads();
         if (!last_flag) return;
         const unsigned long long* base = partials + (int64_t)slot0 * (6 * TCELLS);
-        for (int i = threadIdx.x; i < 6 * TCELLS; i += TW * 64) {
+        for (int i = threadIdx.x; i < NCH * TCELLS; i += TW * 64) {
             unsigned long long sum = 0ull;
             for (int p2 = 0; p2 < nparts; ++p2) sum += base[(int64_t)p2 * slot_stride * (6 * TCELLS) + i];
             sh.acc[acc_idx(i / TCELLS, i % TCELLS)] = sum;
@@ -973,29 +995,108 @@
     }
 
     const int nx = min(TX, X - x0), nz = min(TZ, Z - z0);
-    for (int i = threadIdx.x; i < TCELLS; i += TW * 64) {
-        const int lx = i / TZ, lz = i % TZ;
-        if (lx < nx && lz < nz)
-            g_obj[((int64_t)(x0 + lx) * Y + y) * Z + z0 + lz] = (float)fx_value(sh.acc[acc_idx(0, i)]);
-    }
-    for (int i = threadIdx.x; i < TCELLS * 2; i += TW * 64) {
-        const int cell = i >> 1, j = i & 1;
-        const int lx = cell / TZ, lz = cell % TZ;
-        if (lx < nx && lz < nz) {
-            const double d = (double)(float)fx_value(sh.acc[acc_idx(0, cell)]) + 1e-7;
-            g_rot[(((int64_t)(x0 + lx) * Y + y) * Z + z0 + lz) * 2 + j] =
-                (float)((double)(float)fx_value(sh.acc[acc_idx(1 + j, cell)]) / d);
-        }
-    }
-    for (int i = threadIdx.x; i < TCELLS * 3; i += TW * 64) {
-        const int cell = i / 3, j = i - cell * 3;
-        const int lx = cell / TZ, lz = cell % TZ;
-        if (lx < nx && lz < nz) {
-            const double d = (double)(float)fx_value(sh.acc[acc_idx(0, cell)]) + 1e-7;
-            g_scale[(((int64_t)(x0 + lx) * Y + y) * Z + z0 + lz) * 3 + j] =
-                (float)((double)(float)fx_value(sh.acc[acc_idx(3 + j, cell)]) / d);
-        }
-    }
+    if constexpr (MODE == VOTE_OBJ) {
+        for (int i = threadIdx.x; i < TCELLS; i += TW * 64) {
+            const int lx = i / TZ, lz = i % TZ;
+            if (lx < nx && lz < nz) {
+                const float v = (float)fx_value(sh.acc[acc_idx(0, i)]);
+                g_obj[((int64_t)(x0 + lx) * Y + y) * Z + z0 + lz] = v;
+                if (v >= thresh) {
+                    atomicMin(&hot_lds[0], lx); atomicMax(&hot_lds[1], lx);
+                    atomicMin(&hot_lds[2], lz); atomicMax(&hot_lds[3], lz);
+                }
+            }
+        }
+        __syncthreads();
+        if (threadIdx.x == 0) {
+            hot[y * ntiles + tile] = make_int4(hot_lds[0], hot_lds[1], hot_lds[2], hot_lds[3]);
+            if (hot_lds[0] <= hot_lds[1]) {
+                const int at = atomicAdd(&arrivals[Y * ntiles], nparts);
+                for (int p2 = 0; p2 < nparts; ++p2) hot_items[at + p2] = make_int4(y, tile, p2 | (nparts << 8), slot0);
+            }
+        }
+    } else if constexpr (MODE == VOTE_PEAKS) {
+        for (int i = threadIdx.x; i < TCELLS; i += TW * 64) {
+            const int lx = i / TZ, lz = i % TZ;
+            if (lx < box.x0 || lx > box.x1 || lz < box.z0 || lz > box.z1) continue;
+            const int64_t cell = ((int64_t)(x0 + lx) * Y + y) * Z + z0 + lz;
+            const float v = g_obj[cell];
+            if (!(v >= thresh)) continue;
+            const double d = (double)v + 1e-7;
+#pragma unroll
+            for (int j = 0; j < 2; ++j) g_rot[cell * 2 + j] = (float)((double)(float)fx_value(sh.acc[acc_idx(j, i)]) / d);
+#pragma unroll
+            for (int j = 0; j < 3; ++j) g_scale[cell * 3 + j] = (float)((double)(float)fx_value(sh.acc[acc_idx(2 + j, i)]) / d);
+        }
+    } else {
+        for (int i = threadIdx.x; i < TCELLS; i += TW * 64) {
+            const int lx = i / TZ, lz = i % TZ;
+            if (lx < nx && lz < nz)
+                g_obj[((int64_t)(x0 + lx) * Y + y) * Z + z0 + lz] = (float)fx_value(sh.acc[acc_idx(0, i)]);
+        }
+        for (int i = threadIdx.x; i < TCELLS * 2; i += TW * 64) {
+            const int cell = i >> 1, j = i & 1;
+            const int lx = cell / TZ, lz = cell % TZ;
+            if (lx < nx && lz < nz) {
+                const double d = (double)(float)fx_value(sh.acc[acc_idx(0, cell)]) + 1e-7;
+                g_rot[(((int64_t)(x0 + lx) * Y + y) * Z + z0 + lz) * 2 + j] =
+                    (float)((double)(float)fx_value(sh.acc[acc_idx(1 + j, cell)]) / d);
+            }
+        }
+        for (int i = threadIdx.x; i < TCELLS * 3; i += TW * 64) {
+            const int cell = i / 3, j = i - cell * 3;
+            const int lx = cell / TZ, lz = cell % TZ;
+            if (lx < nx && lz < nz) {
+                const double d = (double)(float)fx_value(sh.acc[acc_idx(0, cell)]) + 1e-7;
+                g_scale[(((int64_t)(x0 + lx) * Y + y) * Z + z0 + lz) * 3 + j] =
+                    (float)((double)(float)fx_value(sh.acc[acc_idx(3 + j, cell)]) / d);
+            }
+        }
+    }
+}
+
+template <bool QUEUE, int MODE>
+__global__ __launch_bounds__(TW * 64) void hv_fwd_tiles(
+    int R, float res, F3 corner, I3 dims, const float2* __restrict__ tab,
+    const int* __restrict__ ystart, const int4* __restrict__ items, const float* __restrict__ rec,
+    int64_t rec_stride, int tiles_x, int tiles_z, unsigned long long* __restrict__ partials,
+    int* __restrict__ arrivals, float* __restrict__ g_obj, float* __restrict__ g_rot,
+    float* __restrict__ g_scale, const int* __restrict__ list_ctl, const int* __restrict__ list_start, const int* __restrict__ list_cnt,
+    const int2* __restrict__ entries, int list_mode ,
+    const int4* __restrict__ q_info, CatStride ks, int4* __restrict__ hot, float thresh, int4* __restrict__ hot_items) {
+    ystart = cat_ws(ystart, ks.ws); items = cat_ws(items, ks.ws); rec = cat_ws(rec, ks.ws);
+    partials = cat_ws(partials, ks.ws); arrivals = cat_ws(arrivals, ks.ws); list_ctl = cat_ws(list_ctl, ks.ws);
+    list_start = cat_ws(list_start, ks.ws); list_cnt = cat_ws(list_cnt, ks.ws); entries = cat_ws(entries, ks.ws);
+    q_info = cat_ws(q_info, ks.ws);
+    g_obj = cat_el(g_obj, ks.cells); g_rot = cat_el(g_rot, 2 * ks.cells); g_scale = cat_el(g_scale, 3 * ks.cells);
+    if (MODE != VOTE_FULL) { hot = cat_ws(hot, ks.ws); hot_items = cat_ws(hot_items, ks.ws); }
+    const int ntiles = tiles_x * tiles_z;
+#define CV_TILE_ITEM_ARGS R, res, corner, dims, ystart, rec, rec_stride, tiles_x, tiles_z, partials, arrivals, g_obj, g_rot, g_scale, \
+                          list_ctl, list_start, list_cnt, entries, list_mode, hot, thresh, hot_items
+    if (MODE == VOTE_PEAKS) {
+        const int count = arrivals[dims.y * ntiles];
+        if ((int)blockIdx.x >= count) return;
+        for (int i = blockIdx.x; i < count; i += gridDim.x) {
+            const int4 item = hot_items[i];
+            hv_tile_item<QUEUE, MODE>(item.x, item.y, item.z & 0xff, item.z >> 8, item.w, QUEUE ? 1 : ntiles, CV_TILE_ITEM_ARGS, tab);
+            __syncthreads();
+        }
+        return;
+    }
+    int y, tile, part, nparts, slot0, slot_stride;
+    if (QUEUE) {
+        if ((int)blockIdx.x >= list_ctl[2]) return;
+        const int4 item = items[blockIdx.x];
+        y = item.x; tile = item.y; part = item.z & 0xff; nparts = item.z >> 8; slot0 = item.w; slot_stride = 1;
+    } else {
+        tile = blockIdx.x % ntiles;
+        const int4 qi = q_info[blockIdx.x / ntiles];
+        if (qi.z < 0) return;
+        y = qi.x; part = qi.y; nparts = qi.z;
+        slot0 = qi.w * ntiles + tile; slot_stride = ntiles;
+    }
+    hv_tile_item<QUEUE, MODE>(y, tile, part, nparts, slot0, slot_stride, CV_TILE_ITEM_ARGS, tab);
+#undef CV_TILE_ITEM_ARGS
 }
 
 __global__ __launch_bounds__(256) void hv_bwd(
@@ -1120,6 +1221,7 @@
 
 int64_t tiles_q_bound(int64_t n, int Y) { return (int64_t)Y + (2 * n + PART_RECORDS - 1) / PART_RECORDS; }
 constexpr int QUEUE_MIN_TILES = 128;
+constexpr int PEAK_WGS = 512;
 int64_t queue_max_slots(int64_t n, int num_rots) { return 4 * n * (int64_t)num_rots / PART_VOTES + 256; }
 int64_t queue_max_items(int64_t n, int num_rots, int64_t Y, int64_t ntiles) { return Y * ntiles + queue_max_slots(n, num_rots); }
 int64_t list_capacity(int64_t n, int64_t ntiles) { return std::min<int64_t>(n * ntiles, 40 * n + 65536); }
@@ -1135,6 +1237,8 @@
     int* ystart; int* cursor; int* part_start; int4* q_info;
     unsigned long long* partials;
     int4* items; int* list_start; int* chunk_start; int* bin_of_chunk; int* chunk_off; int2* entries;
+    int4* hot_items;
+    int4* hot;
     int* zero_from;
     size_t zero_bytes;
     size_t bytes;
@@ -1167,7 +1271,7 @@
     take(L.list_cnt, q * planes);
     take(L.tile_w, q * planes);
     const size_t ycount_at = take(L.ycount, Y);
-    take(L.arrivals, planes);
+    take(L.arrivals, planes + 1);
     L.zero_from = L.queue ? L.list_ctl : L.ycount;
     L.zero_bytes = off - (L.queue ? ctl_at : ycount_at);
     take(L.ystart, Y + 1);
@@ -1181,6 +1285,8 @@
     take(L.bin_of_chunk, (size_t)L.max_chunks);
     take(L.chunk_off, q * (size_t)L.max_chunks * (size_t)ntiles);
     take(L.entries, q * (size_t)L.list_cap);
+    take(L.hot, planes);
+    take(L.hot_items, (size_t)(L.queue ? L.max_items : L.max_q * ntiles));
     L.bytes = cv_align_up(off, 256);
     return L;
 }
@@ -1285,7 +1391,7 @@
 static int hv_forward_cats(const float* d_points, const float* d_xyz, const float* d_scale, const float* d_obj, int64_t n,
                            float res, int num_rots, const float h_corner3[3], const int dims[3], float* d_grid_obj,
                            float* d_grid_rot, float* d_grid_scale, void* d_ws, size_t ws_bytes, int algo, int K,
-                           hipStream_t st) {
+                           hipStream_t st, bool peaks = false, float thresh = 0.f) {
     int rc = CV_OK;
     const float2* tab = nullptr;
     rc = get_rot_table(num_rots, &tab);
@@ -1355,11 +1461,22 @@
     const int64_t wgs = queue ? L.max_items : L.max_q * ntiles;
     CV_REQUIRE(wgs < (1ll << 31), CV_EINVAL, "grid too large");
 #define CV_TILES_ARGS num_rots, res, corner, d3, tab, L.ystart, L.items, L.rec, n, tiles_x, tiles_z, L.partials, L.arrivals, d_grid_obj, \
-                      d_grid_rot, d_grid_scale, L.list_ctl, L.list_start, L.list_cnt, L.entries, list_mode, L.q_info, ks
+                      d_grid_rot, d_grid_scale, L.list_ctl, L.list_start, L.list_cnt, L.entries, list_mode, L.q_info, ks, L.hot, thresh, L.hot_items
+#define CV_TILES_LAUNCH(MODE, WGS)                                                                           \
+    do {                                                                                                      \
+        if (queue) hv_fwd_tiles<true, MODE><<<dim3((unsigned)(WGS), K), TW * 64, 0, st>>>(CV_TILES_ARGS);     \
+        else hv_fwd_tiles<false, MODE><<<dim3((unsigned)(WGS), K), TW * 64, 0, st>>>(CV_TILES_ARGS);          \
+    } while (0)
     if (t_ev_start) CV_HIP_CHECK(hipEventRecord(t_ev_start, st));
-    if (queue) hv_fwd_tiles<true><<<dim3((unsigned)wgs, K), TW * 64, 0, st>>>(CV_TILES_ARGS);
-    else hv_fwd_tiles<false><<<dim3((unsigned)wgs, K), TW * 64, 0, st>>>(CV_TILES_ARGS);
+    if (peaks) {
+        CV_TILES_LAUNCH(VOTE_OBJ, wgs);
+        CV_LAUNCH_CHECK();
+        CV_TILES_LAUNCH(VOTE_PEAKS, std::min<int64_t>(wgs, PEAK_WGS));
+    } else {
+        CV_TILES_LAUNCH(VOTE_FULL, wgs);
+    }
     if (t_ev_stop) CV_HIP_CHECK(hipEventRecord(t_ev_stop, st));
+#undef CV_TILES_LAUNCH
 #undef CV_TILES_ARGS
     CV_LAUNCH_CHECK();
     return CV_OK;
@@ -1389,6 +1506,34 @@
     CV_REQUIRE(d_obj && d_grid_obj && d_grid_rot && d_grid_scale, CV_EINVAL, "null pointer argument");
     return hv_forward_cats(d_points, d_xyz, d_scale, d_obj, n, res, num_rots, h_corner3, dims, d_grid_obj, d_grid_rot, d_grid_scale,
                            d_ws, ws_bytes, algo, num_cats, static_cast<hipStream_t>(stream));
+}
+
+int cv_hv_forward_peaks_f32(const float* d_points, const float* d_xyz, const float* d_scale, const float* d_obj, int64_t n,
+                            float res, int num_rots, const float h_corner3[3], const int dims[3], float* d_grid_obj,
+                            float* d_grid_rot, float* d_grid_scale, void* d_ws, size_t ws_bytes, int algo, float thresh,
+                            void* stream) {
+    CV_REQUIRE(algo_ok(algo), CV_EINVAL, "algo out of range (%d: 0 auto, 1 direct, 2 tiles)", algo);
+    CV_REQUIRE(thresh == thresh, CV_EINVAL, "thresh is not a number");
+    int rc = check_common(d_points, d_xyz, d_scale, n, res, num_rots, h_corner3, dims);
+    if (rc) return rc;
+    CV_REQUIRE(d_obj && d_grid_obj && d_grid_rot && d_grid_scale, CV_EINVAL, "null pointer argument");
+    return hv_forward_cats(d_points, d_xyz, d_scale, d_obj, n, res, num_rots, h_corner3, dims, d_grid_obj, d_grid_rot, d_grid_scale,
+                           d_ws, ws_bytes, algo, 1, static_cast<hipStream_t>(stream), true, thresh);
+}
+
+int cv_hv_forward_peaks_cat_f32(const float* d_points, const float* d_xyz, const float* d_scale, const float* d_obj, int64_t n,
+                                float res, int num_rots, const float h_corner3[3], const int dims[3], int num_cats,
+                                float* d_grid_obj, float* d_grid_rot, float* d_grid_scale, void* d_ws, size_t ws_bytes, int algo,
+                                float thresh, void* stream) {
+    CV_REQUIRE(num_cats >= 1 && num_cats <= CV_MAX_CATEGORIES, CV_EINVAL, "num_cats out of range (%d, 1..%d)", num_cats,
+               CV_MAX_CATEGORIES);
+    CV_REQUIRE(algo_ok(algo), CV_EINVAL, "algo out of range (%d: 0 auto, 1 direct, 2 tiles)", algo);
+    CV_REQUIRE(thresh == thresh, CV_EINVAL, "thresh is not a number");
+    int rc = check_common(d_points, d_xyz, d_scale, n, res, num_rots, h_corner3, dims);
+    if (rc) return rc;
+    CV_REQUIRE(d_obj && d_grid_obj && d_grid_rot && d_grid_scale, CV_EINVAL, "null pointer argument");
+    return hv_forward_cats(d_points, d_xyz, d_scale, d_obj, n, res, num_rots, h_corner3, dims, d_grid_obj, d_grid_rot, d_grid_scale,
+                           d_ws, ws_bytes, algo, num_cats, static_cast<hipStream_t>(stream), true, thresh);
 }
 
 int cv_hv_backward_f32(const float* d_grad_obj, const float* d_points, const float* d_xyz,
diff --git a/canonicalvoting_amd/csrc/scene_exec.cpp b/canonicalvoting_amd/csrc/scene_exec.cpp
--- a/canonicalvoting_amd/csrc/scene_exec.cpp
+++ b/canonicalvoting_amd/csrc/scene_exec.cpp
@@ -187,8 +187,11 @@
     const float* v_scale = d->d_scale_in ? d->d_scale_in : scale;
     const float* v_prob = d->d_prob_in ? d->d_prob_in : prob;
     const int32_t* v_cls = d->d_class_in ? d->d_class_in : cls;
-    rc = cv_hv_forward_f32(d->d_points, v_xyz, v_scale, v_prob, n, d->res, d->num_rots, f.mn, f.dims, g_obj, g_rot, g_scale, vote_ws,
-                           std::max<size_t>(vote_ws_b, 256), d->vote_algo, stream);
+    rc = d->peak_quotients
+             ? cv_hv_forward_peaks_f32(d->d_points, v_xyz, v_scale, v_prob, n, d->res, d->num_rots, f.mn, f.dims, g_obj, g_rot, g_scale,
+                                       vote_ws, std::max<size_t>(vote_ws_b, 256), d->vote_algo, d->decode.thresh_high, stream)
+             : cv_hv_forward_f32(d->d_points, v_xyz, v_scale, v_prob, n, d->res, d->num_rots, f.mn, f.dims, g_obj, g_rot, g_scale, vote_ws,
+                                 std::max<size_t>(vote_ws_b, 256), d->vote_algo, stream);
     if (rc != CV_OK) return rc;
     CV_HIP_CHECK(clock.mark(3));
     clock.lap(2);
diff --git a/canonicalvoting_amd/pipeline.py b/canonicalvoting_amd/pipeline.py
--- a/canonicalvoting_amd/pipeline.py
+++ b/canonicalvoting_amd/pipeline.py
@@ -394,6 +394,7 @@
         d.d_xyz_in, d.d_scale_in, d.d_prob_in, d.d_class_in = (vp(px.data_ptr()), vp(ps.data_ptr()), vp(pp.data_ptr()),
                                                                  vp(pc.data_ptr()))
     _fill_joint_desc(d, host, c_ops, c_bufs, y, nclasses, decode_kw, adaptive_split, events)
+    d.peak_quotients = 1 if keep is None else 0
     r = _lib.SceneResult()
     ws = _call_growing(L.cv_detect_scene_f32, "cv_detect_scene_f32", d, r, dev, "scene_call", host.ws_hint)
     host.ws_hint = max(host.ws_hint, int(r.needed_ws_bytes))
@@ -521,6 +522,7 @@
     host = _scene_host(dev, max_candidates)
     _fill_scene_desc(d.scene, model, hv, None, None, None, res, policy, pieces, max(model.PLANES), log_scale)
     _fill_joint_desc(d.scene, host, c_ops, c_bufs, y, nclasses, decode_kw, adaptive_split, events)
+    d.scene.peak_quotients = 1 if keep is None else 0
     ws = _call_points(L.cv_detect_points_f32, "cv_detect_points_f32", d, r, dev, "scene_call", host.ws_hint)
     del alive
     n = int(r.n)
diff --git a/include/cv_hip.h b/include/cv_hip.h
--- a/include/cv_hip.h
+++ b/include/cv_hip.h
@@ -40,6 +40,15 @@
 int cv_hv_forward_cat_f32(const float* d_points, const float* d_xyz, const float* d_scale, const float* d_obj, int64_t n,
                           float res, int num_rots, const float h_corner3[3], const int dims[3], int num_cats, float* d_grid_obj,
                           float* d_grid_rot, float* d_grid_scale, void* d_ws, size_t ws_bytes, int algo, void* stream);
+
+int cv_hv_forward_peaks_f32(const float* d_points, const float* d_xyz, const float* d_scale, const float* d_obj, int64_t n,
+                            float res, int num_rots, const float h_corner3[3], const int dims[3], float* d_grid_obj,
+                            float* d_grid_rot, float* d_grid_scale, void* d_ws, size_t ws_bytes, int algo, float thresh,
+                            void* stream);
+int cv_hv_forward_peaks_cat_f32(const float* d_points, const float* d_xyz, const float* d_scale, const float* d_obj, int64_t n,
+                                float res, int num_rots, const float h_corner3[3], const int dims[3], int num_cats,
+                                float* d_grid_obj, float* d_grid_rot, float* d_grid_scale, void* d_ws, size_t ws_bytes, int algo,
+                                float thresh, void* stream);
 
 int cv_hv_set_part_records(int records);
 int cv_hv_set_part_records_thread(int records);
@@ -354,6 +363,7 @@
     void* events[5];
     int conv_split_target;
     int vote_part_records;
+    int peak_quotients;
 } cv_scene_desc;
 typedef struct cv_scene_result {
     int n_cand, n_boxes, n_det, truncated, range_flag, duplicates, out_of_window;
diff --git a/profiles/vote_peaks/hot_pricing.py b/profiles/vote_peaks/hot_pricing.py
--- /dev/null
+++ b/profiles/vote_peaks/hot_pricing.py
@@ -0,0 +1,59 @@
+import os
+import sys
+
+import numpy as np
+
+sys.path.insert(0, os.path.dirname(os.path.dirname(os.path.dirname(os.path.abspath(__file__)))))
+import oracle
+from canonicalvoting_amd import decode
+from canonicalvoting_amd.synth import make_scene, synth_predictions
+
+TX, TZ, R = 16, 32, 120
+
+
+def price(seed, thresh=float(decode.thresh_high)):
+    sc = make_scene(seed)
+    xyz, scale, prob, _ = synth_predictions(sc)
+    pts = sc.points
+    g_obj = oracle.hv_forward(pts, xyz, scale, prob, sc.res, R)[0]
+    corner, _, _ = oracle.grid_geometry(pts, sc.res)
+    X, Y, Z = g_obj.shape
+    hot = g_obj >= thresh
+    tx, tz = -(-X // TX), -(-Z // TZ)
+    pad = np.zeros((tx * TX, Y, tz * TZ), bool)
+    pad[:X, :, :Z] = hot
+    pair_hot = pad.reshape(tx, TX, Y, tz, TZ).any((1, 4))
+    box = np.zeros_like(pad)
+    for a, y, b in zip(*np.nonzero(pair_hot)):
+        sub = pad[a * TX:(a + 1) * TX, y, b * TZ:(b + 1) * TZ]
+        xs, zs = np.nonzero(sub.any(1))[0], np.nonzero(sub.any(0))[0]
+        box[a * TX + xs[0]:a * TX + xs[-1] + 1, y, b * TZ + zs[0]:b * TZ + zs[-1] + 1] = True
+    in_pair = np.repeat(np.repeat(pair_hot, TX, 0), TZ, 2)
+    f = np.float32
+    th = (np.arange(R, dtype=f) * f(2 * 3.141592654 / R)).astype(f)
+    cs, sn = np.cos(th.astype(np.float64)).astype(f), np.sin(th.astype(np.float64)).astype(f)
+    c = (xyz * scale).astype(f)
+    res = f(sc.res)
+    gx = ((pts[:, None, 0] + ((-cs)[None] * c[:, None, 0] + sn[None] * c[:, None, 2])) - f(corner[0])) / res
+    gz = ((pts[:, None, 2] + ((-sn)[None] * c[:, None, 0] - cs[None] * c[:, None, 2])) - f(corner[2])) / res
+    gy = np.broadcast_to((((pts[:, 1] - c[:, 1]) - f(corner[1])) / res)[:, None], gx.shape)
+    ok = (gx >= 0) & (gy >= 0) & (gz >= 0) & (gx < X - 1) & (gy < Y - 1) & (gz < Z - 1)
+    fx, fy, fz = gx[ok].astype(np.int64), gy[ok].astype(np.int64), gz[ok].astype(np.int64)
+    n_pair = n_box = n_hot = 0
+    for bx in (0, 1):
+        for by in (0, 1):
+            for bz in (0, 1):
+                i = (fx + bx, fy + by, fz + bz)
+                n_pair += int(in_pair[i].sum()); n_box += int(box[i].sum()); n_hot += int(pad[i].sum())
+    tot = 8 * fx.size
+    return dict(seed=seed, grid=(X, Y, Z), cells=X * Y * Z, votes=int(fx.size), hot_cells=int(hot.sum()), pairs=tx * tz * Y,
+                hot_pairs=int(pair_hot.sum()), in_pairs=n_pair / tot, in_boxes=n_box / tot, in_hot_cells=n_hot / tot)
+
+
+if __name__ == "__main__":
+    oracle.build()
+    for s in ([int(a) for a in sys.argv[1:]] or [0, 1, 2, 3]):
+        r = price(s)
+        print("seed %(seed)d  grid %(grid)s = %(cells)d cells  in-bounds votes %(votes)d  cells >= thresh %(hot_cells)d  "
+              "(plane, tile) pairs with one %(hot_pairs)d of %(pairs)d  contributions in those pairs %(in_pairs).3f  "
+              "in their hot boxes %(in_boxes).3f  in the hot cells %(in_hot_cells).3f" % r, flush=True)
```

Result: faster. 675.0 (median of 6 runs) (+5.7%).
